# HannesStark/3DInfomax

Measured on AMD Instinct MI355X. Metric: molecules/sec pretraining step (PNA+Net3D, QM9-50k); PNA-agg HBM GB/s vs peak, higher is better.
Workload: dtype f32

## Files before the change

### 3dinfomax_amd/_lib.py

```python
import ctypes
import os
import re
from ctypes import POINTER, c_char_p, c_double, c_float, c_int, c_int64, c_long, c_uint64, c_void_p

HERE = os.path.dirname(os.path.abspath(__file__))
_TESTING = os.environ.get('I3D_TESTING') == '1'
TEST_HOOKS = dict(peer_selftest_fail=os.environ.get('I3D_TEST_PEER_SELFTEST_FAIL') if _TESTING else None,
                  peer_fail=os.environ.get('I3D_TEST_PEER_FAIL') if _TESTING else None,
                  force_early_allreduce=_TESTING and os.environ.get('I3D_TEST_FORCE_EARLY_ALLREDUCE') == '1',
                  verbose_selftest=_TESTING and bool(os.environ.get('I3D_DEBUG_SELFTEST')))
LIB_PATH = os.environ.get('I3D_LIB_PATH') or os.path.join(HERE, 'lib', 'lib3dinfomax_hip.so')
HEADER_PATH = os.path.join(os.path.dirname(HERE), 'include', 'infomax3d_hip.h')

ACT = {'none': 0, None: 0, 'relu': 1, 'silu': 2, 'sigmoid': 3, 'leakyrelu': 4, 'tanh': 5, 'elu': 6, 'selu': 7, 'softplus': 8}
AGG = {'mean': 0, 'sum': 1, 'max': 2, 'min': 3, 'std': 4, 'var': 5}
SCALER = {'identity': 0, 'amplification': 1, 'attenuation': 2}

_P = c_void_p


class BnTail(ctypes.Structure):
    _fields_ = [('act', c_int), ('post_act', c_int), ('eps', c_float), ('momentum', c_float), ('gamma', _P),
                ('beta', _P), ('running_mean', _P), ('running_var', _P), ('mean', _P), ('invstd', _P),
                ('workspace', _P), ('gemm_workspace', _P), ('gemm_workspace_bytes', c_long), ('num_batches_tracked', _P)]


class FcArgs(ctypes.Structure):
    _fields_ = [('tail', BnTail), ('rows', c_int), ('f_in', c_int), ('f_out', c_int), ('ldw', c_int), ('x', _P),
                ('W', _P), ('bias', _P), ('residual', _P), ('xact', _P), ('pre_keep', _P), ('y', _P), ('grad_y', _P),
                ('grad_pre', _P), ('grad_gamma', _P), ('grad_beta', _P), ('grad_W', _P), ('grad_bias', _P),
                ('grad_x', _P), ('W_dgrad_panel', _P), ('W_fwd_panel', _P)]


class EdgeFcArgs(ctypes.Structure):
    _fields_ = [('tail', BnTail), ('num_nodes', c_int), ('num_edges', c_int), ('f_h', c_int), ('f_q', c_int),
                ('f_out', c_int), ('ldw', c_int), ('q_rows', c_int), ('v_pad', c_int), ('q_code', _P), ('onehot', _P),
                ('grad_Q', _P), ('h', _P), ('q', _P), ('W', _P), ('bias', _P), ('src_s', _P),
                ('dst_s', _P), ('in_ptr', _P), ('out_ptr', _P), ('out_epos', _P), ('P', _P), ('Q', _P), ('xact', _P),
                ('pre_keep', _P), ('y', _P), ('grad_y', _P), ('grad_pre', _P), ('grad_P', _P), ('grad_gamma', _P),
                ('grad_beta', _P), ('grad_W', _P), ('grad_bias', _P), ('grad_h', _P), ('grad_q', _P),
                ('grad_q_accumulate', c_int)]


class GroupedFcArgs(ctypes.Structure):
    _fields_ = [('tail', BnTail), ('num_nodes', c_int), ('f_h', c_int), ('f_out', c_int), ('agg_width', c_int),
                ('ldw', c_int), ('n_groups', c_int), ('n_scalers', c_int), ('m_padded', c_int),
                ('group_start', c_int * 32), ('group_count', c_int * 32), ('coef', c_float * 128), ('h', _P),
                ('agg', _P), ('W', _P), ('bias', _P), ('residual', _P), ('deg_rows', _P), ('deg_tile_group', _P),
                ('WD', _P), ('xact', _P), ('pre_keep', _P), ('y', _P), ('grad_y', _P), ('grad_pre', _P),
                ('grad_WD', _P), ('grad_gamma', _P), ('grad_beta', _P), ('grad_W', _P), ('grad_bias', _P),
                ('grad_h', _P), ('grad_agg', _P)]


class PnaLayerArgs(ctypes.Structure):
    _fields_ = [('edge', EdgeFcArgs), ('n_pre_extra', c_int), ('pre', FcArgs * 3), ('n_aggregators', c_int),
                ('n_scalers', c_int), ('force_scalers', c_int), ('aggregators', c_int * 8), ('scalers', c_int * 4),
                ('avg_d_log', c_float), ('msg', _P), ('grad_msg', _P), ('post', GroupedFcArgs), ('n_post_extra', c_int),
                ('postx', FcArgs * 3), ('residual', c_int), ('grad_out', _P), ('agg_event_start', _P), ('agg_event_stop', _P),
                ('fused_bn', c_int), ('defer_join', c_int), ('stats_ws', _P), ('aff', _P * 4), ('weights_ready', c_int),
                ('merge_h', c_int), ('Wcat', _P), ('bcat', _P), ('PL', _P), ('DL', _P), ('wgrad_split', c_int), ('eval_mode', c_int), ('msg_bf16', c_int),
                ('edge_bias_partial', _P), ('Wcat_panel', _P), ('Wcat_dgrad_panel', _P)]


class Net3dEdgeArgs(ctypes.Structure):
    _fields_ = [('tail_in', BnTail), ('tail_msg', BnTail), ('num_nodes', c_int), ('num_edges', c_int), ('hidden', c_int),
                ('n_enc', c_int), ('reduce_mean', c_int), ('ld_w_in', c_int), ('ld_w_msg', c_int), ('d_raw', _P), ('perm', _P),
                ('dst_s', _P), ('in_ptr', _P), ('emb', _P), ('W_in', _P), ('b_in', _P), ('W_msg', _P), ('b_msg', _P),
                ('w_gate', _P), ('b_gate', _P), ('stats', _P), ('aff_in', _P), ('aff_msg', _P), ('x_msg', _P), ('d_out', _P),
                ('msg', _P), ('m_sum', _P), ('grad_m_sum', _P), ('grad_ya', _P), ('grad_lin', _P), ('partial', _P), ('grad_W_in', _P),
                ('grad_b_in', _P), ('grad_gamma_in', _P), ('grad_beta_in', _P), ('grad_W_msg', _P), ('grad_b_msg', _P),
                ('grad_gamma_msg', _P), ('grad_beta_msg', _P), ('grad_w_gate', _P), ('grad_b_gate', _P), ('grad_emb', _P), ('store_bf16', c_int), ('x_center', _P)]


class FcParams(ctypes.Structure):
    _fields_ = [('W', _P), ('bias', _P), ('gamma', _P), ('beta', _P), ('running_mean', _P), ('running_var', _P),
                ('num_batches_tracked', _P), ('grad_W', _P), ('grad_bias', _P), ('grad_gamma', _P), ('grad_beta', _P),
                ('f_in', c_int), ('f_out', c_int), ('act', c_int), ('eps', c_float), ('momentum', c_float)]


class PnaModel(ctypes.Structure):
    _fields_ = [('training', c_int), ('n_layers', c_int), ('hidden', c_int), ('n_pre', c_int), ('residual', c_int), ('n_aggregators', c_int),
                ('aggregators', c_int * 8), ('n_scalers', c_int), ('scalers', c_int * 4), ('avg_d_log', c_float),
                ('pre', (FcParams * 4) * 16), ('post', FcParams * 16), ('n_atom_tables', c_int), ('atom_dims', c_int * 16),
                ('atom_tables', _P * 16), ('grad_atom_tables', _P), ('n_bond_tables', c_int), ('bond_dims', c_int * 16),
                ('bond_tables', _P * 16), ('grad_bond_tables', _P), ('n_readout', c_int), ('readout_ops', c_int * 4),
                ('n_head', c_int), ('head', FcParams * 4)]


class PnaBatch(ctypes.Structure):
    _fields_ = [('num_nodes', c_int), ('num_edges', c_int), ('num_graphs', c_int), ('atom_feat', _P), ('bond_feat', _P),
                ('in_ptr', _P), ('perm', _P), ('src_s', _P), ('dst_s', _P), ('out_ptr', _P), ('out_epos', _P),
                ('graph_ptr', _P), ('deg_rows', _P), ('deg_tile_group', _P), ('m_padded', c_int), ('n_groups', c_int),
                ('group_degree', c_int * 32), ('group_start', c_int * 32), ('group_count', c_int * 32), ('comb', _P),
                ('n_comb', c_int), ('v_pad', c_int)]


class BnEvalAff(ctypes.Structure):
    _fields_ = [('running_mean', _P), ('running_var', _P), ('gamma', _P), ('beta', _P), ('aff', _P), ('feat', c_int),
                ('eps', c_float)]


class CopyBlock(ctypes.Structure):
    _fields_ = [('src', _P), ('dst', _P), ('rows', c_int), ('cols', c_int), ('ld_src', c_long), ('ld_dst', c_long)]


class TowerLayerArgs(ctypes.Structure):
    _fields_ = ([(n, c_int) for n in ('num_nodes', 'num_edges', 'f_in', 'f_edge', 'f_msg', 'f_out', 'f_mix', 'ldp', 'ldq', 'ldgp',
                                      'ldgq', 'n_aggregators', 'n_scalers', 'residual', 'training', 'grad_e_accumulate')]
                + [('aggregators', c_int * 8), ('scalers', c_int * 4), ('avg_d_log', c_float), ('eps', c_float), ('momentum', c_float)]
                + [(n, _P) for n in ('h', 'e', 'snorm', 'Wp', 'bp', 'Wq', 'bq', 'gamma', 'beta', 'running_mean', 'running_var', 'Wm',
                                     'bm', 'src_s', 'dst_s', 'in_ptr', 'out_ptr', 'out_epos', 'saved', 'scratch', 'workspace',
                                     'gemm_workspace')]
                + [('gemm_workspace_bytes', c_long)]
                + [(n, _P) for n in ('out', 'grad_out', 'grad_h', 'grad_e', 'grad_Wp', 'grad_bp', 'grad_Wq', 'grad_bq', 'grad_gamma',
                                     'grad_beta', 'grad_Wm', 'grad_bm')]
                + [('n_towers', c_int), ('n_deg_groups', c_int), ('m_padded', c_int), ('group_start', c_int * 32),
                   ('group_count', c_int * 32), ('coef', c_float * 128), ('deg_rows', _P), ('deg_tile_group', _P)])


class NodeDropView(ctypes.Structure):
    _fields_ = ([('keep', _P), ('graph_ptr', _P), ('edge_ptr', _P), ('deg_base', _P), ('pad_range', _P)]
                + [(n, c_int) for n in ('n_groups', 'num_nodes', 'num_edges', 'rows')]
                + [(n, _P) for n in ('src', 'dst', 'atom_feat', 'bond_feat', 'in_ptr', 'perm', 'src_s', 'dst_s', 'out_ptr', 'out_epos',
                                     'inv_perm', 'deg_rows')])


ALL_GATHER_F32 = ctypes.CFUNCTYPE(c_int, c_void_p, c_void_p, c_void_p, c_long, c_void_p)
ALL_REDUCE_F64 = ctypes.CFUNCTYPE(c_int, c_void_p, c_void_p, c_long, c_void_p)


class Collectives(ctypes.Structure):
    _fields_ = [('world', c_int), ('all_gather_f32', ALL_GATHER_F32), ('all_reduce_f64', ALL_REDUCE_F64), ('user', _P),
                ('scratch', _P), ('scratch_bytes', c_long)]


class WgradProblem(ctypes.Structure):
    _fields_ = [('A', _P), ('B', _P), ('rows', _P), ('rows_total', c_long), ('lda', c_int), ('ldb', c_int), ('M', c_int),
                ('N', c_int), ('k_begin', c_int), ('k_count', c_int)]


class WgradOutput(ctypes.Structure):
    _fields_ = [('kind', c_int), ('n_groups', c_int), ('first_problem', c_int), ('ldc', c_int), ('c_split', c_int),
                ('n_scalers', c_int), ('c_delta', c_long), ('scaler_stride', c_long), ('C', _P), ('aff', _P), ('row', _P),
                ('coef', POINTER(c_float))]


_SIGNATURES = {
    'i3d_bn_eval_aff_multi': (c_int, [POINTER(BnEvalAff), c_int, _P]),
    'i3d_set_collectives': (c_int, [POINTER(Collectives)]),
    'i3d_collectives_world': (c_int, []),
    'i3d_collectives_all_gather_f32': (c_int, [c_void_p, c_void_p, c_long, c_void_p]),
    'i3d_collectives_all_reduce_f64': (c_int, [c_void_p, c_long, c_void_p]),
    'i3d_rccl_available': (c_int, []),
    'i3d_rccl_unique_id': (c_int, [ctypes.c_char_p]),
    'i3d_rccl_init': (c_int, [ctypes.c_char_p, c_int, c_int, POINTER(c_void_p)]),
    'i3d_rccl_destroy': (c_int, [_P]),
    'i3d_set_collectives_rccl': (c_int, [_P, c_int, _P, c_long]),
    'i3d_block_copy': (c_int, [_P, c_int, c_int, _P]),
    'i3d_gru_gates_fwd': (c_int, [_P, _P, _P, c_int, c_int, _P, _P, _P]),
    'i3d_gru_gates_bwd': (c_int, [_P, _P, _P, _P, c_int, c_int, _P, _P, _P, _P]),
    'i3d_copy_cols': (c_int, [_P, c_int, c_int, _P, c_int, _P]),
    'i3d_edge_sqdist': (c_int, [_P, _P, _P, c_int, _P, c_int, c_int, c_int, _P]),
    'i3d_tower_layer_saved_floats': (c_long, [POINTER(TowerLayerArgs)]),
    'i3d_tower_layer_scratch_floats': (c_long, [POINTER(TowerLayerArgs)]),
    'i3d_tower_layer_fwd': (c_int, [POINTER(TowerLayerArgs), _P]),
    'i3d_tower_layer_bwd': (c_int, [POINTER(TowerLayerArgs), _P]),
    'i3d_peer_mailbox_bytes': (c_long, []),
    'i3d_peer_handle_bytes': (c_int, []),
    'i3d_peer_alloc': (c_int, [POINTER(c_void_p), ctypes.c_char_p]),
    'i3d_peer_free': (c_int, [_P]),
    'i3d_peer_open': (c_int, [_P, ctypes.c_char_p, c_int, c_int, c_double, POINTER(c_void_p)]),
    'i3d_set_collectives_peer': (c_int, [_P, _P, c_long]),
    'i3d_peer_bind_stream': (c_int, [_P, _P, _P, c_long]),
    'i3d_peer_status': (c_int, [_P]),
    'i3d_peer_sequence': (ctypes.c_longlong, [_P]),
    'i3d_peer_close': (c_int, [_P]),
    'i3d_gemm_f32_fused_src': (c_int, [c_int, c_int, c_int, _P, c_int, c_long, _P, c_int, _P, c_int, _P, c_int, _P, c_int, _P, c_int,
                                       _P, _P, _P, c_long, _P]),
    'i3d_pna_pack_h_weights': (c_int, [_P, c_int, c_int, _P, c_int, c_int, _P, c_int, _P, _P, _P]),
    'i3d_bn_bwd_strided': (c_int, [_P, _P, _P, c_int, c_int, c_int, c_int, _P, _P, _P, _P, _P, _P, _P, c_int, _P, _P, _P]),
    'i3d_wgrad_multi_supported': (c_int, [POINTER(WgradProblem), c_int, POINTER(WgradOutput), c_int]),
    'i3d_wgrad_multi_workspace_bytes': (c_long, [c_int]),
    'i3d_wgrad_multi_min_workspace_bytes': (c_long, [POINTER(WgradProblem), c_int]),
    'i3d_wgrad_multi': (c_int, [POINTER(WgradProblem), c_int, POINTER(WgradOutput), c_int, _P, c_long, _P]),
    'i3d_pna_model_saved_floats': (c_long, [POINTER(PnaModel), POINTER(PnaBatch)]),
    'i3d_pna_model_scratch_floats': (c_long, [POINTER(PnaModel), POINTER(PnaBatch)]),
    'i3d_pna_model_fwd': (c_int, [POINTER(PnaModel), POINTER(PnaBatch), _P, _P, _P, _P, _P, _P, _P, POINTER(c_void_p)]),
    'i3d_pna_model_bwd': (c_int, [_P, POINTER(PnaModel), _P, _P, _P, _P, c_long, _P]),
    'i3d_pna_model_bwd_part': (c_int, [_P, POINTER(PnaModel), _P, _P, _P, _P, c_long, c_int, c_int, _P]),
    'i3d_pna_model_ctx_free': (c_int, [_P]),
    'i3d_pna_messages_normalized': (c_int, [_P, _P, c_long, c_int, _P, _P]),
    'i3d_pna_messages_normalized_ex': (c_int, [_P, c_int, _P, c_long, c_int, _P, _P]),
    'i3d_pna_model_debug_messages': (c_int, [_P, c_int, _P, _P]),
    'i3d_event_create': (c_int, [POINTER(c_void_p)]),
    'i3d_event_destroy': (c_int, [_P]),
    'i3d_event_record': (c_int, [_P, _P]),
    'i3d_event_elapsed_ms': (c_int, [_P, _P, POINTER(c_float)]),
    'i3d_set_matmul_precision': (c_int, [c_int]),
    'i3d_get_matmul_precision': (c_int, []),
    'i3d_set_fp32_products': (c_int, [c_int]),
    'i3d_get_fp32_products': (c_int, []),
    'i3d_net3d_edge_supported': (c_int, [c_int, c_int]),
    'i3d_net3d_edge_stats_floats': (c_long, [c_int, c_int]),
    'i3d_net3d_edge_bwd_floats': (c_long, [c_int, c_int, c_int]),
    'i3d_net3d_edge_fwd': (c_int, [POINTER(Net3dEdgeArgs), _P]),
    'i3d_net3d_edge_bwd': (c_int, [POINTER(Net3dEdgeArgs), _P]),
    'i3d_wgrad_stream_fork': (c_int, [_P, POINTER(_P)]),
    'i3d_wgrad_stream_peek': (c_int, [_P, POINTER(_P)]),
    'i3d_pna_layer_weights_fwd': (c_int, [POINTER(PnaLayerArgs), _P]),
    'i3d_pna_layer_fwd': (c_int, [POINTER(PnaLayerArgs), _P]),
    'i3d_pna_layer_bwd': (c_int, [POINTER(PnaLayerArgs), _P]),
    'i3d_fc_bn_fwd': (c_int, [POINTER(FcArgs), _P]),
    'i3d_fc_bn_bwd': (c_int, [POINTER(FcArgs), _P]),
    'i3d_fc_bn_bwd_chain': (c_int, [POINTER(FcArgs), _P]),
    'i3d_fc_bn_bwd_wgrad': (c_int, [POINTER(FcArgs), _P]),
    'i3d_edge_fc_bn_fwd': (c_int, [POINTER(EdgeFcArgs), _P]),
    'i3d_edge_fc_bn_bwd': (c_int, [POINTER(EdgeFcArgs), _P]),
    'i3d_grouped_fc_bn_fwd': (c_int, [POINTER(GroupedFcArgs), _P]),
    'i3d_grouped_fc_bn_bwd': (c_int, [POINTER(GroupedFcArgs), _P]),
    'i3d_pna_layer_stats_floats': (c_long, [c_int, c_int, c_int, c_int]),
    'i3d_bn_finalize_partials': (c_int, [_P, c_int, c_int, c_float, c_float, _P, _P, _P, _P, _P, _P, _P, _P, _P]),
    'i3d_edge_stats_rows_per_tile': (c_int, [c_int]),
    'i3d_edge_combine_act_stats': (c_int, [_P, c_int, _P, _P, _P, _P, _P, c_int, c_int, c_int, _P, _P, _P]),
    'i3d_gemm_f32_fused': (c_int, [c_int, c_int, c_int, _P, c_int, c_long, _P, c_int, _P, c_int, _P, c_int, _P, c_int, _P, _P,
                                   _P, c_long, _P]),
    'i3d_gemm_f32_wgrad_bn': (c_int, [c_int, c_int, c_int, _P, c_int, _P, c_int, _P, c_int, _P, _P, _P, c_long, _P]),
    'i3d_pna_aggregate_fwd_aff': (c_int, [_P, _P, _P, c_int, c_int, POINTER(c_int), c_int, POINTER(c_int), c_int, c_int, c_float,
                                          _P, _P]),
    'i3d_pna_aggregate_fwd_ex': (c_int, [_P, c_int, _P, _P, c_int, c_int, POINTER(c_int), c_int, POINTER(c_int), c_int, c_int, c_float, _P, _P]),
    'i3d_pna_aggregate_bwd_ex': (c_int, [_P, _P, c_int, _P, _P, c_int, c_int, POINTER(c_int), c_int, POINTER(c_int), c_int, c_int, c_float, _P, _P]),
    'i3d_gemm_f32_fused_bf16out': (c_int, [c_int, c_int, c_int, _P, c_int, c_long, _P, c_int, _P, c_int, _P, _P, c_int, _P, _P]),
    'i3d_bn_bwd_x_bf16': (c_int, [_P, _P, c_int, c_int, c_int, c_int, _P, _P, _P, _P, _P, _P, _P, _P, _P, _P]),
    'i3d_pna_aggregate_bwd_aff': (c_int, [_P, _P, _P, _P, c_int, c_int, POINTER(c_int), c_int, POINTER(c_int), c_int, c_int,
                                          c_float, _P, _P]),
    'i3d_bn_bias_partial_floats': (c_long, [c_int]),
    'i3d_set_bn_bwd_one_launch': (c_int, [c_int]),
    'i3d_panel_packed_bytes': (c_long, [c_int, c_int]),
    'i3d_panel_pack': (c_int, [_P, c_int, c_int, c_int, c_int, _P, _P]),
    'i3d_panel_pack_multi': (c_int, [_P, c_int, _P]),
    'i3d_panel_gemm': (c_int, [c_int, c_int, c_int, _P, c_int, _P, _P, c_int, _P, c_int, _P]),
    'i3d_panel_stats_tiles': (c_int, [c_int]),
    'i3d_panel_gemm_fused': (c_int, [c_int, c_int, c_int, _P, c_int, _P, _P, c_int, _P, _P, c_int, _P, _P]),
    'i3d_bn_bwd_one_launch_supported': (c_int, [c_int, c_int]),
    'i3d_bn_bwd_edge_sums': (c_int, [_P, _P, c_int, c_int, c_int, _P, _P, _P, _P, _P, _P, _P, _P, _P, _P, c_int, _P, _P, c_int, _P, _P]),
    'i3d_colsum_strided': (c_int, [_P, c_int, c_int, c_int, _P, _P, _P]),
    'i3d_wgrad_stream_join': (c_int, [_P]),
    'i3d_adam_chunk_elems': (c_int, []),
    'i3d_adam_chunk_bytes': (c_int, []),
    'i3d_adam_step': (c_int, [_P, c_int, _P, c_int, c_double, c_double, c_double, c_double, c_double, c_double, c_double, _P]),
    'i3d_ema_chunk_elems': (c_int, []),
    'i3d_ema_chunk_bytes': (c_int, []),
    'i3d_ema_update': (c_int, [_P, c_int, c_float, c_float, _P]),
    'i3d_ntxent_loss_scratch_floats': (c_long, [c_int, c_int]),
    'i3d_ntxent_loss_fwd': (c_int, [_P, _P, c_int, c_int, c_int, c_int, c_int, c_float, c_float, c_float, _P, _P, _P]),
    'i3d_ntxent_loss_bwd': (c_int, [_P, _P, c_int, c_int, c_int, c_int, c_int, c_float, c_float, c_float, _P, _P, _P, _P, _P, _P]),
    'i3d_abi_version': (c_int, []),
    'i3d_last_error': (c_char_p, []),
    'i3d_embedding_sum_fwd': (c_int, [_P, _P, c_int, c_int, POINTER(c_void_p), c_int, _P, _P]),
    'i3d_embedding_sum_bwd': (c_int, [_P, _P, c_int, c_int, _P, c_int, POINTER(c_void_p), POINTER(c_int), _P]),
    'i3d_pna_aggregate_fwd_towers': (c_int, [_P, _P, c_int, c_int, c_int, POINTER(c_int), c_int, POINTER(c_int), c_int, c_int, c_float, _P, _P]),
    'i3d_pna_aggregate_bwd_towers': (c_int, [_P, _P, _P, c_int, c_int, c_int, POINTER(c_int), c_int, POINTER(c_int), c_int, c_int, c_float,
                                             _P, _P]),
    'i3d_pna_aggregate_fwd': (c_int, [_P, _P, c_int, c_int, POINTER(c_int), c_int, POINTER(c_int), c_int, c_int, c_float, _P,
                                      _P]),
    'i3d_pna_aggregate_bwd': (c_int, [_P, _P, _P, c_int, c_int, POINTER(c_int), c_int, POINTER(c_int), c_int, c_int, c_float,
                                      _P, _P]),
    'i3d_segment_readout_fwd': (c_int, [_P, _P, c_int, c_int, POINTER(c_int), c_int, _P, _P]),
    'i3d_segment_readout_bwd': (c_int, [_P, _P, _P, c_int, c_int, POINTER(c_int), c_int, _P, _P]),
    'i3d_gemm_f32': (c_int, [c_int, c_int, c_int, c_int, c_int, _P, c_int, _P, c_int, _P, c_int, _P, c_int, _P]),
    'i3d_gemm_f32_ex': (c_int, [c_int, c_int, c_int, c_int, c_int, _P, c_int, _P, c_int, _P, c_int, _P, c_int, c_int, c_int,
                                _P, c_long, _P]),
    'i3d_gemm_f32_blocks': (c_int, [c_int, c_int, c_int, c_int, c_int, _P, c_int, _P, c_int, c_int, c_long, c_long, _P, c_int,
                                    c_int, c_long, c_int, _P, c_long, _P]),
    'i3d_gemm_f32_ws': (c_int, [c_int, c_int, c_int, c_int, c_int, _P, c_int, _P, c_int, _P, c_int, _P, c_int, _P, c_long, _P]),
    'i3d_gemm_f32_grouped_batched': (c_int, [c_int, c_int, c_int, c_int, _P, c_int, c_long, c_long, _P, _P, _P, c_int, c_long, c_long, _P, c_int,
                                             c_long, c_int, c_int, _P]),
    'i3d_gemm_f32_batched': (c_int, [c_int, c_int, c_int, c_int, c_int, _P, c_int, c_long, _P, c_int, c_long, _P, c_int, c_long, c_int,
                                     c_int, _P, c_long, _P]),
    'i3d_pna_combine_weights_fwd': (c_int, [_P, c_int, c_int, c_int, c_int, c_int, c_int, POINTER(c_float), _P, _P]),
    'i3d_pna_combine_weights_bwd': (c_int, [_P, c_int, c_int, c_int, c_int, c_int, c_int, POINTER(c_float), _P, _P]),
    'i3d_gemm_f32_grouped': (c_int, [c_int, c_int, c_int, c_int, _P, c_int, c_long, _P, _P, _P, c_int, c_long, _P, c_int,
                                     c_int, _P]),
    'i3d_gemm_f32_rowsubset': (c_int, [c_int, c_int, c_int, _P, c_int, _P, c_int, _P, c_long, _P, c_int, c_int, _P]),
    'i3d_gemm_f32_rowsubset_multi': (c_int, [c_int, c_int, c_int, POINTER(c_int), POINTER(c_int), _P, c_int, _P, c_int, _P,
                                             c_long, _P, c_long, c_int, c_int, c_int, c_int, _P, c_long, _P]),
    'i3d_colreduce_workspace_bytes': (c_long, [c_int, c_int]),
    'i3d_act_stats_fwd': (c_int, [_P, c_int, c_int, c_int, _P, c_float, c_float, _P, _P, _P, _P, _P, _P, _P]),
    'i3d_act_stats_fwd_counted': (c_int, [_P, c_int, c_int, c_int, _P, c_float, c_float, _P, _P, _P, _P, _P, _P, _P, _P]),
    'i3d_bn_finalize_stats': (c_int, [_P, c_int, c_float, c_float, _P, _P, _P, _P, _P]),
    'i3d_bn_apply_fwd': (c_int, [_P, c_int, c_int, _P, _P, _P, _P, c_int, _P, _P, _P]),
    'i3d_bn_eval_fwd': (c_int, [_P, c_int, c_int, _P, _P, c_float, _P, _P, c_int, _P, _P, _P]),
    'i3d_bn_bwd': (c_int, [_P, _P, _P, c_int, c_int, c_int, c_int, _P, _P, _P, _P, _P, _P, _P, _P, _P, _P, c_long, _P, _P]),
    'i3d_bn_eval_bwd': (c_int, [_P, _P, _P, c_int, c_int, c_int, c_int, _P, _P, c_float, _P, _P, _P, _P, _P, _P, _P]),
    'i3d_colsum': (c_int, [_P, _P, c_int, c_int, _P, _P, _P]),
    'i3d_act_fwd': (c_int, [_P, c_long, c_int, _P, _P]),
    'i3d_act_bwd': (c_int, [_P, _P, c_long, c_int, _P, _P]),
    'i3d_add_inplace': (c_int, [_P, _P, c_long, _P]),
    'i3d_add': (c_int, [_P, _P, c_long, _P, _P]),
    'i3d_mul': (c_int, [_P, _P, c_long, _P, _P]),
    'i3d_broadcast_row': (c_int, [_P, c_long, c_int, _P, _P]),
    'i3d_edge_combine_fwd': (c_int, [_P, c_int, _P, _P, _P, _P, _P, c_int, c_int, _P, _P]),
    'i3d_multihot': (c_int, [_P, _P, c_int, c_int, POINTER(c_int), c_int, _P, _P]),
    'i3d_edge_codes': (c_int, [_P, _P, c_int, c_int, POINTER(c_int), c_int, _P, _P, _P]),
    'i3d_segment_sum_bf16': (c_int, [_P, c_int, _P, _P, c_int, c_int, c_int, _P, c_int, _P]),
    'i3d_segment_sum_pair': (c_int, [_P, c_int, _P, _P, _P, _P, _P, _P, c_int, c_int, c_int, _P]),
    'i3d_segment_sum': (c_int, [_P, c_int, _P, _P, c_int, c_int, c_int, _P, c_int, _P]),
    'i3d_segment_bcast': (c_int, [_P, _P, _P, c_int, c_int, c_int, _P, _P]),
    'i3d_gather_rows': (c_int, [_P, _P, c_int, c_int, _P, _P]),
    'i3d_fourier_encode': (c_int, [_P, c_int, c_int, _P, _P]),
    'i3d_soft_edge_fwd': (c_int, [_P, _P, _P, c_int, c_int, _P, _P, _P]),
    'i3d_soft_edge_bwd': (c_int, [_P, _P, _P, _P, c_int, c_int, _P, _P, _P]),
    'i3d_row_norms': (c_int, [_P, c_int, c_int, _P, _P]),
    'i3d_ntxent_fwd': (c_int, [_P, _P, _P, c_int, c_int, c_int, c_int, c_float, c_float, c_float, _P, _P, _P, _P]),
    'i3d_ntxent_bwd': (c_int, [_P, _P, _P, _P, _P, c_int, c_int, c_int, c_int, c_float, c_float, c_float, _P, _P, _P, _P, _P]),
    'i3d_row_axpy': (c_int, [_P, _P, c_int, c_int, _P, _P]),
    'i3d_row_scale': (c_int, [_P, _P, c_int, c_int, _P, _P]),
    'i3d_contrastive_metrics_out_doubles': (c_long, [c_int, c_int]),
    'i3d_contrastive_metrics_work_floats': (c_long, [c_int] * 5),
    'i3d_contrastive_metrics': (c_int, [_P, _P] + [c_int] * 5 + [c_float] * 3 + [_P, _P, _P]),
    'i3d_complete_graph_build': (c_int, [_P, _P, _P, c_int, c_int, c_int, _P, _P, _P, _P, _P, _P, _P, _P, _P, _P]),
    'i3d_mha_fwd': (c_int, [_P, _P, c_int, c_int, c_int, c_int, c_float, _P, _P, _P]),
    'i3d_mha_bwd': (c_int, [_P, _P, _P, _P, _P, c_int, c_int, c_int, c_int, c_float, _P, _P, _P]),
    'i3d_ln_res_fwd': (c_int, [_P, _P, _P, _P, c_int, c_int, c_float, _P, _P, _P, _P]),
    'i3d_ln_res_partial_floats': (c_long, [c_int, c_int]),
    'i3d_ln_res_bwd': (c_int, [_P, _P, _P, _P, _P, _P, c_int, c_int, _P, _P, _P, _P, _P]),
    'i3d_pair_sum_fwd': (c_int, [_P, _P, _P, _P, _P, c_int, c_int, _P, _P]),
    'i3d_pair_sum_bwd': (c_int, [_P, _P, _P, _P, _P, _P, c_int, c_int, _P, _P]),
    'i3d_pair_norm_fwd': (c_int, [_P, _P, _P, _P, c_int, c_int, _P, _P]),
    'i3d_pair_norm_bwd': (c_int, [_P, _P, _P, _P, _P, _P, c_int, c_int, _P, _P]),
    'i3d_pair_mlp_supported': (c_int, [c_int]),
    'i3d_pair_mlp_workspace_floats': (c_long, [c_int, c_int]),
    'i3d_pair_mlp_fwd': (c_int, [_P] * 9 + [c_int, c_int, c_int, c_float, c_float] + [_P] * 8),
    'i3d_pair_mlp_bwd': (c_int, [_P] * 13 + [c_int, c_int, c_int, c_int] + [_P] * 10),
    'i3d_mse_partial_floats': (c_long, [c_long]),
    'i3d_mse_fwd': (c_int, [_P, _P, c_long, c_double, _P, _P, _P]),
    'i3d_mse_bwd': (c_int, [_P, _P, c_long, c_double, _P, _P, _P, _P]),
    'i3d_node_drop_build': (c_int, [_P, _P, _P, _P, _P, _P, _P, _P, _P, _P, _P, c_int, c_int, c_int, c_int, c_int, c_int,
                                    POINTER(NodeDropView), c_int, _P]),
    'i3d_noised_graph_build': (c_int, [_P, _P, _P, c_int, c_int, c_int, c_int, c_int, c_float, c_uint64, c_uint64] + [_P] * 12),
    'i3d_row_normalize_fwd': (c_int, [_P, c_int, c_int, _P, _P, _P]),
    'i3d_row_normalize_bwd': (c_int, [_P, _P, _P, c_int, c_int, _P, _P]),
    'i3d_sep2d_max_conformers': (c_int, []),
    'i3d_sep2d_fwd': (c_int, [_P, _P, _P, c_int, c_int, c_float, _P, _P, _P, _P]),
    'i3d_sep2d_bwd': (c_int, [_P, _P, _P, _P, _P, c_int, c_int, c_float, _P, _P, _P, _P, _P]),
    'i3d_mmd_pair_fwd': (c_int, [_P, _P, c_int, c_int, c_int, c_int, c_double, _P, _P, _P, _P, _P]),
    'i3d_mmd_pair_bwd': (c_int, [_P] * 7 + [c_int, c_int, c_int, c_int, c_double] + [_P] * 5),
    'i3d_kl_mp_fwd': (c_int, [_P, _P, c_int, c_int, c_int, c_double, _P, _P, _P]),
    'i3d_kl_mp_bwd': (c_int, [_P, _P, c_int, c_int, c_int, c_double, _P, _P, _P, _P]),
    'i3d_gauss_lik_fwd': (c_int, [_P, _P, c_int, c_int, c_int, c_long, c_long, _P, _P]),
    'i3d_gauss_lik_loss': (c_int, [_P, c_int, c_double, _P, _P, _P]),
    'i3d_gauss_lik_probs': (c_int, [_P, c_int, _P, _P]),
    'i3d_gauss_lik_bwd': (c_int, [_P, _P, c_int, c_int, c_int, c_long, c_long, _P, _P, c_double, _P, _P, _P, _P, _P]),
    'i3d_gauss_jsd_fwd': (c_int, [_P, _P, c_int, c_int, c_int, _P, _P, _P, _P, _P]),
    'i3d_gauss_jsd_bwd': (c_int, [_P, _P, c_int, c_int, c_int, _P, _P, _P, _P, _P, _P]),
    'i3d_masked_loss_partial_floats': (c_long, [c_int, c_int]),
    'i3d_masked_loss_fwd': (c_int, [_P, _P, c_int, c_int, c_int, _P, _P, _P]),
    'i3d_masked_loss_bwd': (c_int, [_P, _P, c_int, c_int, c_int, _P, _P, _P, _P]),
    'i3d_task_moments_partial_floats': (c_long, [c_int, c_int]),
    'i3d_task_moments': (c_int, [_P, _P, c_int, c_int, _P, _P, _P]),
    'i3d_gin_chunk_edges': (c_int, []),
    'i3d_gin_conv_bwd_partial_floats': (c_long, [c_int, c_int, c_int, c_int]),
    'i3d_gin_conv_fwd': (c_int, [_P, _P, _P, c_int, _P, c_int, _P, _P, _P, _P, c_int, c_int, c_int, _P, _P, _P]),
    'i3d_gin_conv_bwd': (c_int, [_P] * 3 + [c_int] + [_P] * 8 + [c_int, c_int, c_int] + [_P] * 5),
    'i3d_gate_reduce_max_feat': (c_int, []),
    'i3d_gate_reduce_fwd': (c_int, [_P] * 5 + [c_int] * 4 + [_P] * 3),
    'i3d_gate_reduce_bwd': (c_int, [_P] * 5 + [c_int] * 4 + [_P] * 4),
    'i3d_geomol_edge_fwd': (c_int, [_P] * 4 + [c_int] * 3 + [_P] * 2),
    'i3d_geomol_edge_bwd': (c_int, [_P] * 5 + [c_int] * 3 + [_P] * 3),
    'i3d_geomol_residual_fwd': (c_int, [_P] * 3 + [c_long, c_int] + [_P] * 2),
    'i3d_geomol_residual_bwd': (c_int, [_P] * 3 + [c_long, c_int] + [_P] * 4),
    'i3d_lg_row_chunk': (c_int, []),
    'i3d_lg_ntxent_scratch_floats': (c_long, [c_int, c_int]),
    'i3d_lg_ntxent_work_floats': (c_long, [c_int, c_int, c_int]),
    'i3d_lg_ntxent_fwd': (c_int, [_P, _P, _P, c_int, c_int, c_int, c_float, c_float, c_int, _P, _P, _P]),
    'i3d_lg_ntxent_bwd': (c_int, [_P, _P, _P, c_int, c_int, c_int, c_float, c_float, c_int, _P, _P, _P, _P, _P, _P]),
    'i3d_conf_match_max_conformers': (c_int, []),
    'i3d_per_conf_max_conformers': (c_int, []),
    'i3d_conf_match_work_floats': (c_long, [c_int]),
    'i3d_conf_match_fwd': (c_int, [_P, _P, _P, c_int, c_int, c_int, c_float] + [_P] * 8),
    'i3d_conf_match_bwd': (c_int, [_P] * 9 + [c_int, c_int, c_int, c_int, c_int, c_float] + [_P] * 5),
    'i3d_per_conf_fwd': (c_int, [_P, _P, _P, c_int, c_int, c_int, c_float, _P, _P, _P, _P]),
    'i3d_per_conf_bwd': (c_int, [_P] * 5 + [c_int, c_int, c_int, c_float] + [_P] * 5),
    'i3d_hardneg_max_extra': (c_int, []),
    'i3d_hardneg_norms': (c_int, [_P] * 3 + [c_int] * 5 + [_P] * 5),
    'i3d_hardneg_fwd': (c_int, [c_int] + [_P] * 5 + [c_int] * 4 + [c_double] * 5 + [_P] * 4),
    'i3d_hardneg_bwd': (c_int, [c_int] + [_P] * 9 + [c_int] * 6 + [c_double] * 3 + [_P] * 8),
    'i3d_hardneg_loss_scratch_floats': (c_long, [c_int, c_int, c_int]),
    'i3d_hardneg_loss_fwd': (c_int, [c_int] + [_P] * 3 + [c_int] * 6 + [c_double] * 5 + [_P] * 3),
    'i3d_hardneg_loss_bwd': (c_int, [c_int] + [_P] * 3 + [c_int] * 6 + [c_double] * 3 + [_P] * 7),
    'i3d_bs_max_repeats': (c_int, []),
    'i3d_bs_pass_blocks': (c_int, [c_int]),
    'i3d_bs_moments': (c_int, [_P, _P, c_int, c_int] + [_P] * 6),
    'i3d_bs_matrix_pass': (c_int, [_P, c_int, c_int] + [c_double] * 4 + [_P, _P]),
    'i3d_bs_finish': (c_int, [_P, c_int, c_double, _P, c_int, c_int, c_double, _P, _P]),
    'i3d_bs_col_bwd': (c_int, [_P] * 8 + [c_int, c_int, _P] + [c_double] * 4 + [_P] * 4),
    'i3d_bs_rows_fwd': (c_int, [_P, _P, c_int, c_int, c_int, _P, _P, _P]),
    'i3d_bs_rows_bwd': (c_int, [_P, _P, c_int, c_int, c_int, _P, c_double] + [_P] * 4),
}

_lib = None


class HipLibraryError(RuntimeError):
    pass


def declared_symbols():
    with open(HEADER_PATH) as f:
        text = f.read()
    text = re.sub(r'/\*.*?\*/', '', text, flags=re.S)
    return sorted(set(re.findall(r'\b(i3d_[a-z0-9_]+)\s*\(', text)))


def load():
    global _lib
    if _lib is not None:
        return _lib
    if not os.path.exists(LIB_PATH):
        raise HipLibraryError(
            f'{LIB_PATH} not found: build it with `python -c "import __graft_entry__ as g; g.build()"` '
            '(hipcc --offload-arch=gfx950).  There is no CPU fallback for the product path.')
    lib = ctypes.CDLL(LIB_PATH)
    for name, (res, args) in _SIGNATURES.items():
        fn = getattr(lib, name)
        fn.restype = res
        fn.argtypes = args
    prec = os.environ.get('I3D_MATMUL_PRECISION', 'fp32').lower()
    if prec not in ('fp32', 'bf16'):
        raise HipLibraryError(f'I3D_MATMUL_PRECISION={prec!r}: fp32 or bf16')
    lib.i3d_set_matmul_precision(int(prec == 'bf16'))
    _lib = lib
    return lib


NOT_TAKEN = 1


def check(rc, name):
    if rc != 0:
        msg = load().i3d_last_error()
        raise HipLibraryError(f'{name} failed (rc={rc}): {msg.decode() if msg else ""}')


def int_array(values):
    return (c_int * len(values))(*values)


def ptr_array(ptrs):
    return (c_void_p * len(ptrs))(*ptrs)
```

### 3dinfomax_amd/csrc/composite.hip

```cpp
#include "common.h"

using namespace i3d;

#define TRY(call)                 \
    do {                          \
        int rc_ = (call);         \
        if (rc_ != I3D_OK) return rc_; \
    } while (0)

#include <algorithm>
#include <cstdlib>
#include <cstring>
#include <map>
#include <mutex>
#include <utility>

namespace {

struct Aux {
    hipStream_t s = nullptr;
    hipEvent_t fork = nullptr, join = nullptr;
};

Aux* aux_for(hipStream_t main) {
// ... 162 lines not shown
        const int V = a->q_rows;
        TRY(i3d_gemm_f32_ws(1, 0, a->v_pad, Fo, E, a->onehot, a->v_pad, a->grad_pre, Fo, a->grad_Q, Fo, nullptr, 0, ws, wsb, wst));
        TRY(i3d_gemm_f32_ws(1, 0, Fo, a->f_q, V, a->grad_Q, Fo, a->q, a->f_q, a->grad_W + 2 * Fh, a->ldw, nullptr, 0, ws, wsb, wst));
        if (a->grad_q != nullptr)
            TRY(i3d_gemm_f32(0, 0, V, a->f_q, Fo, a->grad_Q, Fo, a->W + 2 * Fh, a->ldw, a->grad_q, a->f_q, nullptr,
                             a->grad_q_accumulate, wst));
    } else if (a->q != nullptr) {
        TRY(i3d_gemm_f32_ws(1, 0, Fo, a->f_q, E, a->grad_pre, Fo, a->q, a->f_q, a->grad_W + 2 * Fh, a->ldw, nullptr, 0, ws, wsb, wst));
        if (a->grad_q != nullptr)
            TRY(i3d_gemm_f32(0, 0, E, a->f_q, Fo, a->grad_pre, Fo, a->W + 2 * Fh, a->ldw, a->grad_q, a->f_q, nullptr, 0, wst));
    }
    return I3D_OK;
}

static int edge_fc_bn_bwd_wgrad(const I3dEdgeFcArgs* a, void* wst) {
    TRY(edge_fc_bn_bwd_wgrad_p(a, wst));
    return edge_fc_bn_bwd_wgrad_q(a, wst);
}

extern "C" int i3d_edge_fc_bn_bwd(const I3dEdgeFcArgs* a, void* stream) {
    I3D_CHECK_ARG(a != nullptr && a->num_edges > 0 && a->num_nodes > 0, "bad arguments");
    TRY(edge_fc_bn_bwd_chain(a, stream));
    TRY(edge_fc_bn_bwd_wgrad(a, stream));
    return edge_fc_bn_bwd_dgrad(a, stream);
}

extern "C" int i3d_grouped_fc_bn_fwd(const I3dGroupedFcArgs* a, void* stream) {
    I3D_CHECK_ARG(a != nullptr && a->num_nodes > 0 && a->n_groups > 0, "bad arguments");
    const int Fh = a->f_h, Fo = a->f_out, A = a->agg_width, N = a->num_nodes;
    float* lin = a->pre_keep ? a->pre_keep : a->xact;
    TRY(i3d_gemm_f32(0, 1, N, Fo, Fh, a->h, Fh, a->W, a->ldw, lin, Fo, a->bias, 0, stream));
    TRY(i3d_pna_combine_weights_fwd(a->W, a->ldw, Fh, Fo, A, a->n_groups, a->n_scalers, a->coef, a->WD, stream));
    TRY(i3d_gemm_f32_grouped(1, a->m_padded, Fo, A, a->agg, A, N, a->deg_rows, a->deg_tile_group, a->WD, A, (long)Fo * A, lin,
                             Fo, 1, stream));
    return tail_fwd(&a->tail, N, Fo, lin, a->xact, a->residual, a->y, stream);
}

static int grouped_fc_bn_bwd_chain(const I3dGroupedFcArgs* a, void* stream, int grad_h_accumulate = 0) {
    const int Fh = a->f_h, Fo = a->f_out, A = a->agg_width, N = a->num_nodes;
    TRY(tail_bwd(&a->tail, N, Fo, a->grad_y, a->xact, a->pre_keep, a->grad_gamma, a->grad_beta, a->grad_pre, a->grad_bias,
                 stream));
    TRY(i3d_gemm_f32(0, 0, N, Fh, Fo, a->grad_pre, Fo, a->W, a->ldw, a->grad_h, Fh, nullptr, grad_h_accumulate, stream));
    return i3d_gemm_f32_grouped(0, a->m_padded, A, Fo, a->grad_pre, Fo, N, a->deg_rows, a->deg_tile_group, a->WD, A,
                                (long)Fo * A, a->grad_agg, A, 0, stream);
}

static int grouped_fc_bn_bwd_wgrad(const I3dGroupedFcArgs* a, void* wst) {
    const int Fh = a->f_h, Fo = a->f_out, A = a->agg_width, N = a->num_nodes;
    TRY(i3d_gemm_f32_ws(1, 0, Fo, Fh, N, a->grad_pre, Fo, a->h, Fh, a->grad_W, a->ldw, nullptr, 0, a->tail.gemm_workspace,
                        a->tail.gemm_workspace_bytes, wst));
    TRY(i3d_gemm_f32_rowsubset_multi(Fo, A, a->n_groups, a->group_start, a->group_count, a->grad_pre, Fo, a->agg, A,
                                     a->deg_rows, N, a->grad_WD, (long)Fo * A, A, 0, -1, 0, a->tail.gemm_workspace,
                                     a->tail.gemm_workspace_bytes, wst));
    return i3d_pna_combine_weights_bwd(a->grad_WD, a->ldw, Fh, Fo, A, a->n_groups, a->n_scalers, a->coef, a->grad_W, wst);
}

extern "C" int i3d_grouped_fc_bn_bwd(const I3dGroupedFcArgs* a, void* stream) {
    I3D_CHECK_ARG(a != nullptr && a->num_nodes > 0 && a->n_groups > 0, "bad arguments");
    TRY(grouped_fc_bn_bwd_chain(a, stream));
    return grouped_fc_bn_bwd_wgrad(a, stream);
}

static bool merge_h_ok(const I3dPnaLayerArgs* a) {
    return a->merge_h && a->fused_bn && a->n_post_extra == 0 && a->Wcat != nullptr && a->bcat != nullptr && a->PL != nullptr &&
           a->post.f_h == a->edge.f_h && a->post.pre_keep == nullptr;
}

static int pack_layer_weights(const I3dPnaLayerArgs* a, void* stream) {
    const I3dEdgeFcArgs* e = &a->edge;
    const I3dGroupedFcArgs* p = &a->post;
    TRY(i3d_pna_pack_h_weights(e->W, e->ldw, e->f_out, p->W, p->ldw, p->f_out, p->bias, e->f_h, a->Wcat, a->bcat, stream));
    I3dPanelPack w[8];
    int n = 0;
    const int WL = 2 * e->f_out + p->f_out;
    if (a->Wcat_panel != nullptr) w[n++] = I3dPanelPack{a->Wcat, e->f_h, WL, e->f_h, 1, a->Wcat_panel};
    if (a->Wcat_dgrad_panel != nullptr) w[n++] = I3dPanelPack{a->Wcat, e->f_h, e->f_h, WL, 0, a->Wcat_dgrad_panel};
    for (int i = 0; i < a->n_pre_extra && n + 2 <= 8; ++i) {
        const I3dFcArgs* c = &a->pre[i];
        if (c->W_dgrad_panel != nullptr) w[n++] = I3dPanelPack{c->W, c->ldw, c->f_in, c->f_out, 0, c->W_dgrad_panel};
        if (c->W_fwd_panel != nullptr) w[n++] = I3dPanelPack{c->W, c->ldw, c->f_out, c->f_in, 1, c->W_fwd_panel};
    }
    if (n > 0) TRY(i3d_panel_pack_multi(w, n, stream));
    return I3D_OK;
}

static bool edge_bias_on_chain(const I3dPnaLayerArgs* a) {
    return a->wgrad_split != 0;
}

static bool edge_bwd_fused_ok(const I3dPnaLayerArgs* a) {
    const I3dEdgeFcArgs* e = &a->edge;
    return merge_h_ok(a) && a->DL != nullptr && e->pre_keep == nullptr && relu_class(e->tail.act) && e->tail.post_act == I3D_ACT_NONE &&
           e->f_out % 4 == 0 && e->f_out <= 512 && a->post.f_out % 4 == 0 && e->out_ptr != nullptr && e->out_epos != nullptr &&
           a->edge_bias_partial != nullptr && e->grad_bias != nullptr;
}

static int pna_layer_wgrad_multi(const I3dPnaLayerArgs* a, void* wst, bool dry_run, int part = 0) {
    static const bool on = [] { const char* e = getenv("I3D_WGRAD_MULTI"); return e == nullptr || e[0] != '0'; }();
    const I3dEdgeFcArgs* e = &a->edge;
    const I3dGroupedFcArgs* g = &a->post;
    if (!on || a->n_post_extra != 0 || e->q == nullptr || e->q_rows <= 0) return 0;
    const int Fh = e->f_h, Fo = e->f_out, N = e->num_nodes, E = e->num_edges, A = g->agg_width;
    const bool merged = merge_h_ok(a) && a->DL != nullptr;
    const int WL = 2 * Fo + g->f_out;
    const float* dlin = merged ? a->DL + 2 * Fo : g->grad_pre;
    const int ld_dlin = merged ? WL : g->f_out;
    const float* dP = merged ? a->DL : e->grad_P;
    const int ld_dP = merged ? WL : 2 * Fo;
    constexpr int MAX_PROBLEMS = 40, MAX_OUTPUTS = 8, MAX_GROUPS = 32, MAX_SCALERS = 4;
    I3dWgradProblem pr[MAX_PROBLEMS];
    I3dWgradOutput out[MAX_OUTPUTS];
    float coef[MAX_GROUPS * MAX_SCALERS];
    const int fixed_problems = 3 + (a->n_pre_extra > 0 ? a->n_pre_extra : 0);
    if (g->n_scalers > MAX_SCALERS || g->n_scalers < 0 || fixed_problems >= MAX_PROBLEMS || 4 + a->n_pre_extra > MAX_OUTPUTS) return 0;
    const int max_group_problems = MAX_PROBLEMS - fixed_problems < MAX_GROUPS ? MAX_PROBLEMS - fixed_problems : MAX_GROUPS;
    std::memset(pr, 0, sizeof(pr));
    std::memset(out, 0, sizeof(out));
    int np = 0, no = 0;
    auto problem = [&](const float* Ap, int lda, int M, const float* Bp, int ldb, int Nn, long rows_total, const int* rows,
                       int k_begin, int k_count) {
        I3dWgradProblem& p = pr[np++];
        p.A = Ap; p.B = Bp; p.rows = rows; p.rows_total = rows_total; p.lda = lda; p.ldb = ldb; p.M = M; p.N = Nn;
        p.k_begin = k_begin; p.k_count = k_count;
    };
    const bool do_post = part != 2, do_pre = part != 1;
    if (do_post) {
        out[no].kind = I3D_WGRAD_PLAIN; out[no].n_groups = 1; out[no].first_problem = np; out[no].C = g->grad_W; out[no].ldc = g->ldw;
        ++no;
        problem(dlin, ld_dlin, g->f_out, g->h, Fh, Fh, N, nullptr, 0, N);
    }
    if (do_post) {
        I3dWgradOutput& o = out[no];
        o.kind = I3D_WGRAD_COMBINE; o.first_problem = np; o.C = g->grad_W + Fh; o.ldc = g->ldw;
        o.n_scalers = g->n_scalers; o.scaler_stride = A; o.coef = coef;
        int ng = 0;
        for (int k = 0; k < g->n_groups; ++k) {
            bool any = false;
            for (int s = 0; s < g->n_scalers; ++s) any = any || g->coef[k * g->n_scalers + s] != 0.f;
            if (!any || g->group_count[k] == 0) continue;
            if (ng >= max_group_problems) return 0;
            for (int s = 0; s < g->n_scalers; ++s) coef[ng * g->n_scalers + s] = g->coef[k * g->n_scalers + s];
            problem(dlin, ld_dlin, g->f_out, g->agg, A, A, N, g->deg_rows, g->group_start[k], g->group_count[k]);
            ++ng;
        }
        if (ng == 0) return 0;
        o.n_groups = ng;
        ++no;
    }
    for (int i = a->n_pre_extra - 1; i >= 0 && do_pre; --i) {
        const I3dFcArgs* c = &a->pre[i];
        I3dWgradOutput& o = out[no++];
        o.n_groups = 1; o.first_problem = np; o.C = c->grad_W; o.ldc = c->ldw;
        if (a->fused_bn) { o.kind = I3D_WGRAD_BN; o.aff = a->aff[i]; o.row = c->grad_bias; }
        else o.kind = I3D_WGRAD_PLAIN;
        problem(c->grad_pre, c->f_out, c->f_out, c->x, c->f_in, c->f_in, c->rows, nullptr, 0, c->rows);
    }
    if (do_pre) {
        I3dWgradOutput& o = out[no++];
        o.kind = I3D_WGRAD_PLAIN; o.n_groups = 1; o.first_problem = np; o.C = e->grad_W; o.ldc = e->ldw;
        o.c_split = Fo; o.c_delta = (long)Fh - (long)Fo * e->ldw;
        problem(dP, ld_dP, 2 * Fo, e->h, Fh, Fh, N, nullptr, 0, N);
    }
    if (do_pre) {
        I3dWgradOutput& o = out[no++];
        o.kind = I3D_WGRAD_PLAIN; o.n_groups = 1; o.first_problem = np; o.C = e->grad_Q; o.ldc = Fo;
        problem(e->onehot, e->v_pad, e->v_pad, e->grad_pre, Fo, Fo, E, nullptr, 0, E);
// ... 3 lines not shown
    if (ws == nullptr || !i3d_wgrad_multi_supported(pr, np, out, no) || i3d_wgrad_multi_min_workspace_bytes(pr, np) > wsb) return 0;
    if (dry_run) return 1;
    if (do_pre && edge_bwd_fused_ok(a) && !edge_bias_on_chain(a))
        TRY(i3d_colsum_strided(a->DL + Fo, 2 * Fo + a->post.f_out, N, Fo, e->grad_bias, a->edge_bias_partial, wst));
    TRY(i3d_wgrad_multi(pr, np, out, no, ws, wsb, wst));
    if (!do_pre) return 1;
    const int V = e->q_rows;
    TRY(i3d_gemm_f32_ws(1, 0, Fo, e->f_q, V, e->grad_Q, Fo, e->q, e->f_q, e->grad_W + 2 * Fh, e->ldw, nullptr, 0, ws, wsb, wst));
    if (e->grad_q != nullptr)
        TRY(i3d_gemm_f32(0, 0, V, e->f_q, Fo, e->grad_Q, Fo, e->W + 2 * Fh, e->ldw, e->grad_q, e->f_q, nullptr, e->grad_q_accumulate, wst));
    return 1;
}

static bool wgrad_multi_layer_ok(const I3dPnaLayerArgs* a);

static bool simple_act(int act) { return act == I3D_ACT_NONE || act == I3D_ACT_RELU || act == I3D_ACT_LEAKY_RELU; }

static int finalize_stats(const I3dBnTail* t, const float* partial, int tiles, int feat, float* aff, void* stream,
                          int eval_mode = 0) {
    if (eval_mode) return I3D_OK;
    return i3d_bn_finalize_partials(partial, tiles, feat, t->eps, t->momentum, t->gamma, t->beta, t->mean, t->invstd,
                                    t->running_mean, t->running_var, t->num_batches_tracked, aff, stream);
}

static int pna_layer_fwd_fused(const I3dPnaLayerArgs* a, void* stream) {
    const I3dEdgeFcArgs* e = &a->edge;
    const int Fh = e->f_h, Fo = e->f_out, N = e->num_nodes, E = e->num_edges;
    I3D_CHECK_ARG(a->stats_ws != nullptr && a->n_post_extra == 0 && e->pre_keep == nullptr && simple_act(e->tail.act) &&
                      e->tail.post_act == I3D_ACT_NONE && a->aff[0] != nullptr, "fused BatchNorm: unsupported block shape");
    const I3dGroupedFcArgs* pg = &a->post;
    const bool merged = merge_h_ok(a);
    const int WL = 2 * Fo + pg->f_out;
    const float* P = e->P;
    int ldp = 2 * Fo;
    if (merged) {
        if (!a->weights_ready) TRY(pack_layer_weights(a, stream));
        if (panel_ok(a->Wcat_panel, Fh, WL))
            TRY(i3d_panel_gemm(N, WL, Fh, e->h, Fh, a->Wcat_panel, a->PL, WL, a->bcat, 0, stream));
        else
            TRY(i3d_gemm_f32(0, 1, N, WL, Fh, e->h, Fh, a->Wcat, Fh, a->PL, WL, a->bcat, 0, stream));
        P = a->PL;
        ldp = WL;
    } else {
        const long wdelta = (long)Fh - (long)Fo * e->ldw, wview = (long)(Fo - 1) * e->ldw + 2 * Fh;
        TRY(i3d_gemm_f32_blocks(0, 1, N, 2 * Fo, Fh, e->h, Fh, e->W, e->ldw, Fo, wdelta, wview, e->P, 2 * Fo, 0, 0, 0, nullptr, 0,
                                stream));
    }
    if (e->q != nullptr && !a->weights_ready)
        TRY(i3d_gemm_f32(0, 1, e->q_rows > 0 ? e->q_rows : E, Fo, e->f_q, e->q, e->f_q, e->W + 2 * Fh, e->ldw, e->Q, Fo,
                         nullptr, 0, stream));
    TRY(i3d_edge_combine_act_stats(P, ldp, e->q ? e->Q : nullptr, e->q_rows > 0 ? e->q_code : nullptr, e->bias, e->src_s,
                                   e->dst_s, E, Fo, e->tail.act, e->xact, a->stats_ws, stream));
    TRY(finalize_stats(&e->tail, a->stats_ws, cdiv(E, i3d_edge_stats_rows_per_tile(Fo)), Fo, a->aff[0], stream, a->eval_mode));
    const float* x = e->xact;
    const float* aff = a->aff[0];
    int f_in = Fo;
    for (int i = 0; i < a->n_pre_extra; ++i) {
        const I3dFcArgs* c = &a->pre[i];
        I3D_CHECK_ARG(c->pre_keep == nullptr && simple_act(c->tail.act) && c->tail.post_act == I3D_ACT_NONE &&
                          a->aff[i + 1] != nullptr && c->rows == E && c->f_in == f_in, "fused BatchNorm: unsupported block shape");
        int stat_tiles = cdiv(E, 64);
        if (a->msg_bf16 && i == a->n_pre_extra - 1)
            TRY(i3d_gemm_f32_fused_bf16out(E, c->f_out, f_in, x, f_in, E, c->W, c->ldw, c->xact, c->f_out, c->bias, aff, c->tail.act,
                                           a->stats_ws, stream));
        else if (merged && panel_ok(c->W_fwd_panel, f_in, c->f_out) && (((uintptr_t)x | (uintptr_t)c->xact | (uintptr_t)aff) & 15) == 0) {
            TRY(i3d_panel_gemm_fused(E, c->f_out, f_in, x, f_in, c->W_fwd_panel, c->xact, c->f_out, c->bias, aff, c->tail.act, a->stats_ws,
                                     stream));
            stat_tiles = i3d_panel_stats_tiles(E);
        } else
            TRY(i3d_gemm_f32_fused(E, c->f_out, f_in, x, f_in, E, c->W, c->ldw, c->xact, c->f_out, c->bias, 0, aff, c->tail.act,
                                   a->stats_ws, nullptr, nullptr, 0, stream));
        TRY(finalize_stats(&c->tail, a->stats_ws, stat_tiles, c->f_out, a->aff[i + 1], stream, a->eval_mode));
        x = c->xact;
        aff = a->aff[i + 1];
        f_in = c->f_out;
    }
    if (a->agg_event_start != nullptr && a->agg_event_stop != nullptr) k4_time_next_launch(a->agg_event_start, a->agg_event_stop);
    TRY(i3d_pna_aggregate_fwd_ex(x, a->msg_bf16 && a->n_pre_extra > 0, aff, e->in_ptr, N, f_in, a->aggregators, a->n_aggregators, a->scalers,
                                 a->n_scalers, a->force_scalers, a->avg_d_log, const_cast<float*>(a->post.agg), stream));
    const I3dGroupedFcArgs* p = &a->post;
    I3D_CHECK_ARG(p->pre_keep == nullptr && simple_act(p->tail.act), "fused BatchNorm: unsupported block shape");
    const int A = p->agg_width, Fp = p->f_out;
    if (!merged) TRY(i3d_gemm_f32(0, 1, N, Fp, p->f_h, p->h, p->f_h, p->W, p->ldw, p->xact, Fp, p->bias, 0, stream));
    if (!a->weights_ready)
        TRY(i3d_pna_combine_weights_fwd(p->W, p->ldw, p->f_h, Fp, A, p->n_groups, p->n_scalers, p->coef, p->WD, stream));
    TRY(i3d_gemm_f32_fused_src(p->m_padded, Fp, A, p->agg, A, N, p->WD, A, p->xact, Fp, merged ? a->PL + 2 * Fo : nullptr, WL,
                               nullptr, 1, nullptr, p->tail.act, a->stats_ws, p->deg_rows, p->deg_tile_group, (long)Fp * A, stream));
    if (a->eval_mode)
        return i3d_bn_eval_fwd(p->xact, N, Fp, p->tail.running_mean, p->tail.running_var, p->tail.eps, p->tail.gamma, p->tail.beta,
                               p->tail.post_act, p->residual, p->y, stream);
    TRY(finalize_stats(&p->tail, a->stats_ws, p->m_padded / 64, Fp, nullptr, stream));
    return i3d_bn_apply_fwd(p->xact, N, Fp, p->tail.mean, p->tail.invstd, p->tail.gamma, p->tail.beta, p->tail.post_act,
                            p->residual, p->y, stream);
}

extern "C" int i3d_pna_layer_weights_fwd(const I3dPnaLayerArgs* a, void* stream) {
    I3D_CHECK_ARG(a != nullptr && a->fused_bn, "fused_bn layers only");
    const I3dEdgeFcArgs* e = &a->edge;
    const I3dGroupedFcArgs* p = &a->post;
    if (e->q != nullptr)
        TRY(i3d_gemm_f32(0, 1, e->q_rows > 0 ? e->q_rows : e->num_edges, e->f_out, e->f_q, e->q, e->f_q, e->W + 2 * e->f_h, e->ldw,
                         e->Q, e->f_out, nullptr, 0, stream));
    if (merge_h_ok(a)) TRY(pack_layer_weights(a, stream));
    return i3d_pna_combine_weights_fwd(p->W, p->ldw, p->f_h, p->f_out, p->agg_width, p->n_groups, p->n_scalers, p->coef, p->WD,
                                       stream);
}

extern "C" int i3d_wgrad_stream_fork(void* stream, void** side) {
    I3D_CHECK_ARG(side != nullptr, "null");
    *side = fork_wgrad(aux_for((hipStream_t)stream), stream);
    return I3D_OK;
}

extern "C" int i3d_wgrad_stream_peek(void* stream, void** side) {
    I3D_CHECK_ARG(side != nullptr, "null");
    Aux* x = aux_for((hipStream_t)stream);
    *side = x != nullptr ? (void*)x->s : stream;
    return I3D_OK;
}

extern "C" long i3d_pna_layer_stats_floats(int num_nodes, int num_edges, int m_padded, int f) {
    (void)num_nodes;
    const int rpt = i3d_edge_stats_rows_per_tile(f);
    long tiles = cdiv(num_edges, rpt > 0 ? rpt : 1);
    tiles = std::max<long>(tiles, 2L * cdiv(num_edges, 64));
    tiles = std::max<long>(tiles, m_padded / 64 + 1);
    return tiles * 3 * f;
}

extern "C" int i3d_pna_layer_fwd(const I3dPnaLayerArgs* a, void* stream) {
    I3D_CHECK_ARG(a != nullptr && a->n_pre_extra >= 0 && a->n_pre_extra <= I3D_MAX_EXTRA_FC && a->n_post_extra >= 0 &&
                      a->n_post_extra <= I3D_MAX_EXTRA_FC, "bad arguments");
    if (a->fused_bn) return pna_layer_fwd_fused(a, stream);
    TRY(i3d_edge_fc_bn_fwd(&a->edge, stream));
    for (int i = 0; i < a->n_pre_extra; ++i) TRY(i3d_fc_bn_fwd(&a->pre[i], stream));
    if (a->agg_event_start != nullptr && a->agg_event_stop != nullptr) k4_time_next_launch(a->agg_event_start, a->agg_event_stop);
    TRY(i3d_pna_aggregate_fwd(a->msg, a->edge.in_ptr, a->edge.num_nodes, a->edge.f_out, a->aggregators, a->n_aggregators,
                              a->scalers, a->n_scalers, a->force_scalers, a->avg_d_log, const_cast<float*>(a->post.agg), stream));
    TRY(i3d_grouped_fc_bn_fwd(&a->post, stream));
    for (int i = 0; i < a->n_post_extra; ++i) TRY(i3d_fc_bn_fwd(&a->postx[i], stream));
    return I3D_OK;
}

extern "C" int i3d_pna_layer_bwd(const I3dPnaLayerArgs* a, void* stream) {
    I3D_CHECK_ARG(a != nullptr && a->n_pre_extra >= 0 && a->n_pre_extra <= I3D_MAX_EXTRA_FC && a->n_post_extra >= 0 &&
                      a->n_post_extra <= I3D_MAX_EXTRA_FC, "bad arguments");
    Aux* x = aux_for((hipStream_t)stream);
    for (int i = a->n_post_extra - 1; i >= 0; --i) TRY(fc_bn_bwd_chain(&a->postx[i], stream));
    const bool inplace = a->residual && a->post.grad_h == a->grad_out && a->n_post_extra == 0;
    I3D_CHECK_ARG(a->post.grad_h != a->grad_out || inplace, "grad_h may alias grad_out only for a residual layer without extra blocks");
    const bool multi = wgrad_multi_layer_ok(a);
    const bool merged = multi && merge_h_ok(a) && a->DL != nullptr;
    const long n = (long)a->edge.num_nodes * a->edge.f_h;
    if (merged) {
        const I3dGroupedFcArgs* g = &a->post;
        const int WLb = 2 * a->edge.f_out + g->f_out;
        float* dlin = a->DL + 2 * a->edge.f_out;
        TRY(i3d_bn_bwd_strided(g->grad_y, g->xact, g->pre_keep, g->num_nodes, g->f_out, g->tail.act, g->tail.post_act, g->tail.mean,
                               g->tail.invstd, g->tail.gamma, g->tail.beta, g->grad_gamma, g->grad_beta, dlin, WLb, g->grad_bias,
                               g->tail.workspace, stream));
        TRY(i3d_gemm_f32_grouped(0, g->m_padded, g->agg_width, g->f_out, dlin, WLb, g->num_nodes, g->deg_rows, g->deg_tile_group, g->WD,
                                 g->agg_width, (long)g->f_out * g->agg_width, g->grad_agg, g->agg_width, 0, stream));
    } else {
        TRY(grouped_fc_bn_bwd_chain(&a->post, stream, inplace ? 1 : 0));
        if (a->residual && !inplace) TRY(i3d_add_inplace(a->post.grad_h, a->grad_out, n, stream));
    }
    void* wst = stream;
    if (multi && a->wgrad_split) {
        wst = fork_wgrad(x, stream);
        const int took = pna_layer_wgrad_multi(a, wst, false, 1);
        if (took < 0) return took;
        I3D_CHECK_ARG(took == 1, "weight-gradient launch refused a layer it had accepted");
    }
    if (!multi) {
        wst = fork_wgrad(x, stream);
        TRY(grouped_fc_bn_bwd_wgrad(&a->post, wst));
        for (int i = a->n_post_extra - 1; i >= 0; --i) TRY(fc_bn_bwd_wgrad(&a->postx[i], wst));
    }
    const float* msg_aff = a->fused_bn ? a->aff[a->n_pre_extra] : nullptr;
    const int f_msg = a->n_pre_extra > 0 ? a->pre[a->n_pre_extra - 1].f_out : a->edge.f_out;
    const int msg16 = a->fused_bn && a->msg_bf16 && a->n_pre_extra > 0;
    TRY(i3d_pna_aggregate_bwd_ex(a->post.grad_agg, a->msg, msg16, msg_aff, a->edge.in_ptr, a->edge.num_nodes, f_msg, a->aggregators,
                                 a->n_aggregators, a->scalers, a->n_scalers, a->force_scalers, a->avg_d_log, a->grad_msg, stream));
    for (int i = a->n_pre_extra - 1; i >= 0; --i) TRY(fc_bn_bwd_chain(&a->pre[i], stream, msg16 && i == a->n_pre_extra - 1));
    const bool edge_fused = multi && merged && edge_bwd_fused_ok(a);
    if (edge_fused) {
        const I3dEdgeFcArgs* e = &a->edge;
        const int WLb = 2 * e->f_out + a->post.f_out;
        if (i3d_bn_bwd_one_launch_supported(e->num_edges, e->f_out)) {
            TRY(i3d_bn_bwd_strided(e->grad_y, e->xact, nullptr, e->num_edges, e->f_out, e->tail.act, I3D_ACT_NONE, e->tail.mean, e->tail.invstd,
                                   e->tail.gamma, e->tail.beta, e->grad_gamma, e->grad_beta, e->grad_pre, e->f_out, nullptr,
                                   e->tail.workspace, stream));
            TRY(i3d_segment_sum_pair(e->grad_pre, e->f_out, e->out_ptr, e->out_epos, a->DL, e->in_ptr, nullptr, a->DL + e->f_out,
                                     e->num_nodes, e->f_out, WLb, stream));
        } else
        TRY(i3d_bn_bwd_edge_sums(e->grad_y, e->xact, e->num_edges, e->f_out, e->tail.act, e->tail.mean, e->tail.invstd, e->tail.gamma,
                                 e->tail.beta, e->grad_gamma, e->grad_beta, e->grad_pre, e->in_ptr, e->out_ptr, e->out_epos, e->num_nodes,
                                 a->DL, a->DL + e->f_out, WLb, e->tail.workspace, stream));
    } else {
        TRY(edge_fc_bn_bwd_tail(&a->edge, stream));
    }
    if (multi) {
        if (edge_fused) {
        } else if (merged) {
            const I3dEdgeFcArgs* e = &a->edge;
            const int WLb = 2 * e->f_out + a->post.f_out;
            TRY(i3d_segment_sum_pair(e->grad_pre, e->f_out, e->out_ptr, e->out_epos, a->DL, e->in_ptr, nullptr, a->DL + e->f_out,
                                     e->num_nodes, e->f_out, WLb, stream));
        } else {
            TRY(edge_fc_bn_bwd_sums(&a->edge, stream));
        }
        wst = fork_wgrad(x, stream);
        const int took = pna_layer_wgrad_multi(a, wst, false, a->wgrad_split ? 2 : 0);
        if (took < 0) return took;
        I3D_CHECK_ARG(took == 1, "weight-gradient launch refused a layer it had accepted");
    } else {
        TRY(edge_fc_bn_bwd_sums(&a->edge, stream));
        wst = fork_wgrad(x, stream);
        for (int i = a->n_pre_extra - 1; i >= 0; --i) TRY(fc_bn_bwd_wgrad(&a->pre[i], wst, a->fused_bn ? a->aff[i] : nullptr));
        TRY(edge_fc_bn_bwd_wgrad(&a->edge, wst));
    }
    if (merged) {
        const int WLb = 2 * a->edge.f_out + a->post.f_out;
        if (panel_ok(a->Wcat_dgrad_panel, WLb, a->edge.f_h, 1024) && (((uintptr_t)a->DL | (uintptr_t)a->post.grad_h) & 15) == 0)
            TRY(i3d_panel_gemm(a->edge.num_nodes, a->edge.f_h, WLb, a->DL, WLb, a->Wcat_dgrad_panel, a->post.grad_h, a->edge.f_h, nullptr,
                               inplace ? 1 : 0, stream));
        else
            TRY(i3d_gemm_f32(0, 0, a->edge.num_nodes, a->edge.f_h, WLb, a->DL, WLb, a->Wcat, a->edge.f_h, a->post.grad_h, a->edge.f_h,
                             nullptr, inplace ? 1 : 0, stream));
        if (a->residual && !inplace) TRY(i3d_add_inplace(a->post.grad_h, a->grad_out, n, stream));
    } else {
        TRY(edge_fc_bn_bwd_dgrad(&a->edge, stream, a->post.grad_h));
    }
    if (edge_fused && edge_bias_on_chain(a)) {
        const int Fo = a->edge.f_out;
        TRY(i3d_colsum_strided(a->DL + Fo, 2 * Fo + a->post.f_out, a->edge.num_nodes, Fo, a->edge.grad_bias, a->edge_bias_partial, stream));
    }
    if (a->defer_join) return I3D_OK;
    return join_wgrad(x, stream);
}

static bool wgrad_multi_layer_ok(const I3dPnaLayerArgs* a) { return pna_layer_wgrad_multi(a, nullptr, true) == 1; }

extern "C" int i3d_wgrad_stream_join(void* stream) { return join_wgrad(aux_for((hipStream_t)stream), stream); }

extern "C" int i3d_event_create(void** event) {
    I3D_CHECK_ARG(event != nullptr, "null");
    hipEvent_t e;
    if (hipEventCreateWithFlags(&e, hipEventDisableSystemFence) != hipSuccess &&
        hipEventCreateWithFlags(&e, hipEventReleaseToDevice) != hipSuccess && hipEventCreate(&e) != hipSuccess) {
        i3d::set_error("hipEventCreate failed");
        return I3D_ERR_LAUNCH;
    }
    *event = (void*)e;
    return I3D_OK;
}

extern "C" int i3d_event_destroy(void* event) {
    if (event != nullptr) (void)hipEventDestroy((hipEvent_t)event);
    return I3D_OK;
}

extern "C" int i3d_event_record(void* event, void* stream) {
    I3D_CHECK_ARG(event != nullptr, "null");
    if (hipEventRecord((hipEvent_t)event, (hipStream_t)stream) != hipSuccess) {
        i3d::set_error("hipEventRecord failed");
        return I3D_ERR_LAUNCH;
    }
    return I3D_OK;
}

extern "C" int i3d_event_elapsed_ms(void* start, void* stop, float* ms) {
    I3D_CHECK_ARG(start != nullptr && stop != nullptr && ms != nullptr, "null");
    if (hipEventElapsedTime(ms, (hipEvent_t)start, (hipEvent_t)stop) != hipSuccess) {
        i3d::set_error("hipEventElapsedTime failed (events not completed?)");
        return I3D_ERR_LAUNCH;
    }
    return I3D_OK;
}
```

### 3dinfomax_amd/csrc/gemm.hip

```cpp
#include "common.h"
#include <algorithm>

namespace i3d {

typedef float floatx4 __attribute__((ext_vector_type(4)));
typedef float floatx16 __attribute__((ext_vector_type(16)));

struct GemmArgs {
    const float* A;
    const float* B;
    float* C;
    const float* bias;
    int M, N, K;
    int lda, ldb, ldc;
    int accumulate;
    int k_per_split;
    int atomic_out;
    int c_vec;
    unsigned a_bytes, b_bytes;
    const int* m_rows;
    const int* k_rows;
    const int* tile_group;
    long b_group_stride;
    int b_split, c_split;
    long b_delta, c_delta;
    float* slab;
    const float* a_aff;
    float* stats;
    int epi_act;
    const float* Cin;
    int ldcin;
    int c_bf16;
    int n_batch, z_splits;
    long a_batch, b_batch, c_batch;
};

__device__ __forceinline__ int swz(int k, int idx) { return idx ^ ((((k) ^ (k >> 2)) & 1) << 4); }

typedef __bf16 bf16x4 __attribute__((ext_vector_type(4)));
typedef __bf16 bf16x2_t __attribute__((ext_vector_type(2)));
typedef float f32x2_t __attribute__((ext_vector_type(2)));
__device__ __forceinline__ void split_pair(float a, float b, unsigned& hi, unsigned& mid, unsigned& lo) {
    auto pack = [](f32x2_t v) { return __builtin_bit_cast(unsigned, __builtin_convertvector(v, bf16x2_t)); };
    auto widen = [](unsigned u) { f32x2_t r; r.x = __uint_as_float(u << 16); r.y = __uint_as_float(u & 0xffff0000u); return r; };
    f32x2_t v;
    v.x = a; v.y = b;
    hi = pack(v);
    const f32x2_t r1 = v - widen(hi);
    mid = pack(r1);
    const f32x2_t r2 = r1 - widen(mid);
    lo = pack(r2);
}
template <int R, int LD, int BK, bool KC, bool IM = false, int NT = 256, int IH = 0>
struct TileStage {
    static constexpr int LDK = BK + 2;
    static constexpr int LDKH = BK + 8;
    static constexpr int IMG_HALVES = R * LDKH;
    static constexpr int LDS_FLOATS = IH ? IH * R * LDKH / 2 : (IM ? R * LDK : BK * LD);
    static constexpr int SLOTS = R * BK / 4;
    static constexpr int KQ = BK / 4;
    static constexpr int PER_THREAD = (SLOTS + NT - 1) / NT;
    struct Regs { float4 v[PER_THREAD]; };
    unsigned base[PER_THREAD];
    int kloc[PER_THREAD];
    int iloc[PER_THREAD];
    int rowi[PER_THREAD];
    bool ok[PER_THREAD];

    __device__ __forceinline__ void prepare(int ld, int idx0, int idx_max, const int* __restrict__ rows, int split = 0x7fffffff,
                                            long delta = 0) {
#pragma unroll
        for (int it = 0; it < PER_THREAD; ++it) {
            const int s = threadIdx.x + it * NT;
            if (KC) {
                const int idx = idx0 + s / KQ;
                kloc[it] = (s % KQ) * 4;
                int row = -1;
                if (idx < idx_max && s < SLOTS) row = rows ? rows[idx] : idx;
                ok[it] = row >= 0;
                iloc[it] = idx;
                rowi[it] = max(row, 0);
                base[it] = (unsigned)((long)max(row, 0) * ld + kloc[it] + (idx >= split ? delta : 0)) * 4u;
            } else {
                kloc[it] = s / (R / 4);
                iloc[it] = idx0 + (s % (R / 4)) * 4;
                ok[it] = iloc[it] < idx_max && s < SLOTS;
                rowi[it] = 0;
                base[it] = (unsigned)iloc[it] * 4u;
            }
        }
    }

    template <bool VEC, bool ROWS>
    __device__ __forceinline__ void load(Regs& r, __amdgpu_buffer_rsrc_t rsrc, unsigned oob, int ld, int idx_max, int k0,
                                         int k_begin, int k_end, const int* kidx, int split = 0x7fffffff,
                                         long delta = 0) const {
#pragma unroll
        for (int it = 0; it < PER_THREAD; ++it) {
            const int k = k0 + kloc[it];
            unsigned off;
            const bool valid = ok[it] && k < k_end;
            if (KC) {
                off = base[it] + (unsigned)k0 * 4u;
            } else {
                int krow = k;
                if (ROWS) krow = kidx[max(min(k, k_end - 1) - k_begin, 0)];
                off = (unsigned)((long)krow * ld + (k >= split ? delta : 0)) * 4u + base[it];
            }
            if (VEC) {
                auto q = __builtin_amdgcn_raw_buffer_load_b128(rsrc, valid ? off : oob, 0, 0);
                static_assert(sizeof(q) == 16, "b128 load");
                r.v[it] = __builtin_bit_cast(float4, q);
            } else {
                float e[4];
#pragma unroll
                for (int u = 0; u < 4; ++u) {
                    const bool oku = valid && (KC ? (k + u < k_end) : (iloc[it] + u < idx_max));
                    e[u] = __builtin_bit_cast(float, __builtin_amdgcn_raw_buffer_load_b32(rsrc, oku ? off + 4u * u : oob, 0, 0));
// ... 362 lines not shown
                }
                if constexpr ((FUSE & 2) != 0) {
                    if (g.accumulate) {
                        const float* ci = g.Cin != nullptr ? g.Cin + (long)row * g.ldcin + n : c;
#pragma unroll
                        for (int q = 0; q < 4; ++q)
                            if (n + q < g.N) r[q] += ci[q];
                    }
#pragma unroll
                    for (int q = 0; q < 4; ++q) r[q] = apply_act_c<false>(r[q], g.epi_act);
                    if (g.c_bf16) {
                        auto rne = [](float x) { const unsigned u = __float_as_uint(x); return (u + 0x7fffu + ((u >> 16) & 1u)) >> 16; };
                        unsigned short* c16 = reinterpret_cast<unsigned short*>(Cout) + (long)row * g.ldc + n;
                        *reinterpret_cast<uint2*>(c16) = make_uint2(rne(r[0]) | (rne(r[1]) << 16), rne(r[2]) | (rne(r[3]) << 16));
                    } else if (full && g.c_vec) {
                        *reinterpret_cast<float4*>(c) = make_float4(r[0], r[1], r[2], r[3]);
                    } else {
#pragma unroll
                        for (int q = 0; q < 4; ++q)
                            if (n + q < g.N) c[q] = r[q];
                    }
#pragma unroll
                    for (int q = 0; q < 4; ++q) Ct[ml * CT_PITCH + nl + q] = r[q];
                    continue;
                }
                if (g.atomic_out) {
#pragma unroll
                    for (int q = 0; q < 4; ++q)
                        if (n + q < g.N) unsafeAtomicAdd(c + q, r[q]);
                } else if (full && g.c_vec) {
                    float4 o = make_float4(r[0], r[1], r[2], r[3]);
                    if (g.accumulate) {
                        float4 old = *reinterpret_cast<const float4*>(c);
                        o.x += old.x; o.y += old.y; o.z += old.z; o.w += old.w;
                    }
                    *reinterpret_cast<float4*>(c) = o;
                } else {
#pragma unroll
                    for (int q = 0; q < 4; ++q)
                        if (n + q < g.N) c[q] = g.accumulate ? c[q] + r[q] : r[q];
                }
            }
        }
    }
    if constexpr ((FUSE & 2) != 0) {
        static_assert(S::NT == 4 * BN, "statistics epilogue: four row quarters per column");
        __syncthreads();
        const int cl = threadIdx.x % BN, part = threadIdx.x / BN;
        constexpr int RQ = BM / 4;
        float x[RQ], v[RQ];
        float s1 = 0.f, cnt = 0.f;
#pragma unroll
        for (int k = 0; k < RQ; ++k) {
            const int ml = part * RQ + k;
            v[k] = rvalid[ml];
            x[k] = v[k] != 0.f ? Ct[ml * CT_PITCH + cl] : 0.f;
            s1 += x[k];
            cnt += v[k];
        }
        red[part * BN + cl] = s1;
        red[4 * BN + part * BN + cl] = cnt;
        __syncthreads();
        const float tot = ((red[cl] + red[BN + cl]) + red[2 * BN + cl]) + red[3 * BN + cl];
        const float n_rows = ((red[4 * BN + cl] + red[5 * BN + cl]) + red[6 * BN + cl]) + red[7 * BN + cl];
        const float mean_t = n_rows > 0.f ? tot / n_rows : 0.f;
        float m2 = 0.f;
#pragma unroll
        for (int k = 0; k < RQ; ++k) {
            const float d = x[k] - mean_t;
            if (v[k] != 0.f) m2 += d * d;
        }
        __syncthreads();
        red[part * BN + cl] = m2;
        __syncthreads();
        if (part == 0 && n0 + cl < g.N) {
            float* o = g.stats + (long)bx * 3 * g.N + n0 + cl;
            o[0] = tot;
            o[g.N] = ((red[cl] + red[BN + cl]) + red[2 * BN + cl]) + red[3 * BN + cl];
            o[2 * g.N] = n_rows;
        }
    }
}

template <class S, bool VEC, bool A_KC, bool B_KC, int BF16 = 0>
__global__ void __launch_bounds__(256)
gemm_f32_kernel(GemmArgs g) {
    I3D_CHAIN_PRIO();
    int bx, by, bz;
    xcd_tile(bx, by, bz);
    const int slice = bz;
    if (g.n_batch > 1) {
        const int bb = bz / g.z_splits;
        bz -= bb * g.z_splits;
        g.A += bb * g.a_batch; g.B += bb * g.b_batch; g.C += bb * g.c_batch;
    }
    const int k_begin = bz * g.k_per_split;
    const int k_end = min(g.K, k_begin + g.k_per_split);
    if (g.slab != nullptr) {
        GemmArgs gl = g;
        gl.ldc = g.N; gl.accumulate = 0; gl.atomic_out = 0; gl.c_vec = (g.N % 4 == 0); gl.bias = nullptr;
        gl.c_split = 0x7fffffff; gl.c_delta = 0;
        gemm_body<S, VEC, A_KC, B_KC, false, 0, BF16>(gl, bx, by, min(k_begin, g.K), k_end, g.slab + (long)slice * g.M * g.N, nullptr,
                                                      false);
        return;
    }
    if (k_begin >= k_end && !(bz == 0)) return;
    gemm_body<S, VEC, A_KC, B_KC, false, 0, BF16>(g, bx, by, k_begin, k_end, g.C, nullptr, bz == 0);
}

template <class S, bool VEC, int BF16 = 0>
__global__ void __launch_bounds__(256)
gemm_f32_rowseg_kernel(GemmArgs g, SegTable segs) {
    I3D_CHAIN_PRIO();
    __shared__ int kidx[SEG_MAX_K];
    int bx, by, bz;
    xcd_tile(bx, by, bz);
    const Seg sg = segs.s[bz];
    for (int i = threadIdx.x; i < sg.k_end - sg.k_begin; i += S::NT) kidx[i] = g.k_rows[sg.k_begin + i];
    __syncthreads();
    if (g.slab != nullptr) {
        GemmArgs gl = g;
        gl.ldc = g.N; gl.accumulate = 0; gl.atomic_out = 0; gl.c_vec = (g.N % 4 == 0);
        gl.c_split = 0x7fffffff; gl.c_delta = 0;
        gemm_body<S, VEC, false, false, true, 0, BF16>(gl, bx, by, sg.k_begin, sg.k_end, g.slab + (long)bz * g.M * g.N, kidx, false);
        return;
    }
    gemm_body<S, VEC, false, false, true, 0, BF16>(g, bx, by, sg.k_begin, sg.k_end, g.C + sg.c_off, kidx, false);
}

struct SlabReduce {
    const float* slab;
    float* C;
    const float* bias;
    int M, N, ldc, accumulate, n_groups;
    long c_group_stride;
    int c_split;
    long c_delta;
    int seg_ptr[34];
    const float* post_aff;
    const float* post_row;
};

template <int V>
__global__ void __launch_bounds__(256) slab_reduce_kernel(SlabReduce a) {
    I3D_CHAIN_PRIO();
    const int NV = a.N / V;
    const long per_group = (long)a.M * NV;
    long t = (long)blockIdx.x * blockDim.x + threadIdx.x;
    if (t >= per_group * a.n_groups) return;
    const int gi = (int)(t / per_group);
    const long r = t - gi * per_group;
    const int m = (int)(r / NV), n = (int)(r - (long)m * NV) * V;
    float* c = a.C + gi * a.c_group_stride + (long)m * a.ldc + n + (m >= a.c_split ? a.c_delta : 0);
    float acc[V];
#pragma unroll
    for (int i = 0; i < V; ++i) acc[i] = a.accumulate ? c[i] : 0.f;
    const long slice = (long)a.M * a.N;
    const float* p = a.slab + (long)m * a.N + n;
    const int z_end = a.seg_ptr[gi + 1];
    for (int z0 = a.seg_ptr[gi]; z0 < z_end; z0 += 4) {
        float x[4][V];
#pragma unroll
        for (int k = 0; k < 4; ++k) {
            const float* q = p + (long)min(z0 + k, z_end - 1) * slice;
            if (V == 4) {
                const float4 t4 = *reinterpret_cast<const float4*>(q);
                x[k][0] = t4.x; x[k][1 % V] = t4.y; x[k][2 % V] = t4.z; x[k][3 % V] = t4.w;
            } else {
                x[k][0] = q[0];
            }
        }
#pragma unroll
        for (int k = 0; k < 4; ++k) {
            if (z0 + k < z_end) {
#pragma unroll
                for (int i = 0; i < V; ++i) acc[i] += x[k][i];
            }
// ... 115 lines not shown
static void launch(const GemmArgs& g, int layout, int splits, bool vec, hipStream_t s) {
    dim3 grid(cdiv(g.M, S::BM), cdiv(g.N, S::BN), splits * (g.n_batch > 1 ? g.n_batch : 1)), block(S::NT);
    if constexpr (split_shape<S>()) {
        if (!g_matmul_bf16 && g_fp32_split && vec && layout <= 1) {
            if (layout == 0) hipLaunchKernelGGL((gemm_f32_kernel<S, true, true, true, 2>), grid, block, 0, s, g);
            else hipLaunchKernelGGL((gemm_f32_kernel<S, true, true, false, 2>), grid, block, 0, s, g);
            return;
        }
    }
    if constexpr (bf16_shape<S>()) {
        if (g_matmul_bf16 && vec) {
            switch (layout) {
                case 0: hipLaunchKernelGGL((gemm_f32_kernel<S, true, true, true, true>), grid, block, 0, s, g); break;
                case 1: hipLaunchKernelGGL((gemm_f32_kernel<S, true, true, false, true>), grid, block, 0, s, g); break;
                default: hipLaunchKernelGGL((gemm_f32_kernel<S, true, false, false, true>), grid, block, 0, s, g); break;
            }
            return;
        }
    }
#define I3D_GEMM_LAUNCH(V, AK, BKC) hipLaunchKernelGGL((gemm_f32_kernel<S, V, AK, BKC>), grid, block, 0, s, g)
    switch (layout * 2 + (vec ? 1 : 0)) {
        case 0: I3D_GEMM_LAUNCH(false, true, true); break;
        case 1: I3D_GEMM_LAUNCH(true, true, true); break;
        case 2: I3D_GEMM_LAUNCH(false, true, false); break;
        case 3: I3D_GEMM_LAUNCH(true, true, false); break;
        case 4: I3D_GEMM_LAUNCH(false, false, false); break;
        default: I3D_GEMM_LAUNCH(true, false, false); break;
    }
#undef I3D_GEMM_LAUNCH
}

template <class S>
static void launch_rowseg(const GemmArgs& g, const SegTable& t, int n_segs, bool vec, hipStream_t s) {
    dim3 grid(cdiv(g.M, S::BM), cdiv(g.N, S::BN), n_segs);
    if constexpr (bf16_shape<S>()) {
        if (g_matmul_bf16 && vec) {
            hipLaunchKernelGGL((gemm_f32_rowseg_kernel<S, true, true>), grid, dim3(S::NT), 0, s, g, t);
            return;
        }
    }
    if (vec) hipLaunchKernelGGL((gemm_f32_rowseg_kernel<S, true>), grid, dim3(S::NT), 0, s, g, t);
    else hipLaunchKernelGGL((gemm_f32_rowseg_kernel<S, false>), grid, dim3(S::NT), 0, s, g, t);
}

typedef Shape<32, 2, 2, 2, 2, 16, 2> Cfg0;
typedef Shape<16, 4, 1, 4, 2, 16, 2> Cfg1;
typedef Shape<32, 2, 2, 1, 1, 16, 4> Cfg2;
typedef Shape<16, 2, 2, 1, 2, 32, 2> Cfg3;
typedef Shape<32, 2, 2, 1, 1, 32, 2> Cfg4;
typedef Shape<32, 2, 2, 2, 1, 16, 4> Cfg5;
typedef Shape<32, 2, 2, 1, 1, 16, 1> Cfg6;
typedef Shape<32, 2, 2, 1, 1, 16, 2> Cfg7;
typedef Shape<16, 2, 2, 1, 1, 32, 2> Cfg8;
typedef Shape<32, 2, 2, 1, 1, 16, 4, true> Cfg9;
typedef Shape<32, 2, 2, 2, 2, 16, 2, true> Cfg10;
typedef Shape<32, 2, 1, 1, 1, 16, 4, true> Cfg11;
typedef Shape<32, 1, 1, 1, 1, 16, 4, true> Cfg12;
typedef Shape<32, 2, 2, 1, 1, 32, 2, true> Cfg13;
typedef Shape<32, 2, 1, 1, 1, 32, 2, true> Cfg14;
typedef Shape<32, 2, 2, 1, 1, 64, 2, true> Cfg15;
typedef Shape<32, 2, 1, 1, 1, 64, 2, true> Cfg16;
constexpr int N_CFG = 17;
static const int CFG_BM[N_CFG] = {Cfg0::BM, Cfg1::BM, Cfg2::BM, Cfg3::BM, Cfg4::BM, Cfg5::BM, Cfg6::BM, Cfg7::BM, Cfg8::BM, Cfg9::BM, Cfg10::BM, Cfg11::BM, Cfg12::BM, Cfg13::BM, Cfg14::BM, Cfg15::BM, Cfg16::BM};
static const int CFG_BN[N_CFG] = {Cfg0::BN, Cfg1::BN, Cfg2::BN, Cfg3::BN, Cfg4::BN, Cfg5::BN, Cfg6::BN, Cfg7::BN, Cfg8::BN, Cfg9::BN, Cfg10::BN, Cfg11::BN, Cfg12::BN, Cfg13::BN, Cfg14::BN, Cfg15::BN, Cfg16::BN};
static const int CFG_BK[N_CFG] = {Cfg0::BK, Cfg1::BK, Cfg2::BK, Cfg3::BK, Cfg4::BK, Cfg5::BK, Cfg6::BK, Cfg7::BK, Cfg8::BK, Cfg9::BK, Cfg10::BK, Cfg11::BK, Cfg12::BK, Cfg13::BK, Cfg14::BK, Cfg15::BK, Cfg16::BK};

static int bf16_bk() {
    return 32;
}

template <bool VEC>
__global__ void __launch_bounds__(256)
gemm_f32_tt_kernel(GemmArgs g) {
    I3D_CHAIN_PRIO();
    gemm_body<Cfg6, VEC, false, true, false>(g, blockIdx.x, blockIdx.y, 0, g.K, g.C, nullptr, true);
}

template <class S, int FUSE, int BF16 = 0>
__global__ void __launch_bounds__(256)
gemm_f32_fused_kernel(GemmArgs g) {
    I3D_CHAIN_PRIO();
    int bx, by, bz;
    xcd_tile(bx, by, bz);
    gemm_body<S, true, true, true, false, FUSE, BF16>(g, bx, by, 0, g.K, g.C, nullptr, true);
}

template <class S, int FUSE>
__global__ void __launch_bounds__(256) __attribute__((amdgpu_waves_per_eu(5)))
gemm_f32_fused_o5_kernel(GemmArgs g) {
    I3D_CHAIN_PRIO();
    int bx, by, bz;
    xcd_tile(bx, by, bz);
    gemm_body<S, true, true, true, false, FUSE, false>(g, bx, by, 0, g.K, g.C, nullptr, true);
}

template <class S>
static void launch_fused(const GemmArgs& g, int fuse, hipStream_t s) {
    dim3 grid(cdiv(g.M, S::BM), cdiv(g.N, S::BN), 1), block(S::NT);
    if (g_matmul_bf16) {
        switch (fuse) {
            case 1: hipLaunchKernelGGL((gemm_f32_fused_kernel<S, 1, true>), grid, block, 0, s, g); break;
            case 2: hipLaunchKernelGGL((gemm_f32_fused_kernel<S, 2, true>), grid, block, 0, s, g); break;
            default: hipLaunchKernelGGL((gemm_f32_fused_kernel<S, 3, true>), grid, block, 0, s, g); break;
        }
        return;
    }
    if constexpr (split_shape<S>()) {
        if (g_fp32_split) {
            switch (fuse) {
                case 1: hipLaunchKernelGGL((gemm_f32_fused_kernel<S, 1, 2>), grid, block, 0, s, g); break;
                case 2: hipLaunchKernelGGL((gemm_f32_fused_kernel<S, 2, 2>), grid, block, 0, s, g); break;
                default: hipLaunchKernelGGL((gemm_f32_fused_kernel<S, 3, 2>), grid, block, 0, s, g); break;
            }
            return;
        }
    }
    constexpr bool occ5 = true;
    if constexpr (S::WAVES_N == 2 && S::BK == 16) {
        if (occ5) {
            switch (fuse) {
                case 1: hipLaunchKernelGGL((gemm_f32_fused_o5_kernel<S, 1>), grid, block, 0, s, g); break;
                case 2: hipLaunchKernelGGL((gemm_f32_fused_o5_kernel<S, 2>), grid, block, 0, s, g); break;
                default: hipLaunchKernelGGL((gemm_f32_fused_o5_kernel<S, 3>), grid, block, 0, s, g); break;
            }
            return;
        }
    }
    switch (fuse) {
        case 1: hipLaunchKernelGGL((gemm_f32_fused_kernel<S, 1>), grid, block, 0, s, g); break;
        case 2: hipLaunchKernelGGL((gemm_f32_fused_kernel<S, 2>), grid, block, 0, s, g); break;
        default: hipLaunchKernelGGL((gemm_f32_fused_kernel<S, 3>), grid, block, 0, s, g); break;
    }
}

struct Extra {
    const int* m_rows = nullptr;
    const int* k_rows = nullptr;
    const int* tile_group = nullptr;
    long b_group_stride = 0;
    long a_rows_total = -1;
    long k_rows_total = -1;
    int n_groups = 0;
    const int* group_start = nullptr;
    const int* group_count = nullptr;
    long c_group_stride = 0;
    void* workspace = nullptr;
    long workspace_bytes = 0;
    int b_split = 0x7fffffff, c_split = 0x7fffffff;
    long b_delta = 0, c_delta = 0, b_view_floats = 0;
    const float* post_aff = nullptr;
    const float* post_row = nullptr;
    int n_batch = 1;
    long a_batch = 0, b_batch = 0, c_batch = 0;
};

static int fill_views(GemmArgs& g, int trans_a, int trans_b, int M, int N, int K, int lda, int ldb, const Extra& ex) {
    long a_rows = trans_a ? K : M, a_cols = trans_a ? M : K, b_rows = trans_b ? N : K, b_cols = trans_b ? K : N;
    if (!trans_a && ex.m_rows) a_rows = ex.a_rows_total;
    if (trans_a && ex.k_rows) a_rows = ex.k_rows_total;
    if (!trans_b && ex.k_rows) b_rows = ex.k_rows_total;
    const long ab = a_rows > 0 ? ((a_rows - 1) * lda + a_cols) * 4 : 0, bb = b_rows > 0 ? ((b_rows - 1) * ldb + b_cols) * 4 : 0;
    I3D_CHECK_ARG(ab < (1L << 32) - 16 && bb < (1L << 32) - 16, "operand view larger than 4 GiB (32-bit buffer offsets)");
    g.a_bytes = (unsigned)ab;
    g.b_bytes = (unsigned)bb;
    return I3D_OK;
}

static int gemm_impl(int trans_a, int trans_b, int M, int N, int K, const float* A, int lda, const float* B, int ldb,
                     float* C, int ldc, const float* bias, int accumulate, int force_cfg, int force_splits,
                     const Extra& ex, void* stream) {
    I3D_CHECK_ARG(M >= 0 && N >= 0 && K >= 0, "negative dimension");
    I3D_CHECK_ARG(lda >= (trans_a ? M : K) && ldb >= (trans_b ? K : N) && ldc >= N, "leading dimension too small");
    if (M == 0 || N == 0) return I3D_OK;
    hipStream_t s = (hipStream_t)stream;
    GemmArgs g = {};
    g.A = A; g.B = B; g.C = C; g.bias = bias;
    g.M = M; g.N = N; g.K = K;
    g.lda = lda; g.ldb = ldb; g.ldc = ldc;
    g.accumulate = accumulate ? 1 : 0;
    g.m_rows = ex.m_rows; g.k_rows = nullptr; g.tile_group = ex.tile_group; g.b_group_stride = ex.b_group_stride;
    g.slab = nullptr;
    g.a_aff = nullptr; g.stats = nullptr; g.epi_act = I3D_ACT_NONE; g.Cin = nullptr; g.ldcin = 0; g.c_bf16 = 0;
    g.b_split = ex.b_split; g.b_delta = ex.b_delta; g.c_split = ex.c_split; g.c_delta = ex.c_delta;
    int rc = fill_views(g, trans_a, trans_b, M, N, K, lda, ldb, ex);
    if (rc != I3D_OK) return rc;
    if (ex.b_view_floats > 0) {
        I3D_CHECK_ARG(ex.b_view_floats * 4 < (1L << 32) - 16, "operand view larger than 4 GiB (32-bit buffer offsets)");
        g.b_bytes = (unsigned)(ex.b_view_floats * 4);
    }
    const bool a_al = (((uintptr_t)A & 15) == 0) && (lda % 4 == 0), b_al = (((uintptr_t)B & 15) == 0) && (ldb % 4 == 0);
    g.c_vec = (((uintptr_t)C & 15) == 0) && (ldc % 4 == 0);
    const int nb = ex.n_batch > 1 ? ex.n_batch : 1;
    const bool vec = a_al && b_al && ((trans_a ? M : K) % 4 == 0) && ((trans_b ? K : N) % 4 == 0) &&
                     (ex.b_group_stride % 4 == 0) && (ex.b_delta % 4 == 0) && (nb == 1 || (ex.a_batch % 4 == 0 && ex.b_batch % 4 == 0));
    if (ex.c_delta % 4 != 0 || (nb > 1 && ex.c_batch % 4 != 0)) g.c_vec = 0;
    const int layout = trans_a ? (trans_b ? 3 : 2) : (trans_b ? 0 : 1);
    if (nb > 1) {
        I3D_CHECK_ARG(nb <= 32 && layout != 3 && (trans_a == 0 || (ex.m_rows == nullptr && ex.tile_group == nullptr)) &&
                          ex.b_split == 0x7fffffff && ex.c_split == 0x7fffffff && bias == nullptr && ex.post_aff == nullptr,
                      "batched product: plain (or row-grouped forward / data-gradient) operands, at most 32 batches");
        g.n_batch = nb; g.a_batch = ex.a_batch; g.b_batch = ex.b_batch; g.c_batch = ex.c_batch;
    }

    if (layout == 3) {
        I3D_CHECK_ARG(ex.m_rows == nullptr && ex.tile_group == nullptr, "row indirection needs a k-contiguous A");
        g.k_per_split = K; g.atomic_out = 0;
        dim3 grid(cdiv(M, Cfg6::BM), cdiv(N, Cfg6::BN), 1);
        if (vec) hipLaunchKernelGGL((gemm_f32_tt_kernel<true>), grid, dim3(256), 0, s, g);
        else hipLaunchKernelGGL((gemm_f32_tt_kernel<false>), grid, dim3(256), 0, s, g);
        I3D_CHECK_LAUNCH();
        return I3D_OK;
    }

    int cfg;
    const long tiles64 = (long)cdiv(M, 64) * cdiv(N, 64) * nb;
    const bool have_ws = ex.workspace != nullptr && (((uintptr_t)ex.workspace & 15) == 0) && ex.m_rows == nullptr;
    if (trans_a && M <= 32 && N <= 32) cfg = 8;
    else if (trans_a && have_ws && tiles64 <= 16) cfg = 8;
    else if (N <= 32) cfg = (nb > 1 && !trans_a && trans_b) ? 11 : 1;
    else if (trans_a && tiles64 < 512) cfg = 3;
    else cfg = 2;
    if (ex.tile_group != nullptr) cfg = 2;
    if (cfg == 2 && (!trans_a || trans_b)) cfg = 9;
    if (cfg == 9 && !trans_a && narrow_pays(N, tiles64)) cfg = 11;
    const long tiles32 = (long)cdiv(M, 32) * cdiv(N, 32) * nb;
    constexpr bool small_tiles = true;
    if (small_tiles && ex.tile_group == nullptr && N > 32 && tiles32 <= 1024 && (!trans_a || K < 2048)) cfg = 8;
    if (g_matmul_bf16 && vec && (cfg == 9 || cfg == 11) && bf16_bk() != 16)
        cfg = (cfg == 9 ? 13 : 14) + (bf16_bk() == 64 ? 2 : 0);
    if (force_cfg >= 0) {
        I3D_CHECK_ARG(force_cfg < N_CFG, "tile_cfg out of range");
        I3D_CHECK_ARG(ex.tile_group == nullptr || CFG_BM[force_cfg] == 64, "grouped GEMM needs 64-row tiles");
        cfg = force_cfg;
    }
    const int bm = CFG_BM[cfg], bn = CFG_BN[cfg], BK = CFG_BK[cfg];
    int tiles = cdiv(M, bm) * cdiv(N, bn) * nb;
    int splits = 1;
    if (trans_a && have_ws && tiles < 800 && K >= 2048) {
        const int target = K >= 65536 ? 3072 : (K >= 32768 ? 1600 : 800);
        splits = (target + tiles / 2) / tiles;
        int max_splits = K / 1024;
        if (splits > max_splits) splits = max_splits;
        if (splits < 1) splits = 1;
    } else if (trans_a && tiles < 512 && K >= 1024) {
        splits = (512 + tiles - 1) / tiles;
        int max_splits = K / 512;
        if (splits > max_splits) splits = max_splits;
        if (splits < 1) splits = 1;
    }
    if (force_splits > 0) splits = force_splits;
    int kps = cdiv(cdiv(K, splits), BK) * BK;
    if (kps < BK) kps = BK;
    splits = K > 0 ? cdiv(K, kps) : 1;
    g.k_per_split = kps;
    g.atomic_out = splits > 1;
    const bool use_slab = splits > 1 && ex.workspace != nullptr && (long)splits * nb * M * N * 4 <= ex.workspace_bytes &&
                          (((uintptr_t)ex.workspace & 15) == 0) && ex.m_rows == nullptr;
    g.z_splits = splits;
    I3D_CHECK_ARG(nb == 1 || splits == 1 || use_slab, "batched product with K-slices needs the scratch");
    if (use_slab) {
        g.slab = (float*)ex.workspace;
        g.atomic_out = 0;
    }
    if (splits > 1 && !accumulate && !use_slab) {
        const int m1 = std::min(M, ex.c_split);
        hipError_t e = hipMemset2DAsync(C, (size_t)ldc * sizeof(float), 0, (size_t)N * sizeof(float), m1, s);
        if (e == hipSuccess && M > m1)
            e = hipMemset2DAsync(C + (long)m1 * ldc + ex.c_delta, (size_t)ldc * sizeof(float), 0, (size_t)N * sizeof(float), M - m1, s);
        if (e != hipSuccess) {
            set_error("i3d_gemm_f32: memset failed");
            return I3D_ERR_LAUNCH;
        }
    }
    switch (cfg) {
        case 0: launch<Cfg0>(g, layout, splits, vec, s); break;
        case 1: launch<Cfg1>(g, layout, splits, vec, s); break;
        case 2: launch<Cfg2>(g, layout, splits, vec, s); break;
        case 3: launch<Cfg3>(g, layout, splits, vec, s); break;
        case 4: launch<Cfg4>(g, layout, splits, vec, s); break;
        case 5: launch<Cfg5>(g, layout, splits, vec, s); break;
        case 6: launch<Cfg6>(g, layout, splits, vec, s); break;
        case 7: launch<Cfg7>(g, layout, splits, vec, s); break;
        case 8: launch<Cfg8>(g, layout, splits, vec, s); break;
        case 9: launch<Cfg9>(g, layout, splits, vec, s); break;
        case 10: launch<Cfg10>(g, layout, splits, vec, s); break;
// ... 133 lines not shown

}

using namespace i3d;

extern "C" int i3d_set_matmul_precision(int bf16) {
    I3D_CHECK_ARG(bf16 == 0 || bf16 == 1, "0: fp32 MFMA, 1: bf16 MFMA on bf16-rounded operands");
    g_matmul_bf16 = bf16;
    return I3D_OK;
}

extern "C" int i3d_get_matmul_precision(void) { return g_matmul_bf16; }

extern "C" int i3d_set_fp32_products(int split) {
    I3D_CHECK_ARG(split == 0 || split == 1, "0: fp32 MFMA, 1: three-part bf16 split of both operands, six part products");
    g_fp32_split = split;
    return I3D_OK;
}

extern "C" int i3d_get_fp32_products(void) { return g_fp32_split; }

extern "C" int i3d_gemm_f32(int trans_a, int trans_b, int M, int N, int K, const float* A, int lda, const float* B,
                            int ldb, float* C, int ldc, const float* bias, int accumulate, void* stream) {
    return gemm_impl(trans_a, trans_b, M, N, K, A, lda, B, ldb, C, ldc, bias, accumulate, -1, 0, Extra(), stream);
}

extern "C" int i3d_gemm_f32_ex(int trans_a, int trans_b, int M, int N, int K, const float* A, int lda, const float* B,
                               int ldb, float* C, int ldc, const float* bias, int accumulate, int tile_cfg,
                               int splits, void* workspace, long workspace_bytes, void* stream) {
    Extra ex;
    ex.workspace = workspace; ex.workspace_bytes = workspace_bytes;
    return gemm_impl(trans_a, trans_b, M, N, K, A, lda, B, ldb, C, ldc, bias, accumulate, tile_cfg, splits, ex, stream);
}

extern "C" int i3d_gemm_f32_ws(int trans_a, int trans_b, int M, int N, int K, const float* A, int lda, const float* B,
                               int ldb, float* C, int ldc, const float* bias, int accumulate, void* workspace,
                               long workspace_bytes, void* stream) {
    Extra ex;
    ex.workspace = workspace; ex.workspace_bytes = workspace_bytes;
    return gemm_impl(trans_a, trans_b, M, N, K, A, lda, B, ldb, C, ldc, bias, accumulate, -1, 0, ex, stream);
}

extern "C" int i3d_gemm_f32_blocks(int trans_a, int trans_b, int M, int N, int K, const float* A, int lda, const float* B,
                                   int ldb, int b_split, long b_delta, long b_view_floats, float* C, int ldc, int c_split,
                                   long c_delta, int accumulate, void* workspace, long workspace_bytes, void* stream) {
    Extra ex;
    ex.workspace = workspace; ex.workspace_bytes = workspace_bytes;
    if (b_split > 0) { ex.b_split = b_split; ex.b_delta = b_delta; ex.b_view_floats = b_view_floats; }
    if (c_split > 0) { ex.c_split = c_split; ex.c_delta = c_delta; }
    I3D_CHECK_ARG(!(trans_a && trans_b), "layout not supported");
    return gemm_impl(trans_a, trans_b, M, N, K, A, lda, B, ldb, C, ldc, nullptr, accumulate, -1, 0, ex, stream);
}

extern "C" int i3d_gemm_f32_batched(int trans_a, int trans_b, int M, int N, int K, const float* A, int lda, long a_batch,
                                    const float* B, int ldb, long b_batch, float* C, int ldc, long c_batch, int n_batch,
                                    int accumulate, void* workspace, long workspace_bytes, void* stream) {
    I3D_CHECK_ARG(n_batch >= 1 && !(trans_a && trans_b), "n_batch >= 1, layout not supported");
    Extra ex;
    ex.workspace = workspace; ex.workspace_bytes = workspace_bytes;
    ex.n_batch = n_batch; ex.a_batch = a_batch; ex.b_batch = b_batch; ex.c_batch = c_batch;
    return gemm_impl(trans_a, trans_b, M, N, K, A, lda, B, ldb, C, ldc, nullptr, accumulate, -1, 0, ex, stream);
}

extern "C" int i3d_gemm_f32_grouped_batched(int trans_b, int m_padded, int N, int K, const float* A, int lda, long a_batch,
                                            long a_rows_total, const int* m_rows, const int* tile_group, const float* B, int ldb,
                                            long b_group_stride, long b_batch, float* C, int ldc, long c_batch, int n_batch,
                                            int accumulate, void* stream) {
    I3D_CHECK_ARG(m_rows != nullptr && tile_group != nullptr && m_padded % 64 == 0 && n_batch >= 1, "grouped GEMM needs 64-padded m_rows");
    Extra ex;
    ex.m_rows = m_rows; ex.tile_group = tile_group; ex.b_group_stride = b_group_stride; ex.a_rows_total = a_rows_total;
    ex.n_batch = n_batch; ex.a_batch = a_batch; ex.b_batch = b_batch; ex.c_batch = c_batch;
    return gemm_impl(0, trans_b, m_padded, N, K, A, lda, B, ldb, C, ldc, nullptr, accumulate, -1, 0, ex, stream);
}

extern "C" int i3d_gemm_f32_grouped(int trans_b, int m_padded, int N, int K, const float* A, int lda, long a_rows_total,
                                    const int* m_rows, const int* tile_group, const float* B, int ldb,
                                    long b_group_stride, float* C, int ldc, int accumulate, void* stream) {
    I3D_CHECK_ARG(m_rows != nullptr && tile_group != nullptr && m_padded % 64 == 0, "grouped GEMM needs 64-padded m_rows");
    Extra ex;
    ex.m_rows = m_rows; ex.tile_group = tile_group; ex.b_group_stride = b_group_stride; ex.a_rows_total = a_rows_total;
    return gemm_impl(0, trans_b, m_padded, N, K, A, lda, B, ldb, C, ldc, nullptr, accumulate, -1, 0, ex, stream);
}

extern "C" int i3d_gemm_f32_rowsubset(int M, int N, int n_rows, const float* A, int lda, const float* B, int ldb,
                                      const int* k_rows, long rows_total, float* C, int ldc, int accumulate,
                                      void* stream) {
    I3D_CHECK_ARG(k_rows != nullptr && n_rows >= 0, "k_rows required");
    const int start = 0;
    Extra ex;
    ex.k_rows = k_rows; ex.k_rows_total = rows_total;
    ex.n_groups = 1; ex.group_start = &start; ex.group_count = &n_rows; ex.c_group_stride = 0;
    return rowseg_impl(M, N, A, lda, B, ldb, C, ldc, accumulate, -1, 0, ex, stream);
}

extern "C" int i3d_gemm_f32_rowsubset_multi(int M, int N, int n_groups, const int* group_start, const int* group_count,
                                            const float* A, int lda, const float* B, int ldb, const int* k_rows,
                                            long rows_total, float* C, long c_group_stride, int ldc, int accumulate,
                                            int tile_cfg, int seg_rows, void* workspace, long workspace_bytes,
                                            void* stream) {
    I3D_CHECK_ARG(k_rows != nullptr && group_start != nullptr && group_count != nullptr && n_groups > 0, "bad arguments");
    Extra ex;
    ex.workspace = workspace; ex.workspace_bytes = workspace_bytes;
    ex.k_rows = k_rows; ex.k_rows_total = rows_total;
    ex.n_groups = n_groups; ex.group_start = group_start; ex.group_count = group_count; ex.c_group_stride = c_group_stride;
    return rowseg_impl(M, N, A, lda, B, ldb, C, ldc, accumulate, tile_cfg, seg_rows, ex, stream);
}

extern "C" int i3d_gemm_f32_fused(int M, int N, int K, const float* A, int lda, long a_rows_total, const float* W, int ldb,
                                  float* C, int ldc, const float* bias, int accumulate, const float* a_aff, int epi_act,
                                  float* stats, const int* m_rows, const int* tile_group, long b_group_stride,
                                  void* stream) {
    return i3d_gemm_f32_fused_src(M, N, K, A, lda, a_rows_total, W, ldb, C, ldc, nullptr, 0, bias, accumulate, a_aff, epi_act, stats,
                                  m_rows, tile_group, b_group_stride, stream);
}

static thread_local int g_fused_c_bf16 = 0;
extern "C" int i3d_gemm_f32_fused_bf16out(int M, int N, int K, const float* A, int lda, long a_rows_total, const float* W, int ldb,
                                          void* C, int ldc, const float* bias, const float* a_aff, int epi_act, float* stats,
                                          void* stream) {
    I3D_CHECK_ARG(stats != nullptr && N % 4 == 0 && ldc % 4 == 0 && (((uintptr_t)C) & 15) == 0, "bf16 output: statistics variant, N and ldc multiples of 4");
    g_fused_c_bf16 = 1;
    const int rc = i3d_gemm_f32_fused_src(M, N, K, A, lda, a_rows_total, W, ldb, (float*)C, ldc, nullptr, 0, bias, 0, a_aff, epi_act, stats,
                                          nullptr, nullptr, 0, stream);
    g_fused_c_bf16 = 0;
    return rc;
}

extern "C" int i3d_gemm_f32_fused_src(int M, int N, int K, const float* A, int lda, long a_rows_total, const float* W, int ldb,
                                      float* C, int ldc, const float* c_in, int ldcin, const float* bias, int accumulate,
                                      const float* a_aff, int epi_act, float* stats, const int* m_rows, const int* tile_group,
                                      long b_group_stride, void* stream) {
    I3D_CHECK_ARG(c_in == nullptr || (stats != nullptr && accumulate && ldcin >= N && ldcin % 4 == 0 && (((uintptr_t)c_in) & 15) == 0),
                  "c_in needs the statistics variant with accumulate, a pitch >= N that is a multiple of 4, 16-byte alignment");
    I3D_CHECK_ARG(M > 0 && N > 0 && K > 0, "empty GEMM");
    I3D_CHECK_ARG(a_aff != nullptr || stats != nullptr, "nothing to fuse: use i3d_gemm_f32");
    I3D_CHECK_ARG(lda >= K && ldb >= K && ldc >= N, "leading dimension too small");
    I3D_CHECK_ARG(a_aff == nullptr || K <= FUSE_MAX_K, "BatchNorm prologue: K <= 1024");
    I3D_CHECK_ARG((m_rows == nullptr) == (tile_group == nullptr), "grouped GEMM needs m_rows and tile_group");
    I3D_CHECK_ARG(m_rows == nullptr || M % 64 == 0, "grouped GEMM needs 64-padded m_rows");
    I3D_CHECK_ARG(relu_class(epi_act), "epilogue activation: none, ReLU or LeakyReLU (the others: a pass of their own)");
    const bool al = ((((uintptr_t)A | (uintptr_t)W | (uintptr_t)C) & 15) == 0) && lda % 4 == 0 && ldb % 4 == 0 && ldc % 4 == 0 &&
                    K % 4 == 0 && b_group_stride % 4 == 0;
    I3D_CHECK_ARG(al, "fused GEMM needs 16-byte aligned operands and K, leading dimensions multiples of 4");
    GemmArgs g = {};
    g.A = A; g.B = W; g.C = C; g.bias = bias;
    g.M = M; g.N = N; g.K = K;
    g.lda = lda; g.ldb = ldb; g.ldc = ldc;
    g.accumulate = accumulate ? 1 : 0;
    g.k_per_split = K; g.atomic_out = 0; g.c_vec = 1;
    g.m_rows = m_rows; g.k_rows = nullptr; g.tile_group = tile_group; g.b_group_stride = b_group_stride;
    g.b_split = g.c_split = 0x7fffffff; g.b_delta = g.c_delta = 0;
    g.slab = nullptr;
    g.a_aff = a_aff; g.stats = stats; g.epi_act = epi_act; g.Cin = c_in; g.ldcin = ldcin; g.c_bf16 = g_fused_c_bf16;
    Extra ex;
    ex.m_rows = m_rows; ex.a_rows_total = a_rows_total;
    int rc = fill_views(g, 0, 1, M, N, K, lda, ldb, ex);
    if (rc != I3D_OK) return rc;
    const int fuse = (a_aff != nullptr ? 1 : 0) | (stats != nullptr ? 2 : 0);
    hipStream_t s = (hipStream_t)stream;
    const bool narrow = narrow_pays(N, (long)cdiv(M, 64) * cdiv(N, 64)) && K >= 400;
    if (g_matmul_bf16 && bf16_bk() == 32) {
        if (narrow) launch_fused<Cfg14>(g, fuse, s);
        else launch_fused<Cfg13>(g, fuse, s);
    } else if (g_matmul_bf16 && bf16_bk() == 64) {
        if (narrow) launch_fused<Cfg16>(g, fuse, s);
        else launch_fused<Cfg15>(g, fuse, s);
    } else if (narrow) launch_fused<Cfg11>(g, fuse, s);
    else launch_fused<Cfg9>(g, fuse, s);
    I3D_CHECK_LAUNCH();
    return I3D_OK;
}

extern "C" int i3d_gemm_f32_wgrad_bn(int f_out, int f_in, int rows, const float* dY, int ldy, const float* x, int ldx,
                                     float* dW, int ldw, const float* grad_bias, const float* aff, void* workspace,
                                     long workspace_bytes, void* stream) {
    I3D_CHECK_ARG(grad_bias != nullptr && aff != nullptr, "grad_bias and aff required");
    Extra ex;
    ex.workspace = workspace; ex.workspace_bytes = workspace_bytes;
    ex.post_aff = aff; ex.post_row = grad_bias;
    return gemm_impl(1, 0, f_out, f_in, rows, dY, ldy, x, ldx, dW, ldw, nullptr, 0, -1, 0, ex, stream);
}
```

### 3dinfomax_amd/csrc/grouped.hip

```cpp
#include "common.h"

namespace i3d {

constexpr int MAX_GROUPS = 32, MAX_SCALERS = 4;
struct Coef {
    float c[MAX_GROUPS][MAX_SCALERS];
};

template <int S>
__global__ void __launch_bounds__(256)
combine_weights_fwd_kernel(const float4* __restrict__ W, int ldw4, int f_in4, int f_out, int A4, int n_groups, Coef coef,
                           float4* __restrict__ WD) {
    I3D_CHAIN_PRIO();
    long t = (long)blockIdx.x * blockDim.x + threadIdx.x;
    long per = (long)f_out * A4;
    if (t >= per) return;
    int n = (int)(t / A4), k = (int)(t - (long)n * A4);
    float4 w[S];
#pragma unroll
    for (int s = 0; s < S; ++s) w[s] = W[(long)n * ldw4 + f_in4 + (long)s * A4 + k];
    for (int g = 0; g < n_groups; ++g) {
        float4 o = make_float4(0.f, 0.f, 0.f, 0.f);
#pragma unroll
        for (int s = 0; s < S; ++s) {
            const float c = coef.c[g][s];
            o.x += c * w[s].x; o.y += c * w[s].y; o.z += c * w[s].z; o.w += c * w[s].w;
        }
        WD[(long)g * per + t] = o;
    }
}

template <int S>
__global__ void __launch_bounds__(256)
combine_weights_bwd_kernel(const float4* __restrict__ dWD, int ldw4, int f_in4, int f_out, int A4, int n_groups, Coef coef,
                           float4* __restrict__ dW) {
    I3D_CHAIN_PRIO();
    long t = (long)blockIdx.x * blockDim.x + threadIdx.x;
    long per = (long)f_out * A4;
    if (t >= per) return;
    int n = (int)(t / A4), k = (int)(t - (long)n * A4);
    float4 acc[S];
#pragma unroll
    for (int s = 0; s < S; ++s) acc[s] = make_float4(0.f, 0.f, 0.f, 0.f);
    for (int g = 0; g < n_groups; ++g) {
        const float4 d = dWD[(long)g * per + t];
#pragma unroll
        for (int s = 0; s < S; ++s) {
            const float c = coef.c[g][s];
            acc[s].x += c * d.x; acc[s].y += c * d.y; acc[s].z += c * d.z; acc[s].w += c * d.w;
        }
    }
#pragma unroll
    for (int s = 0; s < S; ++s) dW[(long)n * ldw4 + f_in4 + (long)s * A4 + k] = acc[s];
}

__global__ void __launch_bounds__(256)
pack_h_weights_kernel(const float4* __restrict__ We, int ldwe4, int Fo, const float4* __restrict__ Wp, int ldwp4, int Fp,
                      const float* __restrict__ bias_p, int Fh4, float4* __restrict__ Wcat, float* __restrict__ bcat) {
    I3D_CHAIN_PRIO();
    const long t = (long)blockIdx.x * blockDim.x + threadIdx.x;
    const int rows = 2 * Fo + Fp;
    if (t < rows) bcat[t] = t < 2 * Fo ? 0.f : (bias_p != nullptr ? bias_p[t - 2 * Fo] : 0.f);
    if (t >= (long)rows * Fh4) return;
    const int r = (int)(t / Fh4), k = (int)(t - (long)r * Fh4);
    float4 v;
    if (r < Fo) v = We[(long)r * ldwe4 + k];
    else if (r < 2 * Fo) v = We[(long)(r - Fo) * ldwe4 + Fh4 + k];
    else v = Wp[(long)(r - 2 * Fo) * ldwp4 + k];
    Wcat[t] = v;
}

#define I3D_COMBINE_LAUNCH(KERNEL, ...)                                                                         \
    switch (n_scalers) {                                                                                        \
        case 1: hipLaunchKernelGGL(KERNEL<1>, dim3(cdiv(items, 256)), dim3(256), 0, (hipStream_t)stream, __VA_ARGS__); break; \
        case 2: hipLaunchKernelGGL(KERNEL<2>, dim3(cdiv(items, 256)), dim3(256), 0, (hipStream_t)stream, __VA_ARGS__); break; \
        case 3: hipLaunchKernelGGL(KERNEL<3>, dim3(cdiv(items, 256)), dim3(256), 0, (hipStream_t)stream, __VA_ARGS__); break; \
        default: hipLaunchKernelGGL(KERNEL<4>, dim3(cdiv(items, 256)), dim3(256), 0, (hipStream_t)stream, __VA_ARGS__); break; \
    }

static int fill_coef(const float* coef_host, int n_groups, int n_scalers, Coef& c) {
    if (n_groups < 1 || n_groups > MAX_GROUPS || n_scalers < 1 || n_scalers > MAX_SCALERS) return -1;
    for (int g = 0; g < n_groups; ++g)
        for (int s = 0; s < n_scalers; ++s) c.c[g][s] = coef_host[g * n_scalers + s];
    return 0;
}

}

using namespace i3d;

extern "C" int i3d_pna_combine_weights_fwd(const float* W, int ldw, int f_in, int f_out, int agg_width, int n_groups,
                                           int n_scalers, const float* coef, float* WD, void* stream) {
    I3D_CHECK_ARG(f_in % 4 == 0 && agg_width % 4 == 0 && ldw % 4 == 0, "dimensions must be multiples of 4");
    I3D_CHECK_ARG((((uintptr_t)W | (uintptr_t)WD) & 15) == 0, "16-byte aligned pointers required");
    Coef c;
    I3D_CHECK_ARG(fill_coef(coef, n_groups, n_scalers, c) == 0, "1..32 groups and 1..4 scalers supported");
    long items = (long)f_out * (agg_width / 4);
    I3D_COMBINE_LAUNCH(combine_weights_fwd_kernel, (const float4*)W, ldw / 4, f_in / 4, f_out, agg_width / 4, n_groups, c,
                       (float4*)WD);
    I3D_CHECK_LAUNCH();
    return I3D_OK;
}

extern "C" int i3d_pna_combine_weights_bwd(const float* dWD, int ldw, int f_in, int f_out, int agg_width, int n_groups,
                                           int n_scalers, const float* coef, float* dW, void* stream) {
    I3D_CHECK_ARG(f_in % 4 == 0 && agg_width % 4 == 0 && ldw % 4 == 0, "dimensions must be multiples of 4");
    I3D_CHECK_ARG((((uintptr_t)dW | (uintptr_t)dWD) & 15) == 0, "16-byte aligned pointers required");
    Coef c;
    I3D_CHECK_ARG(fill_coef(coef, n_groups, n_scalers, c) == 0, "1..32 groups and 1..4 scalers supported");
    long items = (long)f_out * (agg_width / 4);
    I3D_COMBINE_LAUNCH(combine_weights_bwd_kernel, (const float4*)dWD, ldw / 4, f_in / 4, f_out, agg_width / 4, n_groups, c,
                       (float4*)dW);
    I3D_CHECK_LAUNCH();
    return I3D_OK;
}

extern "C" int i3d_pna_pack_h_weights(const float* W_edge, int ldw_edge, int f_out_edge, const float* W_post, int ldw_post,
                                      int f_out_post, const float* bias_post, int f_h, float* Wcat, float* bcat, void* stream) {
    I3D_CHECK_ARG(W_edge != nullptr && W_post != nullptr && Wcat != nullptr && bcat != nullptr, "null");
    I3D_CHECK_ARG(f_h % 4 == 0 && ldw_edge % 4 == 0 && ldw_post % 4 == 0 && ldw_edge >= 2 * f_h && ldw_post >= f_h,
                  "dimensions must be multiples of 4");
    I3D_CHECK_ARG((((uintptr_t)W_edge | (uintptr_t)W_post | (uintptr_t)Wcat) & 15) == 0, "16-byte aligned pointers required");
    const long items = (long)(2 * f_out_edge + f_out_post) * (f_h / 4);
    hipLaunchKernelGGL(pack_h_weights_kernel, dim3(cdiv(items, 256)), dim3(256), 0, (hipStream_t)stream, (const float4*)W_edge,
                       ldw_edge / 4, f_out_edge, (const float4*)W_post, ldw_post / 4, f_out_post, bias_post, f_h / 4, (float4*)Wcat,
                       bcat);
    I3D_CHECK_LAUNCH();
    return I3D_OK;
}
```

### 3dinfomax_amd/csrc/model.hip

```cpp
#include "common.h"


#include <algorithm>
#include <cmath>
#include <cstdlib>
#include <cstring>
#include <new>
#include <vector>

using namespace i3d;

#define TRY(call)                 \
    do {                          \
        int rc_ = (call);         \
        if (rc_ != I3D_OK) return rc_; \
    } while (0)

namespace {

inline long al4(long n) { return (n + 3) & ~3L; }

struct Bump {
    float* base;
    long used = 0;
// ... 123 lines not shown
    I3D_CHECK_ARG(b->n_groups >= 1 && b->n_groups <= 32 && b->n_groups * m->n_scalers <= 128 && b->m_padded % 64 == 0,
                  "bad degree groups");
    I3D_CHECK_ARG(b->n_comb >= 1 && b->v_pad >= b->n_comb && b->v_pad % 4 == 0, "bad bond table");
    for (int l = 0; l < m->n_layers; ++l) {
        for (int i = 0; i < m->n_pre; ++i) {
            const I3dFcParams& p = m->pre[l][i];
            I3D_CHECK_ARG(p.gamma != nullptr && simple_act(p.act) && p.f_out % 4 == 0 && p.f_in % 4 == 0 && p.f_in <= 3 * 1024,
                          "pretrans block: BatchNorm, activation none / ReLU / LeakyReLU, widths multiples of 4");
        }
        const I3dFcParams& p = m->post[l];
        I3D_CHECK_ARG(p.gamma != nullptr && simple_act(p.act) && p.f_out == m->hidden, "posttrans block");
    }
    return I3D_OK;
}

long plan_forward(PnaCtx& c, float* saved, float* node_emb, float* out) {
    const I3dPnaModel& m = c.m;
    const I3dPnaBatch& b = c.b;
    const int N = b.num_nodes, E = b.num_edges, B = b.num_graphs, F = m.hidden, L = m.n_layers;
    Bump ar(saved);
    c.h.assign(L + 1, nullptr);
    c.h[0] = ar.take((long)N * F);
    c.bond_table = ar.take((long)b.n_comb * F);
    c.codes = reinterpret_cast<int*>(ar.take(E));
    c.onehot = ar.take((long)E * b.v_pad);
    c.n_scalers_cfg = m.n_scalers;
    for (int g = 0; g < b.n_groups; ++g)
        for (int s = 0; s < m.n_scalers; ++s) c.coef[g * m.n_scalers + s] = scaler_coef(m.scalers[s], b.group_degree[g], m.avg_d_log);
    int f_max = F;
    for (int l = 0; l < L; ++l)
        for (int i = 0; i < m.n_pre; ++i) f_max = std::max(f_max, m.pre[l][i].f_out);
    float* stats_ws = ar.take(i3d_pna_layer_stats_floats(N, E, b.m_padded, f_max));
    c.layers.assign(L, I3dPnaLayerArgs());
    for (int l = 0; l < L; ++l) {
        I3dPnaLayerArgs& a = c.layers[l];
        std::memset(&a, 0, sizeof(a));
        a.fused_bn = 1;
        a.merge_h = 1;
        a.stats_ws = stats_ws;
        c.h[l + 1] = (l == L - 1) ? node_emb : ar.take((long)N * F);
        I3dEdgeFcArgs& e = a.edge;
        const I3dFcParams& p0 = m.pre[l][0];
        const int Fo0 = p0.f_out;
        fill_tail(e.tail, p0, ar.take(Fo0), ar.take(Fo0));
        e.num_nodes = N; e.num_edges = E; e.f_h = F; e.f_q = F; e.f_out = Fo0; e.ldw = p0.f_in;
        e.q_rows = b.n_comb; e.v_pad = b.v_pad; e.q_code = c.codes; e.onehot = c.onehot;
        e.h = c.h[l]; e.q = c.bond_table; e.W = p0.W; e.bias = p0.bias;
        e.src_s = b.src_s; e.dst_s = b.dst_s; e.in_ptr = b.in_ptr; e.out_ptr = b.out_ptr; e.out_epos = b.out_epos;
        e.Q = ar.take((long)b.n_comb * Fo0);
        e.P = ar.take((long)N * 2 * Fo0);
        a.Wcat = ar.take((long)(2 * Fo0 + F) * F);
        a.bcat = ar.take(2 * Fo0 + F);
        a.PL = ar.take((long)N * (2 * Fo0 + F));
        a.Wcat_panel = ar.take(i3d_panel_packed_bytes(2 * Fo0 + F, F) / 4);
        a.Wcat_dgrad_panel = ar.take(i3d_panel_packed_bytes(F, 2 * Fo0 + F) / 4);
        e.xact = ar.take((long)E * Fo0);
        a.aff[0] = ar.take(3L * Fo0);
        const float* x = e.xact;
        int f_in = Fo0;
        a.n_pre_extra = m.n_pre - 1;
        for (int i = 1; i < m.n_pre; ++i) {
            const I3dFcParams& p = m.pre[l][i];
            I3dFcArgs& fc = a.pre[i - 1];
            fill_tail(fc.tail, p, ar.take(p.f_out), ar.take(p.f_out));
            fc.rows = E; fc.f_in = f_in; fc.f_out = p.f_out; fc.ldw = p.f_in;
            fc.x = x; fc.W = p.W; fc.bias = p.bias;
            fc.xact = ar.take((long)E * p.f_out);
            fc.W_dgrad_panel = ar.take(i3d_panel_packed_bytes(f_in, p.f_out) / 4);
            fc.W_fwd_panel = ar.take(i3d_panel_packed_bytes(p.f_out, f_in) / 4);
            a.aff[i] = ar.take(3L * p.f_out);
            x = fc.xact;
            f_in = p.f_out;
        }
        a.n_aggregators = m.n_aggregators;
        for (int i = 0; i < m.n_aggregators; ++i) a.aggregators[i] = m.aggregators[i];
        a.n_scalers = 1; a.scalers[0] = I3D_SCALE_IDENTITY; a.force_scalers = 0; a.avg_d_log = m.avg_d_log;
        a.msg = x;
        const int A = m.n_aggregators * f_in;
        I3dGroupedFcArgs& g = a.post;
        const I3dFcParams& pp = m.post[l];
        fill_tail(g.tail, pp, ar.take(F), ar.take(F));
        g.num_nodes = N; g.f_h = F; g.f_out = F; g.agg_width = A; g.ldw = pp.f_in;
        g.n_groups = b.n_groups; g.n_scalers = m.n_scalers; g.m_padded = b.m_padded;
        for (int k = 0; k < b.n_groups; ++k) { g.group_start[k] = b.group_start[k]; g.group_count[k] = b.group_count[k]; }
        for (int k = 0; k < b.n_groups * m.n_scalers; ++k) g.coef[k] = c.coef[k];
        g.h = c.h[l]; g.W = pp.W; g.bias = pp.bias;
        g.agg = ar.take((long)N * A);
        g.deg_rows = b.deg_rows; g.deg_tile_group = b.deg_tile_group;
        g.WD = ar.take((long)b.n_groups * F * A);
        g.xact = ar.take((long)N * F);
        g.y = c.h[l + 1];
        a.n_post_extra = 0;
        a.residual = m.residual ? 1 : 0;
        g.residual = m.residual ? c.h[l] : nullptr;
    }
    c.readout = ar.take((long)B * m.n_readout * F);
    c.head.assign(m.n_head, HeadSaved());
    c.head_args.assign(m.n_head, I3dFcArgs());
    const float* x = c.readout;
    for (int i = 0; i < m.n_head; ++i) {
        const I3dFcParams& p = m.head[i];
        I3dFcArgs& fc = c.head_args[i];
        std::memset(&fc, 0, sizeof(fc));
        const bool last = i == m.n_head - 1;
        float* y = last ? out : ar.take((long)B * p.f_out);
        fc.rows = B; fc.f_in = p.f_in; fc.f_out = p.f_out; fc.ldw = p.f_in;
        fc.x = x; fc.W = p.W; fc.bias = p.bias; fc.y = y;
        if (p.gamma != nullptr) {
            c.head[i].mean = ar.take(p.f_out);
            c.head[i].invstd = ar.take(p.f_out);
            fill_tail(fc.tail, p, c.head[i].mean, c.head[i].invstd);
            fc.xact = ar.take((long)B * p.f_out);
            if (!simple_act(p.act)) fc.pre_keep = ar.take((long)B * p.f_out);
        } else if (p.act != I3D_ACT_NONE) {
            fc.xact = ar.take((long)B * p.f_out);
        }
        c.head[i].xact = fc.xact;
        c.head[i].y = y;
        x = y;
    }
    c.out = out;
    {
        long oa = 0, ob = 0;
        for (int k = 0; k < m.n_atom_tables; ++k) oa += m.atom_dims[k];
        for (int k = 0; k < m.n_bond_tables; ++k) ob += m.bond_dims[k];
        c.hot_atoms = ar.take((long)N * ((oa + 31) / 32 * 32));
        c.hot_bonds = ar.take((long)b.n_comb * ((ob + 31) / 32 * 32));
    }
    c.saved_floats = ar.used;
    return ar.used;
}

}

extern "C" long i3d_pna_model_saved_floats(const I3dPnaModel* m, const I3dPnaBatch* b) {
    if (check_model(m, b) != I3D_OK) return -1;
    PnaCtx c;
    c.m = *m;
    c.b = *b;
    return plan_forward(c, nullptr, nullptr, nullptr);
}

extern "C" long i3d_pna_model_scratch_floats(const I3dPnaModel* m, const I3dPnaBatch* b) {
    if (check_model(m, b) != I3D_OK) return -1;
    const long N = b->num_nodes, E = b->num_edges, B = b->num_graphs, F = m->hidden;
    const long top = 2 * al4(N * F) + al4((long)b->n_comb * F);
    const long head = head_floats(*m, B) + head_colsum_floats(*m, B);
    long layer = 0;
    for (int l = 0; l < m->n_layers; ++l) {
        const long f_msg = m->pre[l][m->n_pre - 1].f_out, A = m->n_aggregators * f_msg, Fo0 = m->pre[l][0].f_out;
        long t = al4(N * F) + al4((long)b->n_groups * F * A) + al4(N * A) + al4(E * f_msg);
        for (int i = 1; i < m->n_pre; ++i)
            t += al4(E * (long)m->pre[l][i].f_out) + al4(E * (long)m->pre[l][i].f_in);
        t += al4(E * Fo0) + al4(N * 2 * Fo0) + al4(N * F) + al4((long)b->v_pad * Fo0) + al4(i3d_bn_bias_partial_floats(Fo0));
        t += al4(N * (2 * Fo0 + F));
        layer = std::max(layer, t);
    }
    long oa = 0, ob = 0;
    for (int k = 0; k < m->n_atom_tables; ++k) oa += m->atom_dims[k];
    for (int k = 0; k < m->n_bond_tables; ++k) ob += m->bond_dims[k];
    const long emb = al4(N * ((oa + 31) / 32 * 32)) + al4((long)b->n_comb * ((ob + 31) / 32 * 32)) + al4(((oa + 3) / 4 * 4) * F);
    long side = 0;
    for (int l = 0; l < m->n_layers; ++l) side += side_floats(*m, *b, l);
    return top + side + head + std::max(layer, emb);
}

extern "C" int i3d_pna_model_fwd(const I3dPnaModel* m, const I3dPnaBatch* b, float* saved, float* node_emb, float* edge_emb,
// ... 277 lines not shown
```

### 3dinfomax_amd/layer_native.py

```python
import ctypes

import torch

from . import _lib, ops, tape
from . import layers as _layers
from .layers import _keeps_pre, _set_workspaces

_SIMPLE_ACTS = (None, 'relu', 'leakyrelu')
KEEP_LAST_ARGS = None


def fused_bn_ok(plan, params, n_pre, n_post):
    if n_post != 1:
        return False
    for spec in plan.pre_specs + plan.post_specs[:1]:
        if spec.act not in _SIMPLE_ACTS:
            return False
    for spec in plan.pre_specs:
        if spec.post_act is not None:
            return False
    for i in range(1, n_pre):
        if params[4 * i].shape[1] > 1024:
            return False
    return True
# ... 82 lines not shown
    total += _al(N * A) + _al(nG * Fp0 * A)
    merged = fused and n_post == 1 and Fp0 % 4 == 0
    WL = 2 * Fo0 + Fp0
    if merged:
        total += _al(WL * Fh) + _al(WL) + _al(N * WL)
        total += _al(L.i3d_panel_packed_bytes(WL, Fh) // 4) + _al(L.i3d_panel_packed_bytes(Fh, WL) // 4)
        f_prev = Fo0
        for i in range(1, n_pre):
            total += _al(L.i3d_panel_packed_bytes(f_prev, pre_p[i][0].shape[0]) // 4)
            total += _al(L.i3d_panel_packed_bytes(pre_p[i][0].shape[0], f_prev) // 4)
            f_prev = pre_p[i][0].shape[0]
    for i, spec in enumerate(plan.post_specs):
        Fo = post_p[i][0].shape[0]
        total += _al(N * Fo) * (2 + (1 if _keeps_pre(spec) else 0)) + 2 * _al(Fo)
    ar = _Arena(total, dev)
    Fout = post_p[-1][0].shape[0]
    y_out = torch.empty(N, Fout, dtype=torch.float32, device=dev)

    a = _lib.PnaLayerArgs()
    if fused:
        a.fused_bn = 1
        a.stats_ws = ar.take(n_stats)
    e = a.edge
    W, b, ga, be = pre_p[0]
    spec = plan.pre_specs[0]
    _tail(e.tail, spec, ga, be, ar.take(Fo0), ar.take(Fo0), Fo0, dev)
    e.num_nodes, e.num_edges, e.f_h, e.f_q, e.f_out, e.ldw = N, E, Fh, Fq, Fo0, W.stride(0)
    e.h, e.W, e.bias = h.data_ptr(), W.data_ptr(), b.data_ptr()
    if q is not None:
        e.q = q.data_ptr()
        if q_rows:
            e.q_rows, e.v_pad, e.q_code, e.onehot = q_rows, qmap.v_pad, qmap.codes.data_ptr(), qmap.onehot.data_ptr()
        e.Q = ar.take((q_rows or E) * Fo0)
    e.src_s, e.dst_s, e.in_ptr = index.src_s.data_ptr(), index.dst_s.data_ptr(), index.in_ptr.data_ptr()
    e.out_ptr, e.out_epos = index.out_ptr.data_ptr(), index.out_epos.data_ptr()
    e.P = ar.take(N * 2 * Fo0)
    if merged:
        a.merge_h = 1
        a.Wcat, a.bcat, a.PL = ar.take(WL * Fh), ar.take(WL), ar.take(N * WL)
        a.Wcat_panel = ar.take(L.i3d_panel_packed_bytes(WL, Fh) // 4)
        a.Wcat_dgrad_panel = ar.take(L.i3d_panel_packed_bytes(Fh, WL) // 4)
    e.xact = ar.take(E * Fo0)
    if _keeps_pre(spec):
        e.pre_keep = ar.take(E * Fo0)
    if fused:
        a.aff[0] = ar.take(3 * Fo0)
        x_ptr, f_in = e.xact, Fo0
    else:
        e.y = ar.take(E * Fo0)
        x_ptr, f_in = e.y, Fo0
    a.n_pre_extra = n_pre - 1
    for i in range(1, n_pre):
        W, b, ga, be = pre_p[i]
        spec = plan.pre_specs[i]
        Fo = W.shape[0]
        c = a.pre[i - 1]
        _tail(c.tail, spec, ga, be, ar.take(Fo), ar.take(Fo), Fo, dev)
        c.rows, c.f_in, c.f_out, c.ldw = E, f_in, Fo, W.stride(0)
        c.x, c.W, c.bias = x_ptr, W.data_ptr(), b.data_ptr()
        c.xact = ar.take(E * Fo)
        if merged:
            c.W_dgrad_panel = ar.take(L.i3d_panel_packed_bytes(f_in, Fo) // 4)
            c.W_fwd_panel = ar.take(L.i3d_panel_packed_bytes(Fo, f_in) // 4)
        if _keeps_pre(spec):
            c.pre_keep = ar.take(E * Fo)
        if fused:
            a.aff[i] = ar.take(3 * Fo)
            x_ptr, f_in = c.xact, Fo
        else:
            c.y = ar.take(E * Fo)
            x_ptr, f_in = c.y, Fo
    a.n_aggregators, a.n_scalers, a.force_scalers, a.avg_d_log = len(plan.aggregators), len(plan.agg_scalers), 0, plan.avg
    for i, v in enumerate(plan.aggregators):
        a.aggregators[i] = v
    for i, v in enumerate(plan.agg_scalers):
        a.scalers[i] = v
    a.msg = x_ptr
    p = a.post
    W, b, ga, be = post_p[0]
    spec = plan.post_specs[0]
    _tail(p.tail, spec, ga, be, ar.take(Fp0), ar.take(Fp0), Fp0, dev)
    p.num_nodes, p.f_h, p.f_out, p.agg_width, p.ldw = N, Fh, Fp0, A, W.stride(0)
    p.n_groups, p.n_scalers, p.m_padded = nG, nS, rows_d.shape[0]
    for gi, (_, start, count) in enumerate(groups):
        p.group_start[gi], p.group_count[gi] = start, count
    k = 0
    for g_ in plan.coef:
        for v in g_:
            p.coef[k] = v
            k += 1
    p.h, p.W, p.bias = h.data_ptr(), W.data_ptr(), b.data_ptr()
    p.agg = ar.take(N * A)
    p.deg_rows, p.deg_tile_group = rows_d.data_ptr(), tiles_d.data_ptr()
    p.WD = ar.take(nG * Fp0 * A)
    p.xact = ar.take(N * Fp0)
    if _keeps_pre(spec):
        p.pre_keep = ar.take(N * Fp0)
    a.n_post_extra = n_post - 1
    a.residual = 1 if plan.residual else 0
    if n_post == 1:
        p.y = y_out.data_ptr()
        if plan.residual:
            p.residual = h.data_ptr()
    else:
        p.y = ar.take(N * Fp0)
    x_ptr, f_in = p.y, Fp0
    for i in range(1, n_post):
        W, b, ga, be = post_p[i]
        spec = plan.post_specs[i]
        Fo = W.shape[0]
        c = a.postx[i - 1]
        _tail(c.tail, spec, ga, be, ar.take(Fo), ar.take(Fo), Fo, dev)
        c.rows, c.f_in, c.f_out, c.ldw = N, f_in, Fo, W.stride(0)
        c.x, c.W, c.bias = x_ptr, W.data_ptr(), b.data_ptr()
        c.xact = ar.take(N * Fo)
        if _keeps_pre(spec):
            c.pre_keep = ar.take(N * Fo)
        last = i == n_post - 1
        c.y = y_out.data_ptr() if last else ar.take(N * Fo)
        if last and plan.residual:
            c.residual = h.data_ptr()
        x_ptr, f_in = c.y, Fo
    if ops.KERNEL_TIMERS is not None:
        t0, t1 = ops.RawEvent(), ops.RawEvent()
        a.agg_event_start, a.agg_event_stop = t0.handle, t1.handle
        ops.KERNEL_TIMERS.setdefault('pna_aggregate_fwd', []).append(
            (t0, t1, N, E, Fmsg, len(plan.aggregators) * len(plan.agg_scalers) * Fmsg))
    _lib.check(L.i3d_pna_layer_fwd(ctypes.byref(a), ops._stream()), 'i3d_pna_layer_fwd')
    a.agg_event_start = a.agg_event_stop = None
    ctx.native = (a, ar, h, q, qmap, index, plan, params, (N, E, Fh, Fq, A, nG))
    if KEEP_LAST_ARGS is not None:
        KEEP_LAST_ARGS.append((a, ctx.native))
    return y_out


def backward(ctx, grad):
    a, ar_fwd, h, q, qmap, index, plan, params, (N, E, Fh, Fq, A, nG) = ctx.native
    dev = h.device
    grad = grad.contiguous()
    n_pre, n_post = len(plan.pre_specs), len(plan.post_specs)
    dims_pre = [params[4 * i].shape for i in range(n_pre)]
    dims_post = [params[4 * (n_pre + i)].shape for i in range(n_post)]
    Fo0, Fmsg, Fp0 = dims_pre[0][0], dims_pre[-1][0], dims_post[0][0]
    need_q = q is not None and ctx.needs_input_grad[1]
    total = 0
    for (Fo, Fi) in dims_post[1:]:
        total += _al(N * Fo) + _al(N * Fi)
    total += _al(N * Fp0) + _al(nG * Fp0 * A) + _al(N * A) + _al(E * Fmsg)
    for (Fo, Fi) in dims_pre[1:]:
        total += _al(E * Fo) + _al(E * Fi)
    total += _al(E * Fo0) + _al(N * 2 * Fo0) + _al(N * Fh) + (_al(qmap.v_pad * Fo0) if (qmap is not None and q is not None) else 0)
    if a.merge_h:
        total += _al(N * (2 * Fo0 + Fp0)) + _al(_lib.load().i3d_bn_bias_partial_floats(Fo0))
    ar = _Arena(total, dev)
    grads = []

    def param_grads(k):
        return tuple(tape.grad_like(params[4 * k + j]) for j in range(4))

    def set_param_grads(c, g4):
        c.grad_W, c.grad_bias, c.grad_gamma, c.grad_beta = (t.data_ptr() for t in g4)

    a.grad_out = grad.data_ptr()
    gy = grad.data_ptr()
    post_g = [None] * n_post
    for i in range(n_post - 1, 0, -1):
        c = a.postx[i - 1]
        Fo, Fi = dims_post[i]
# ... 44 lines not shown
```

### include/infomax3d_hip.h

```cpp
#ifndef INFOMAX3D_HIP_H
#define INFOMAX3D_HIP_H

#include <stdint.h>

#ifdef __cplusplus
extern "C" {
#endif

#define I3D_OK 0
#define I3D_ERR_INVALID (-1)
#define I3D_ERR_LAUNCH (-2)
#define I3D_NOT_TAKEN 1

#define I3D_ACT_NONE 0
#define I3D_ACT_RELU 1
#define I3D_ACT_SILU 2
#define I3D_ACT_SIGMOID 3
#define I3D_ACT_LEAKY_RELU 4
#define I3D_ACT_TANH 5
#define I3D_ACT_ELU 6
#define I3D_ACT_SELU 7
#define I3D_ACT_SOFTPLUS 8

#define I3D_AGG_MEAN 0
#define I3D_AGG_SUM 1
#define I3D_AGG_MAX 2
#define I3D_AGG_MIN 3
#define I3D_AGG_STD 4
#define I3D_AGG_VAR 5

#define I3D_SCALE_IDENTITY 0
#define I3D_SCALE_AMPLIFICATION 1
#define I3D_SCALE_ATTENUATION 2

int i3d_abi_version(void);
const char* i3d_last_error(void);

int i3d_embedding_sum_fwd(const int64_t* idx, const int* row_perm, int rows, int n_cols, const float* const* tables,
                          int feat, float* out, void* stream);
int i3d_embedding_sum_bwd(const int64_t* idx, const int* row_perm, int rows, int n_cols, const float* grad_out,
                          int feat, float* const* grad_tables, const int* dims, void* stream);

int i3d_pna_aggregate_fwd(const float* e, const int* in_ptr, int num_nodes, int feat, const int* aggregators,
                          int n_aggregators, const int* scalers, int n_scalers, int force_scalers, float avg_d_log,
                          float* out, void* stream);
int i3d_pna_aggregate_bwd(const float* grad_out, const float* e, const int* in_ptr, int num_nodes, int feat,
                          const int* aggregators, int n_aggregators, const int* scalers, int n_scalers,
                          int force_scalers, float avg_d_log, float* grad_e, void* stream);

int i3d_segment_readout_fwd(const float* x, const int* graph_ptr, int num_graphs, int feat, const int* ops,
                            int n_ops, float* out, void* stream);
int i3d_segment_readout_bwd(const float* grad_out, const float* x, const int* graph_ptr, int num_graphs, int feat,
                            const int* ops, int n_ops, float* grad_x, void* stream);

int i3d_gemm_f32(int trans_a, int trans_b, int M, int N, int K, const float* A, int lda, const float* B, int ldb,
                 float* C, int ldc, const float* bias, int accumulate, void* stream);
int i3d_gemm_f32_ex(int trans_a, int trans_b, int M, int N, int K, const float* A, int lda, const float* B, int ldb,
                    float* C, int ldc, const float* bias, int accumulate, int tile_cfg, int splits, void* workspace,
                    long workspace_bytes, void* stream);
int i3d_set_matmul_precision(int bf16);
int i3d_get_matmul_precision(void);
int i3d_set_fp32_products(int split);
int i3d_get_fp32_products(void);

long i3d_panel_packed_bytes(int N, int K);
int i3d_panel_pack(const float* W, int ldw, int N, int K, int trans, void* packed, void* stream);
typedef struct {
    const float* W;
    int ldw, N, K, trans;
    void* packed;
} I3dPanelPack;
int i3d_panel_pack_multi(const I3dPanelPack* weights, int n, void* stream);
int i3d_panel_gemm(int M, int N, int K, const float* A, int lda, const void* packed, float* C, int ldc, const float* bias,
                   int accumulate, void* stream);
int i3d_panel_stats_tiles(int M);
int i3d_panel_gemm_fused(int M, int N, int K, const float* A, int lda, const void* packed, float* C, int ldc, const float* bias,
                         const float* a_aff, int epi_act, float* stats, void* stream);

int i3d_gemm_f32_ws(int trans_a, int trans_b, int M, int N, int K, const float* A, int lda, const float* B, int ldb,
                    float* C, int ldc, const float* bias, int accumulate, void* workspace, long workspace_bytes,
                    void* stream);

int i3d_gemm_f32_blocks(int trans_a, int trans_b, int M, int N, int K, const float* A, int lda, const float* B, int ldb,
                        int b_split, long b_delta, long b_view_floats, float* C, int ldc, int c_split, long c_delta,
                        int accumulate, void* workspace, long workspace_bytes, void* stream);

int i3d_pna_aggregate_fwd_towers(const float* e, const int* in_ptr, int num_nodes, int feat, int tower_feat,
                                 const int* aggregators, int n_aggregators, const int* scalers, int n_scalers,
                                 int force_scalers, float avg_d_log, float* out, void* stream);
int i3d_pna_aggregate_bwd_towers(const float* grad_out, const float* e, const int* in_ptr, int num_nodes, int feat,
                                 int tower_feat, const int* aggregators, int n_aggregators, const int* scalers,
                                 int n_scalers, int force_scalers, float avg_d_log, float* grad_e, void* stream);
int i3d_gemm_f32_batched(int trans_a, int trans_b, int M, int N, int K, const float* A, int lda, long a_batch, const float* B,
                         int ldb, long b_batch, float* C, int ldc, long c_batch, int n_batch, int accumulate, void* workspace,
                         long workspace_bytes, void* stream);

int i3d_gemm_f32_grouped_batched(int trans_b, int m_padded, int N, int K, const float* A, int lda, long a_batch, long a_rows_total,
                                 const int* m_rows, const int* tile_group, const float* B, int ldb, long b_group_stride, long b_batch,
                                 float* C, int ldc, long c_batch, int n_batch, int accumulate, void* stream);

int i3d_pna_combine_weights_fwd(const float* W, int ldw, int f_in, int f_out, int agg_width, int n_groups,
                                int n_scalers, const float* coef, float* WD, void* stream);
int i3d_pna_combine_weights_bwd(const float* dWD, int ldw, int f_in, int f_out, int agg_width, int n_groups,
                                int n_scalers, const float* coef, float* dW, void* stream);
int i3d_gemm_f32_grouped(int trans_b, int m_padded, int N, int K, const float* A, int lda, long a_rows_total,
                         const int* m_rows, const int* tile_group, const float* B, int ldb, long b_group_stride,
                         float* C, int ldc, int accumulate, void* stream);
int i3d_gemm_f32_rowsubset(int M, int N, int n_rows, const float* A, int lda, const float* B, int ldb,
                           const int* k_rows, long rows_total, float* C, int ldc, int accumulate, void* stream);
int i3d_gemm_f32_rowsubset_multi(int M, int N, int n_groups, const int* group_start, const int* group_count,
                                 const float* A, int lda, const float* B, int ldb, const int* k_rows, long rows_total,
                                 float* C, long c_group_stride, int ldc, int accumulate, int tile_cfg, int seg_rows,
                                 void* workspace, long workspace_bytes, void* stream);

long i3d_colreduce_workspace_bytes(int rows, int feat);
int i3d_act_stats_fwd(const float* pre, int rows, int feat, int act, float* x, float eps, float momentum,
                      float* mean, float* invstd, float* running_mean, float* running_var, double* sums_out,
                      void* workspace, void* stream);
int i3d_act_stats_fwd_counted(const float* pre, int rows, int feat, int act, float* x, float eps, float momentum,
                      float* mean, float* invstd, float* running_mean, float* running_var, double* sums_out, long long* num_batches_tracked,
                      void* workspace, void* stream);
int i3d_bn_finalize_stats(const double* sums, int feat, float eps, float momentum, float* mean, float* invstd,
                          float* running_mean, float* running_var, void* stream);
int i3d_bn_apply_fwd(const float* x, int rows, int feat, const float* mean, const float* invstd,
                     const float* gamma, const float* beta, int post_act, const float* residual, float* y,
                     void* stream);
int i3d_bn_eval_fwd(const float* x, int rows, int feat, const float* running_mean, const float* running_var,
                    float eps, const float* gamma, const float* beta, int post_act, const float* residual, float* y,
                    void* stream);
int i3d_bn_bwd(const float* grad_y, const float* x, const float* pre, int rows, int feat, int act, int post_act,
               const float* mean, const float* invstd, const float* gamma, const float* beta, float* grad_gamma,
               float* grad_beta, float* grad_pre, float* grad_bias, double* sums_out, const double* sums_in,
               long total_rows, void* workspace, void* stream);
int i3d_bn_eval_bwd(const float* grad_y, const float* x, const float* pre, int rows, int feat, int act,
                    int post_act, const float* running_mean, const float* running_var, float eps,
                    const float* gamma, const float* beta, float* grad_gamma, float* grad_beta, float* grad_pre,
                    void* workspace, void* stream);
int i3d_colsum(const float* x, const float* w, int rows, int feat, float* out, void* workspace, void* stream);
int i3d_act_fwd(const float* x, long n, int act, float* y, void* stream);
int i3d_act_bwd(const float* grad_y, const float* x, long n, int act, float* grad_x, void* stream);
int i3d_gru_gates_fwd(const float* GI, const float* GH, const float* h0, int rows, int hidden, float* out, float* saved, void* stream);
int i3d_gru_gates_bwd(const float* grad_out, const float* saved, const float* GH, const float* h0, int rows, int hidden, float* grad_GI,
                      float* grad_GH, float* grad_h0, void* stream);
int i3d_add_inplace(float* dst, const float* src, long n, void* stream);
int i3d_add(const float* a, const float* b, long n, float* out, void* stream);
int i3d_mul(const float* a, const float* b, long n, float* out, void* stream);
int i3d_broadcast_row(const float* row, long rows, int feat, float* out, void* stream);

int i3d_edge_combine_fwd(const float* P, int ldp, const float* Q, const int* q_code, const float* bias,
                         const int* src_s, const int* dst_s, int num_edges, int feat, float* pre, void* stream);
int i3d_multihot(const int64_t* idx, const int* row_perm, int rows, int n_cols, const int* offsets, int v_pad, float* out,
                 void* stream);
int i3d_edge_codes(const int64_t* idx, const int* row_perm, int rows, int n_cols, const int* strides, int v_pad,
                   int* codes, float* onehot, void* stream);
int i3d_segment_sum(const float* x, int ldx, const int* ptr, const int* idx, int num_segments, int feat,
                    int scale_mode, float* out, int ldo, void* stream);
int i3d_segment_sum_bf16(const void* x, int ldx, const int* ptr, const int* idx, int num_segments, int feat, int scale_mode,
                         float* out, int ldo, void* stream);
int i3d_segment_sum_pair(const float* x, int ldx, const int* ptr0, const int* idx0, float* out0, const int* ptr1,
                         const int* idx1, float* out1, int num_segments, int feat, int ldo, void* stream);
int i3d_segment_bcast(const float* g, const int* ptr, const int* seg_of_row, int rows, int feat, int scale_mode,
                      float* out, void* stream);
int i3d_gather_rows(const float* x, const int* idx, int rows, int feat, float* out, void* stream);

int i3d_fourier_encode(const float* d, int num_edges, int n_enc, float* out, void* stream);
int i3d_soft_edge_fwd(const float* m, const float* ws, const float* bs, int num_edges, int feat, float* msg,
                      float* w, void* stream);
int i3d_soft_edge_bwd(const float* grad_msg, const float* m, const float* w, const float* ws, int num_edges,
                      int feat, float* grad_m, float* g_gate, void* stream);

int i3d_row_norms(const float* z, int rows, int dim, float* norms, void* stream);
int i3d_ntxent_fwd(const float* sim, const float* n1, const float* n2, int b1, int b2, int conf, int pos_offset,
                   float tau, float eps, float loss_scale, float* row_sum, float* row_pos, float* loss_sum, void* stream);
int i3d_ntxent_bwd(const float* sim, const float* n1, const float* n2, const float* row_sum, const float* row_pos,
                   int b1, int b2, int conf, int pos_offset, float tau, float eps, float grad_scale,
                   const float* grad_scale_dev, float* dsim, float* ca, float* cb, void* stream);
long i3d_ntxent_loss_scratch_floats(int b1, int b2c);
int i3d_ntxent_loss_fwd(const float* z1, const float* z2, int b1, int b2, int conf, int dim, int pos_offset, float tau,
                        float eps, float loss_scale, float* scratch, float* loss, void* stream);
int i3d_ntxent_loss_bwd(const float* z1, const float* z2, int b1, int b2, int conf, int dim, int pos_offset, float tau,
                        float eps, float loss_scale, const float* scratch, const float* grad_scale_dev, float* work, float* dz1,
                        float* dz2, void* stream);
int i3d_row_axpy(const float* z, const float* coef, int rows, int dim, float* out, void* stream);
int i3d_row_scale(const float* z, const float* coef, int rows, int dim, float* out, void* stream);
typedef struct {
    const float* src;
    float* dst;
    int rows, cols;
    long ld_src, ld_dst;
} I3dCopyBlock;
int i3d_block_copy(const I3dCopyBlock* table , int n_blocks, int reverse, void* stream);
int i3d_copy_cols(const float* src, int rows, int cols_src, float* dst, int cols_dst, void* stream);
int i3d_edge_sqdist(const float* x, const int* src, const int* dst, int num_edges, float* out, int ld, int col, int take_sqrt,
                    void* stream);

typedef struct {
    int num_nodes, num_edges, f_in, f_edge, f_msg, f_out, f_mix, ldp, ldq, ldgp, ldgq;
    int n_aggregators, n_scalers, residual, training, grad_e_accumulate;
    int aggregators[8], scalers[4];
    float avg_d_log, eps, momentum;
    const float* h;
    const float* e;
    const float* snorm;
    const float* Wp;
    const float* bp;
    const float* Wq;
    const float* bq;
    const float* gamma;
    const float* beta;
    float* running_mean;
    float* running_var;
    const float* Wm;
    const float* bm;
    const int* src_s;
    const int* dst_s;
    const int* in_ptr;
    const int* out_ptr;
    const int* out_epos;
    float* saved;
    float* scratch;
    void* workspace;
    void* gemm_workspace;
    long gemm_workspace_bytes;
    float* out;
    const float* grad_out;
    float* grad_h;
    float* grad_e;
    float* grad_Wp;
    float* grad_bp;
    float* grad_Wq;
    float* grad_bq;
    float* grad_gamma;
    float* grad_beta;
    float* grad_Wm;
    float* grad_bm;
    int n_towers;
    int n_deg_groups, m_padded;
    int group_start[32];
    int group_count[32];
    float coef[128];
    const int* deg_rows;
    const int* deg_tile_group;
} I3dTowerLayerArgs;
long i3d_tower_layer_saved_floats(const I3dTowerLayerArgs* a);
long i3d_tower_layer_scratch_floats(const I3dTowerLayerArgs* a);
int i3d_tower_layer_fwd(const I3dTowerLayerArgs* a, void* stream);
int i3d_tower_layer_bwd(const I3dTowerLayerArgs* a, void* stream);

int i3d_bn_finalize_partials(const float* partial, int n_tiles, int feat, float eps, float momentum, const float* gamma,
                             const float* beta, float* mean, float* invstd, float* running_mean, float* running_var,
                             long long* num_batches_tracked, float* aff, void* stream);
int i3d_edge_stats_rows_per_tile(int feat);
int i3d_edge_combine_act_stats(const float* P, int ldp, const float* Q, const int* q_code, const float* bias,
                               const int* src_s, const int* dst_s, int num_edges, int feat, int act, float* x,
                               float* partial, void* stream);
int i3d_gemm_f32_fused(int M, int N, int K, const float* A, int lda, long a_rows_total, const float* W, int ldb, float* C,
                       int ldc, const float* bias, int accumulate, const float* a_aff, int epi_act, float* stats,
                       const int* m_rows, const int* tile_group, long b_group_stride, void* stream);
int i3d_gemm_f32_fused_src(int M, int N, int K, const float* A, int lda, long a_rows_total, const float* W, int ldb, float* C,
                           int ldc, const float* c_in, int ldcin, const float* bias, int accumulate, const float* a_aff,
                           int epi_act, float* stats, const int* m_rows, const int* tile_group, long b_group_stride,
                           void* stream);
int i3d_gemm_f32_fused_bf16out(int M, int N, int K, const float* A, int lda, long a_rows_total, const float* W, int ldb, void* C, int ldc,
                               const float* bias, const float* a_aff, int epi_act, float* stats, void* stream);
int i3d_pna_pack_h_weights(const float* W_edge, int ldw_edge, int f_out_edge, const float* W_post, int ldw_post, int f_out_post,
                           const float* bias_post, int f_h, float* Wcat, float* bcat, void* stream);
int i3d_bn_bwd_strided(const float* grad_y, const float* x, const float* pre, int rows, int feat, int act, int post_act,
                       const float* mean, const float* invstd, const float* gamma, const float* beta, float* grad_gamma,
                       float* grad_beta, float* grad_pre, int ld_out, float* grad_bias, void* workspace, void* stream);
int i3d_bn_bwd_x_bf16(const float* grad_y, const void* x, int rows, int feat, int act, int post_act, const float* mean,
                      const float* invstd, const float* gamma, const float* beta, float* grad_gamma, float* grad_beta, float* grad_pre,
                      float* grad_bias, void* workspace, void* stream);
int i3d_gemm_f32_wgrad_bn(int f_out, int f_in, int rows, const float* dY, int ldy, const float* x, int ldx, float* dW,
                          int ldw, const float* grad_bias, const float* aff, void* workspace, long workspace_bytes,
                          void* stream);
typedef struct {
    int world;
    int (*all_gather_f32)(void* user, const float* send, float* recv, long count, void* stream);
    int (*all_reduce_f64)(void* user, double* buf, long count, void* stream);
    void* user;
    void* scratch;
    long scratch_bytes;
} I3dCollectives;
int i3d_set_collectives(const I3dCollectives* c );
int i3d_collectives_world(void);
int i3d_collectives_all_gather_f32(const float* send, float* recv, long count, void* stream);
int i3d_collectives_all_reduce_f64(double* buf, long count, void* stream);
int i3d_rccl_available(void);
int i3d_rccl_unique_id(char* out128 );
int i3d_rccl_init(const char* id128 , int rank, int world, void** comm);
int i3d_rccl_destroy(void* comm);
int i3d_set_collectives_rccl(void* comm, int world, void* scratch, long scratch_bytes);
long i3d_peer_mailbox_bytes(void);
int i3d_peer_handle_bytes(void);
int i3d_peer_alloc(void** mailbox , char* handle_out );
int i3d_peer_free(void* mailbox);
int i3d_peer_open(void* mailbox, const char* handles , int rank, int world,
                  double timeout_s , void** ctx );
int i3d_set_collectives_peer(void* ctx, void* scratch, long scratch_bytes);
int i3d_peer_bind_stream(void* ctx, void* stream, void* scratch, long scratch_bytes);
int i3d_peer_status(void* ctx);
long long i3d_peer_sequence(void* ctx);
int i3d_peer_close(void* ctx);

#define I3D_WGRAD_PLAIN 0
#define I3D_WGRAD_BN 1
#define I3D_WGRAD_COMBINE 2
typedef struct {
    const float* A;
    const float* B;
    const int* rows;
    long rows_total;
    int lda, ldb, M, N;
    int k_begin, k_count;
} I3dWgradProblem;
typedef struct {
    int kind, n_groups, first_problem;
    int ldc, c_split, n_scalers;
    long c_delta, scaler_stride;
    float* C;
    const float* aff;
    const float* row;
    const float* coef;
} I3dWgradOutput;
int i3d_wgrad_multi_supported(const I3dWgradProblem* problems, int n_problems, const I3dWgradOutput* outputs, int n_outputs);
long i3d_wgrad_multi_workspace_bytes(int max_units);
long i3d_wgrad_multi_min_workspace_bytes(const I3dWgradProblem* problems, int n_problems);
int i3d_wgrad_multi(const I3dWgradProblem* problems, int n_problems, const I3dWgradOutput* outputs, int n_outputs,
                    void* workspace, long workspace_bytes, void* stream);

int i3d_pna_aggregate_fwd_aff(const float* e, const float* aff, const int* in_ptr, int num_nodes, int feat,
                              const int* aggregators, int n_aggregators, const int* scalers, int n_scalers,
                              int force_scalers, float avg_d_log, float* out, void* stream);
int i3d_pna_aggregate_bwd_aff(const float* grad_out, const float* e, const float* aff, const int* in_ptr, int num_nodes,
                              int feat, const int* aggregators, int n_aggregators, const int* scalers, int n_scalers,
                              int force_scalers, float avg_d_log, float* grad_e, void* stream);
int i3d_pna_aggregate_fwd_ex(const void* e, int e_bf16, const float* aff, const int* in_ptr, int num_nodes, int feat,
                             const int* aggregators, int n_aggregators, const int* scalers, int n_scalers, int force_scalers,
                             float avg_d_log, float* out, void* stream);
int i3d_pna_aggregate_bwd_ex(const float* grad_out, const void* e, int e_bf16, const float* aff, const int* in_ptr, int num_nodes,
                             int feat, const int* aggregators, int n_aggregators, const int* scalers, int n_scalers,
                             int force_scalers, float avg_d_log, float* grad_e, void* stream);

int i3d_set_bn_bwd_one_launch(int on);
int i3d_bn_bwd_one_launch_supported(int rows, int feat);
// ... 20 lines not shown
} I3dBnTail;

typedef struct {
    I3dBnTail tail;
    int rows, f_in, f_out, ldw;
    const float* x;
    const float* W;
    const float* bias;
    const float* residual;
    float* xact;
    float* pre_keep;
    float* y;
    const float* grad_y;
    float* grad_pre;
    float* grad_gamma;
    float* grad_beta;
    float* grad_W;
    float* grad_bias;
    float* grad_x;
    void* W_dgrad_panel;
    void* W_fwd_panel;
} I3dFcArgs;

typedef struct {
    I3dBnTail tail;
    int num_nodes, num_edges, f_h, f_q, f_out, ldw;
    int q_rows;
    int v_pad;
    const int* q_code;
    const float* onehot;
    float* grad_Q;
    const float* h;
    const float* q;
    const float* W;
    const float* bias;
    const int* src_s;
    const int* dst_s;
    const int* in_ptr;
    const int* out_ptr;
    const int* out_epos;
    float* P;
    float* Q;
    float* xact;
    float* pre_keep;
    float* y;
    const float* grad_y;
    float* grad_pre;
    float* grad_P;
    float* grad_gamma;
    float* grad_beta;
    float* grad_W;
    float* grad_bias;
    float* grad_h;
    float* grad_q;
    int grad_q_accumulate;
} I3dEdgeFcArgs;

typedef struct {
    I3dBnTail tail;
    int num_nodes, f_h, f_out, agg_width, ldw, n_groups, n_scalers, m_padded;
    int group_start[32];
    int group_count[32];
    float coef[128];
    const float* h;
    const float* agg;
    const float* W;
    const float* bias;
    const float* residual;
    const int* deg_rows;
    const int* deg_tile_group;
    float* WD;
    float* xact;
    float* pre_keep;
    float* y;
    const float* grad_y;
    float* grad_pre;
    float* grad_WD;
    float* grad_gamma;
    float* grad_beta;
    float* grad_W;
    float* grad_bias;
    float* grad_h;
    float* grad_agg;
} I3dGroupedFcArgs;

#define I3D_MAX_EXTRA_FC 3
typedef struct {
    I3dEdgeFcArgs edge;
    int n_pre_extra;
    I3dFcArgs pre[I3D_MAX_EXTRA_FC];
    int n_aggregators, n_scalers, force_scalers;
    int aggregators[8];
    int scalers[4];
    float avg_d_log;
    const float* msg;
    float* grad_msg;
    I3dGroupedFcArgs post;
    int n_post_extra;
    I3dFcArgs postx[I3D_MAX_EXTRA_FC];
    int residual;
    const float* grad_out;
    void* agg_event_start;
    void* agg_event_stop;
    int fused_bn;
    int defer_join;
    float* stats_ws;
    float* aff[I3D_MAX_EXTRA_FC + 1];
    int weights_ready;
    int merge_h;
    float* Wcat;
    float* bcat;
    float* PL;
    float* DL;
    int wgrad_split;
    int eval_mode;
    int msg_bf16;
    float* edge_bias_partial;
    void* Wcat_panel;
    void* Wcat_dgrad_panel;
} I3dPnaLayerArgs;

typedef struct {
    const float* running_mean;
    const float* running_var;
    const float* gamma;
    const float* beta;
    float* aff;
    int feat;
    float eps;
} I3dBnEvalAff;
int i3d_bn_eval_aff_multi(const I3dBnEvalAff* entries , int n, void* stream);

long i3d_pna_layer_stats_floats(int num_nodes, int num_edges, int m_padded, int f);

typedef struct {
    I3dBnTail tail_in;
    I3dBnTail tail_msg;
    int num_nodes, num_edges, hidden, n_enc, reduce_mean;
    int ld_w_in, ld_w_msg;
    const float* d_raw;
    const int* perm;
    const int* dst_s;
    const int* in_ptr;
    const float* emb;
    const float* W_in;
    const float* b_in;
    const float* W_msg;
    const float* b_msg;
    const float* w_gate;
    const float* b_gate;
    float* stats;
    float* aff_in;
    float* aff_msg;
    float* x_msg;
    float* d_out;
    float* msg;
    float* m_sum;
    const float* grad_m_sum;
    float* grad_ya;
    float* grad_lin;
    float* partial;
    float* grad_W_in;
    float* grad_b_in;
    float* grad_gamma_in;
    float* grad_beta_in;
    float* grad_W_msg;
    float* grad_b_msg;
// ... 307 lines not shown
```

Baseline: 281,100.

## Collapse PNA aggregator K-range for degree-1 node groups in post GEMMs

```diff
diff --git a/3dinfomax_amd/_lib.py b/3dinfomax_amd/_lib.py
--- a/3dinfomax_amd/_lib.py
+++ b/3dinfomax_amd/_lib.py
@@ -1,7 +1,7 @@
 import ctypes
 import os
 import re
-from ctypes import POINTER, c_char_p, c_double, c_float, c_int, c_int64, c_long, c_uint64, c_void_p
+from ctypes import POINTER, c_char_p, c_double, c_float, c_int, c_int64, c_long, c_uint, c_uint64, c_void_p
 
 HERE = os.path.dirname(os.path.abspath(__file__))
 _TESTING = os.environ.get('I3D_TESTING') == '1'
@@ -49,7 +49,7 @@
                 ('agg', _P), ('W', _P), ('bias', _P), ('residual', _P), ('deg_rows', _P), ('deg_tile_group', _P),
                 ('WD', _P), ('xact', _P), ('pre_keep', _P), ('y', _P), ('grad_y', _P), ('grad_pre', _P),
                 ('grad_WD', _P), ('grad_gamma', _P), ('grad_beta', _P), ('grad_W', _P), ('grad_bias', _P),
-                ('grad_h', _P), ('grad_agg', _P)]
+                ('grad_h', _P), ('grad_agg', _P), ('group_degree', c_int * 32)]
 
 
 class PnaLayerArgs(ctypes.Structure):
@@ -177,6 +177,8 @@
     'i3d_peer_close': (c_int, [_P]),
     'i3d_gemm_f32_fused_src': (c_int, [c_int, c_int, c_int, _P, c_int, c_long, _P, c_int, _P, c_int, _P, c_int, _P, c_int, _P, c_int,
                                        _P, _P, _P, c_long, _P]),
+    'i3d_gemm_f32_fused_src_kskip': (c_int, [c_int, c_int, c_int, _P, c_int, c_long, _P, c_int, _P, c_int, _P, c_int, _P, c_int, _P,
+                                             c_int, _P, _P, _P, c_long, c_uint, c_int, _P]),
     'i3d_pna_pack_h_weights': (c_int, [_P, c_int, c_int, _P, c_int, c_int, _P, c_int, _P, _P, _P]),
     'i3d_bn_bwd_strided': (c_int, [_P, _P, _P, c_int, c_int, c_int, c_int, _P, _P, _P, _P, _P, _P, _P, c_int, _P, _P, _P]),
     'i3d_wgrad_multi_supported': (c_int, [POINTER(WgradProblem), c_int, POINTER(WgradOutput), c_int]),
@@ -278,6 +280,12 @@
     'i3d_gemm_f32_batched': (c_int, [c_int, c_int, c_int, c_int, c_int, _P, c_int, c_long, _P, c_int, c_long, _P, c_int, c_long, c_int,
                                      c_int, _P, c_long, _P]),
     'i3d_pna_combine_weights_fwd': (c_int, [_P, c_int, c_int, c_int, c_int, c_int, c_int, POINTER(c_float), _P, _P]),
+    'i3d_pna_combine_weights_fwd_deg1': (c_int, [_P, c_int, c_int, c_int, c_int, c_int, c_int, POINTER(c_float), c_uint, _P, _P]),
+    'i3d_gemm_f32_grouped_live': (c_int, [c_int, c_int, c_int, _P, c_int, c_long, _P, _P, _P, c_int, c_long, _P, c_int, c_uint,
+                                          c_int, c_int, _P]),
+    'i3d_pna_layer_args_bytes': (c_long, []),
+    'i3d_set_deg1_collapse': (c_int, [c_int]),
+    'i3d_get_deg1_collapse': (c_int, []),
     'i3d_pna_combine_weights_bwd': (c_int, [_P, c_int, c_int, c_int, c_int, c_int, c_int, POINTER(c_float), _P, _P]),
     'i3d_gemm_f32_grouped': (c_int, [c_int, c_int, c_int, c_int, _P, c_int, c_long, _P, _P, _P, c_int, c_long, _P, c_int,
                                      c_int, _P]),
@@ -425,6 +433,9 @@
         fn = getattr(lib, name)
         fn.restype = res
         fn.argtypes = args
+    if lib.i3d_pna_layer_args_bytes() != ctypes.sizeof(PnaLayerArgs):
+        raise HipLibraryError(f'{LIB_PATH} is stale: I3dPnaLayerArgs is {lib.i3d_pna_layer_args_bytes()} bytes there, '
+                              f'{ctypes.sizeof(PnaLayerArgs)} here - rebuild it')
     prec = os.environ.get('I3D_MATMUL_PRECISION', 'fp32').lower()
     if prec not in ('fp32', 'bf16'):
         raise HipLibraryError(f'I3D_MATMUL_PRECISION={prec!r}: fp32 or bf16')
diff --git a/3dinfomax_amd/csrc/composite.hip b/3dinfomax_amd/csrc/composite.hip
--- a/3dinfomax_amd/csrc/composite.hip
+++ b/3dinfomax_amd/csrc/composite.hip
@@ -268,6 +268,34 @@
     }
     if (n > 0) TRY(i3d_panel_pack_multi(w, n, stream));
     return I3D_OK;
+}
+
+constexpr long DEG1_MIN_WORKGROUPS = 1024;
+static int g_deg1_collapse = [] {
+    const char* e = getenv("I3D_DEG1_COLLAPSE");
+    return e == nullptr ? 1 : (e[0] == '0' ? 0 : (e[0] == '2' ? 2 : 1));
+}();
+extern "C" int i3d_set_deg1_collapse(int mode) {
+    g_deg1_collapse = mode <= 0 ? 0 : (mode >= 2 ? 2 : 1);
+    return I3D_OK;
+}
+extern "C" int i3d_get_deg1_collapse(void) { return g_deg1_collapse; }
+
+static unsigned deg1_mask(const I3dPnaLayerArgs* a) {
+    const I3dGroupedFcArgs* p = &a->post;
+    if (!g_deg1_collapse || !a->fused_bn || a->n_post_extra != 0) return 0;
+    if (a->n_aggregators != 4 || a->aggregators[0] != I3D_AGG_MEAN || a->aggregators[1] != I3D_AGG_MAX ||
+        a->aggregators[2] != I3D_AGG_MIN || a->aggregators[3] != I3D_AGG_STD)
+        return 0;
+    if (a->n_scalers != 1 || (a->force_scalers && a->scalers[0] != I3D_SCALE_IDENTITY)) return 0;
+    const int f_msg = a->n_pre_extra > 0 ? a->pre[a->n_pre_extra - 1].f_out : a->edge.f_out;
+    if (f_msg <= 0 || f_msg % 4 != 0 || p->agg_width != 4 * f_msg || p->n_groups > 32) return 0;
+    if ((((uintptr_t)p->WD | (uintptr_t)p->agg | (uintptr_t)p->W) & 15) != 0 || p->ldw % 4 != 0 || p->f_h % 4 != 0) return 0;
+    if (g_deg1_collapse < 2 && (long)(p->m_padded / 64) * cdiv(p->agg_width, 64) < DEG1_MIN_WORKGROUPS) return 0;
+    unsigned mask = 0;
+    for (int g = 0; g < p->n_groups; ++g)
+        if (p->group_degree[g] == 1) mask |= 1u << g;
+    return mask;
 }
 
 static bool edge_bias_on_chain(const I3dPnaLayerArgs* a) {
@@ -437,10 +465,12 @@
     I3D_CHECK_ARG(p->pre_keep == nullptr && simple_act(p->tail.act), "fused BatchNorm: unsupported block shape");
     const int A = p->agg_width, Fp = p->f_out;
     if (!merged) TRY(i3d_gemm_f32(0, 1, N, Fp, p->f_h, p->h, p->f_h, p->W, p->ldw, p->xact, Fp, p->bias, 0, stream));
+    const unsigned deg1 = deg1_mask(a);
     if (!a->weights_ready)
-        TRY(i3d_pna_combine_weights_fwd(p->W, p->ldw, p->f_h, Fp, A, p->n_groups, p->n_scalers, p->coef, p->WD, stream));
-    TRY(i3d_gemm_f32_fused_src(p->m_padded, Fp, A, p->agg, A, N, p->WD, A, p->xact, Fp, merged ? a->PL + 2 * Fo : nullptr, WL,
-                               nullptr, 1, nullptr, p->tail.act, a->stats_ws, p->deg_rows, p->deg_tile_group, (long)Fp * A, stream));
+        TRY(i3d_pna_combine_weights_fwd_deg1(p->W, p->ldw, p->f_h, Fp, A, p->n_groups, p->n_scalers, p->coef, deg1, p->WD, stream));
+    TRY(i3d_gemm_f32_fused_src_kskip(p->m_padded, Fp, A, p->agg, A, N, p->WD, A, p->xact, Fp, merged ? a->PL + 2 * Fo : nullptr, WL,
+                                     nullptr, 1, nullptr, p->tail.act, a->stats_ws, p->deg_rows, p->deg_tile_group, (long)Fp * A,
+                                     deg1, A / 2, stream));
     if (a->eval_mode)
         return i3d_bn_eval_fwd(p->xact, N, Fp, p->tail.running_mean, p->tail.running_var, p->tail.eps, p->tail.gamma, p->tail.beta,
                                p->tail.post_act, p->residual, p->y, stream);
@@ -457,8 +487,8 @@
         TRY(i3d_gemm_f32(0, 1, e->q_rows > 0 ? e->q_rows : e->num_edges, e->f_out, e->f_q, e->q, e->f_q, e->W + 2 * e->f_h, e->ldw,
                          e->Q, e->f_out, nullptr, 0, stream));
     if (merge_h_ok(a)) TRY(pack_layer_weights(a, stream));
-    return i3d_pna_combine_weights_fwd(p->W, p->ldw, p->f_h, p->f_out, p->agg_width, p->n_groups, p->n_scalers, p->coef, p->WD,
-                                       stream);
+    return i3d_pna_combine_weights_fwd_deg1(p->W, p->ldw, p->f_h, p->f_out, p->agg_width, p->n_groups, p->n_scalers, p->coef,
+                                            deg1_mask(a), p->WD, stream);
 }
 
 extern "C" int i3d_wgrad_stream_fork(void* stream, void** side) {
@@ -514,8 +544,10 @@
         TRY(i3d_bn_bwd_strided(g->grad_y, g->xact, g->pre_keep, g->num_nodes, g->f_out, g->tail.act, g->tail.post_act, g->tail.mean,
                                g->tail.invstd, g->tail.gamma, g->tail.beta, g->grad_gamma, g->grad_beta, dlin, WLb, g->grad_bias,
                                g->tail.workspace, stream));
-        TRY(i3d_gemm_f32_grouped(0, g->m_padded, g->agg_width, g->f_out, dlin, WLb, g->num_nodes, g->deg_rows, g->deg_tile_group, g->WD,
-                                 g->agg_width, (long)g->f_out * g->agg_width, g->grad_agg, g->agg_width, 0, stream));
+        const int A = g->agg_width;
+        const bool al16 = ((((uintptr_t)dlin | (uintptr_t)g->grad_agg) & 15) == 0) && WLb % 4 == 0 && g->f_out % 4 == 0;
+        TRY(i3d_gemm_f32_grouped_live(g->m_padded, A, g->f_out, dlin, WLb, g->num_nodes, g->deg_rows, g->deg_tile_group, g->WD, A,
+                                      (long)g->f_out * A, g->grad_agg, A, al16 ? deg1_mask(a) : 0u, A / 2, A / 4 * 3, stream));
     } else {
         TRY(grouped_fc_bn_bwd_chain(&a->post, stream, inplace ? 1 : 0));
         if (a->residual && !inplace) TRY(i3d_add_inplace(a->post.grad_h, a->grad_out, n, stream));
@@ -597,6 +629,8 @@
 
 static bool wgrad_multi_layer_ok(const I3dPnaLayerArgs* a) { return pna_layer_wgrad_multi(a, nullptr, true) == 1; }
 
+extern "C" long i3d_pna_layer_args_bytes(void) { return (long)sizeof(I3dPnaLayerArgs); }
+
 extern "C" int i3d_wgrad_stream_join(void* stream) { return join_wgrad(aux_for((hipStream_t)stream), stream); }
 
 extern "C" int i3d_event_create(void** event) {
diff --git a/3dinfomax_amd/csrc/gemm.hip b/3dinfomax_amd/csrc/gemm.hip
--- a/3dinfomax_amd/csrc/gemm.hip
+++ b/3dinfomax_amd/csrc/gemm.hip
@@ -33,7 +33,17 @@
     int c_bf16;
     int n_batch, z_splits;
     long a_batch, b_batch, c_batch;
+    unsigned grp_mask;
+    int grp_k_begin, grp_n_begin, grp_n_end;
+    int grp_m_stride;
 };
+
+__device__ __forceinline__ bool grp_marked(const GemmArgs& g, int bx) {
+    return g.grp_mask != 0 && ((g.grp_mask >> g.tile_group[bx]) & 1u) != 0;
+}
+__device__ __forceinline__ int grp_m_tile(const GemmArgs& g, int bx) {
+    return g.grp_mask != 0 ? (int)(((long)bx * g.grp_m_stride) % gridDim.x) : bx;
+}
 
 __device__ __forceinline__ int swz(int k, int idx) { return idx ^ ((((k) ^ (k >> 2)) & 1) << 4); }
 
@@ -562,17 +572,39 @@
     }
 }
 
+template <class S>
+__device__ __forceinline__ void zero_tile_cols(const GemmArgs& g, int bx, int c0, int c1) {
+    const int w4 = (c1 - c0) / 4;
+    for (int i = threadIdx.x; i < S::BM * w4; i += S::NT) {
+        const int ml = i / w4, m = bx * S::BM + ml;
+        const int row = m < g.M ? g.m_rows[m] : -1;
+        if (row >= 0) *reinterpret_cast<float4*>(g.C + (long)row * g.ldc + c0 + 4 * (i - ml * w4)) = make_float4(0.f, 0.f, 0.f, 0.f);
+    }
+}
+
 template <class S, bool VEC, bool A_KC, bool B_KC, int BF16 = 0>
 __global__ void __launch_bounds__(256)
 gemm_f32_kernel(GemmArgs g) {
     I3D_CHAIN_PRIO();
     int bx, by, bz;
     xcd_tile(bx, by, bz);
+    bx = grp_m_tile(g, bx);
     const int slice = bz;
     if (g.n_batch > 1) {
         const int bb = bz / g.z_splits;
         bz -= bb * g.z_splits;
         g.A += bb * g.a_batch; g.B += bb * g.b_batch; g.C += bb * g.c_batch;
+    }
+    if (grp_marked(g, bx)) {
+        const int n0 = by * S::BN, n1 = min(n0 + S::BN, g.N);
+        if (n0 >= g.grp_n_end || n1 <= g.grp_n_begin) {
+            zero_tile_cols<S>(g, bx, n0, n1);
+            return;
+        }
+        if (n1 > g.grp_n_end) {
+            zero_tile_cols<S>(g, bx, g.grp_n_end, n1);
+            g.N = g.grp_n_end;
+        }
     }
     const int k_begin = bz * g.k_per_split;
     const int k_end = min(g.K, k_begin + g.k_per_split);
@@ -854,7 +886,8 @@
     I3D_CHAIN_PRIO();
     int bx, by, bz;
     xcd_tile(bx, by, bz);
-    gemm_body<S, true, true, true, false, FUSE, BF16>(g, bx, by, 0, g.K, g.C, nullptr, true);
+    bx = grp_m_tile(g, bx);
+    gemm_body<S, true, true, true, false, FUSE, BF16>(g, bx, by, grp_marked(g, bx) ? g.grp_k_begin : 0, g.K, g.C, nullptr, true);
 }
 
 template <class S, int FUSE>
@@ -863,7 +896,8 @@
     I3D_CHAIN_PRIO();
     int bx, by, bz;
     xcd_tile(bx, by, bz);
-    gemm_body<S, true, true, true, false, FUSE, false>(g, bx, by, 0, g.K, g.C, nullptr, true);
+    bx = grp_m_tile(g, bx);
+    gemm_body<S, true, true, true, false, FUSE, false>(g, bx, by, grp_marked(g, bx) ? g.grp_k_begin : 0, g.K, g.C, nullptr, true);
 }
 
 template <class S>
@@ -902,6 +936,15 @@
         case 1: hipLaunchKernelGGL((gemm_f32_fused_kernel<S, 1>), grid, block, 0, s, g); break;
         case 2: hipLaunchKernelGGL((gemm_f32_fused_kernel<S, 2>), grid, block, 0, s, g); break;
         default: hipLaunchKernelGGL((gemm_f32_fused_kernel<S, 3>), grid, block, 0, s, g); break;
+    }
+}
+
+static int grp_stride_for(int m_tiles) {
+    if (m_tiles <= 8) return 1;
+    for (int s = 7;; ++s) {
+        int a = s, b = m_tiles;
+        while (b != 0) { const int t = a % b; a = b; b = t; }
+        if (a == 1) return s;
     }
 }
 
@@ -924,6 +967,8 @@
     const float* post_row = nullptr;
     int n_batch = 1;
     long a_batch = 0, b_batch = 0, c_batch = 0;
+    unsigned grp_mask = 0;
+    int grp_n_begin = 0, grp_n_end = 0;
 };
 
 static int fill_views(GemmArgs& g, int trans_a, int trans_b, int M, int N, int K, int lda, int ldb, const Extra& ex) {
@@ -973,6 +1018,14 @@
                       "batched product: plain (or row-grouped forward / data-gradient) operands, at most 32 batches");
         g.n_batch = nb; g.a_batch = ex.a_batch; g.b_batch = ex.b_batch; g.c_batch = ex.c_batch;
     }
+    if (ex.grp_mask != 0) {
+        I3D_CHECK_ARG(layout == 1 && nb == 1 && ex.m_rows != nullptr && ex.tile_group != nullptr && !accumulate && bias == nullptr &&
+                          vec && g.c_vec && N % 4 == 0 && ex.grp_n_begin % 4 == 0 && ex.grp_n_end % 4 == 0 &&
+                          0 <= ex.grp_n_begin && ex.grp_n_begin < ex.grp_n_end && ex.grp_n_end <= N,
+                      "live columns: grouped data gradient without accumulate, 16-byte aligned operands, bounds multiples of 4");
+        g.grp_mask = ex.grp_mask; g.grp_n_begin = ex.grp_n_begin; g.grp_n_end = ex.grp_n_end;
+        g.grp_m_stride = grp_stride_for(cdiv(M, 64));
+    }
 
     if (layout == 3) {
         I3D_CHECK_ARG(ex.m_rows == nullptr && ex.tile_group == nullptr, "row indirection needs a k-contiguous A");
@@ -1272,6 +1325,16 @@
     return gemm_impl(0, trans_b, m_padded, N, K, A, lda, B, ldb, C, ldc, nullptr, accumulate, -1, 0, ex, stream);
 }
 
+extern "C" int i3d_gemm_f32_grouped_live(int m_padded, int N, int K, const float* A, int lda, long a_rows_total, const int* m_rows,
+                                         const int* tile_group, const float* B, int ldb, long b_group_stride, float* C, int ldc,
+                                         unsigned group_mask, int n_begin, int n_end, void* stream) {
+    I3D_CHECK_ARG(m_rows != nullptr && tile_group != nullptr && m_padded % 64 == 0, "grouped GEMM needs 64-padded m_rows");
+    Extra ex;
+    ex.m_rows = m_rows; ex.tile_group = tile_group; ex.b_group_stride = b_group_stride; ex.a_rows_total = a_rows_total;
+    ex.grp_mask = group_mask; ex.grp_n_begin = n_begin; ex.grp_n_end = n_end;
+    return gemm_impl(0, 0, m_padded, N, K, A, lda, B, ldb, C, ldc, nullptr, 0, -1, 0, ex, stream);
+}
+
 extern "C" int i3d_gemm_f32_rowsubset(int M, int N, int n_rows, const float* A, int lda, const float* B, int ldb,
                                       const int* k_rows, long rows_total, float* C, int ldc, int accumulate,
                                       void* stream) {
@@ -1320,6 +1383,16 @@
                                       float* C, int ldc, const float* c_in, int ldcin, const float* bias, int accumulate,
                                       const float* a_aff, int epi_act, float* stats, const int* m_rows, const int* tile_group,
                                       long b_group_stride, void* stream) {
+    return i3d_gemm_f32_fused_src_kskip(M, N, K, A, lda, a_rows_total, W, ldb, C, ldc, c_in, ldcin, bias, accumulate, a_aff, epi_act,
+                                        stats, m_rows, tile_group, b_group_stride, 0, 0, stream);
+}
+
+extern "C" int i3d_gemm_f32_fused_src_kskip(int M, int N, int K, const float* A, int lda, long a_rows_total, const float* W, int ldb,
+                                            float* C, int ldc, const float* c_in, int ldcin, const float* bias, int accumulate,
+                                            const float* a_aff, int epi_act, float* stats, const int* m_rows, const int* tile_group,
+                                            long b_group_stride, unsigned group_mask, int k_begin, void* stream) {
+    I3D_CHECK_ARG(group_mask == 0 || (tile_group != nullptr && k_begin >= 0 && k_begin < K && k_begin % 4 == 0),
+                  "per-group K start: grouped form, a multiple of 4 inside [0, K)");
     I3D_CHECK_ARG(c_in == nullptr || (stats != nullptr && accumulate && ldcin >= N && ldcin % 4 == 0 && (((uintptr_t)c_in) & 15) == 0),
                   "c_in needs the statistics variant with accumulate, a pitch >= N that is a multiple of 4, 16-byte alignment");
     I3D_CHECK_ARG(M > 0 && N > 0 && K > 0, "empty GEMM");
@@ -1342,6 +1415,8 @@
     g.b_split = g.c_split = 0x7fffffff; g.b_delta = g.c_delta = 0;
     g.slab = nullptr;
     g.a_aff = a_aff; g.stats = stats; g.epi_act = epi_act; g.Cin = c_in; g.ldcin = ldcin; g.c_bf16 = g_fused_c_bf16;
+    g.grp_mask = group_mask; g.grp_k_begin = group_mask != 0 ? k_begin : 0;
+    g.grp_m_stride = grp_stride_for(cdiv(M, 64));
     Extra ex;
     ex.m_rows = m_rows; ex.a_rows_total = a_rows_total;
     int rc = fill_views(g, 0, 1, M, N, K, lda, ldb, ex);
diff --git a/3dinfomax_amd/csrc/grouped.hip b/3dinfomax_amd/csrc/grouped.hip
--- a/3dinfomax_amd/csrc/grouped.hip
+++ b/3dinfomax_amd/csrc/grouped.hip
@@ -25,6 +25,47 @@
         for (int s = 0; s < S; ++s) {
             const float c = coef.c[g][s];
             o.x += c * w[s].x; o.y += c * w[s].y; o.z += c * w[s].z; o.w += c * w[s].w;
+        }
+        WD[(long)g * per + t] = o;
+    }
+}
+
+template <int S>
+__global__ void __launch_bounds__(256)
+combine_weights_fwd_deg1_kernel(const float4* __restrict__ W, int ldw4, int f_in4, int f_out, int A4, int n_groups, Coef coef,
+                                unsigned collapse, float4* __restrict__ WD) {
+    I3D_CHAIN_PRIO();
+    long t = (long)blockIdx.x * blockDim.x + threadIdx.x;
+    long per = (long)f_out * A4;
+    if (t >= per) return;
+    int n = (int)(t / A4), k = (int)(t - (long)n * A4);
+    const int FV = A4 / 4, blk = k / FV;
+    float4 w[S], w0[S], w1[S];
+#pragma unroll
+    for (int s = 0; s < S; ++s) {
+        const float4* row = W + (long)n * ldw4 + f_in4 + (long)s * A4;
+        w[s] = row[k];
+        w0[s] = blk == 2 ? row[k - 2 * FV] : make_float4(0.f, 0.f, 0.f, 0.f);
+        w1[s] = blk == 2 ? row[k - FV] : make_float4(0.f, 0.f, 0.f, 0.f);
+    }
+    auto combine = [&](const float4* v, int g) {
+        float4 o = make_float4(0.f, 0.f, 0.f, 0.f);
+#pragma unroll
+        for (int s = 0; s < S; ++s) {
+            const float c = coef.c[g][s];
+            o.x += c * v[s].x; o.y += c * v[s].y; o.z += c * v[s].z; o.w += c * v[s].w;
+        }
+        return o;
+    };
+    for (int g = 0; g < n_groups; ++g) {
+        float4 o = combine(w, g);
+        if ((collapse >> g) & 1u) {
+            if (blk < 2) {
+                o = make_float4(0.f, 0.f, 0.f, 0.f);
+            } else if (blk == 2) {
+                const float4 a = combine(w0, g), b = combine(w1, g);
+                o = make_float4((a.x + b.x) + o.x, (a.y + b.y) + o.y, (a.z + b.z) + o.z, (a.w + b.w) + o.w);
+            }
         }
         WD[(long)g * per + t] = o;
     }
@@ -102,6 +143,20 @@
     return I3D_OK;
 }
 
+extern "C" int i3d_pna_combine_weights_fwd_deg1(const float* W, int ldw, int f_in, int f_out, int agg_width, int n_groups,
+                                                int n_scalers, const float* coef, unsigned collapse_mask, float* WD, void* stream) {
+    if (collapse_mask == 0) return i3d_pna_combine_weights_fwd(W, ldw, f_in, f_out, agg_width, n_groups, n_scalers, coef, WD, stream);
+    I3D_CHECK_ARG(f_in % 4 == 0 && agg_width % 16 == 0 && ldw % 4 == 0, "four aggregator blocks whose width is a multiple of 4");
+    I3D_CHECK_ARG((((uintptr_t)W | (uintptr_t)WD) & 15) == 0, "16-byte aligned pointers required");
+    Coef c;
+    I3D_CHECK_ARG(fill_coef(coef, n_groups, n_scalers, c) == 0, "1..32 groups and 1..4 scalers supported");
+    long items = (long)f_out * (agg_width / 4);
+    I3D_COMBINE_LAUNCH(combine_weights_fwd_deg1_kernel, (const float4*)W, ldw / 4, f_in / 4, f_out, agg_width / 4, n_groups, c,
+                       collapse_mask, (float4*)WD);
+    I3D_CHECK_LAUNCH();
+    return I3D_OK;
+}
+
 extern "C" int i3d_pna_combine_weights_bwd(const float* dWD, int ldw, int f_in, int f_out, int agg_width, int n_groups,
                                            int n_scalers, const float* coef, float* dW, void* stream) {
     I3D_CHECK_ARG(f_in % 4 == 0 && agg_width % 4 == 0 && ldw % 4 == 0, "dimensions must be multiples of 4");
diff --git a/3dinfomax_amd/csrc/model.hip b/3dinfomax_amd/csrc/model.hip
--- a/3dinfomax_amd/csrc/model.hip
+++ b/3dinfomax_amd/csrc/model.hip
@@ -229,7 +229,9 @@
         fill_tail(g.tail, pp, ar.take(F), ar.take(F));
         g.num_nodes = N; g.f_h = F; g.f_out = F; g.agg_width = A; g.ldw = pp.f_in;
         g.n_groups = b.n_groups; g.n_scalers = m.n_scalers; g.m_padded = b.m_padded;
-        for (int k = 0; k < b.n_groups; ++k) { g.group_start[k] = b.group_start[k]; g.group_count[k] = b.group_count[k]; }
+        for (int k = 0; k < b.n_groups; ++k) {
+            g.group_start[k] = b.group_start[k]; g.group_count[k] = b.group_count[k]; g.group_degree[k] = b.group_degree[k];
+        }
         for (int k = 0; k < b.n_groups * m.n_scalers; ++k) g.coef[k] = c.coef[k];
         g.h = c.h[l]; g.W = pp.W; g.bias = pp.bias;
         g.agg = ar.take((long)N * A);
diff --git a/3dinfomax_amd/layer_native.py b/3dinfomax_amd/layer_native.py
--- a/3dinfomax_amd/layer_native.py
+++ b/3dinfomax_amd/layer_native.py
@@ -188,8 +188,8 @@
     _tail(p.tail, spec, ga, be, ar.take(Fp0), ar.take(Fp0), Fp0, dev)
     p.num_nodes, p.f_h, p.f_out, p.agg_width, p.ldw = N, Fh, Fp0, A, W.stride(0)
     p.n_groups, p.n_scalers, p.m_padded = nG, nS, rows_d.shape[0]
-    for gi, (_, start, count) in enumerate(groups):
-        p.group_start[gi], p.group_count[gi] = start, count
+    for gi, (degree, start, count) in enumerate(groups):
+        p.group_start[gi], p.group_count[gi], p.group_degree[gi] = start, count, degree
     k = 0
     for g_ in plan.coef:
         for v in g_:
diff --git a/include/infomax3d_hip.h b/include/infomax3d_hip.h
--- a/include/infomax3d_hip.h
+++ b/include/infomax3d_hip.h
@@ -106,6 +106,11 @@
 int i3d_gemm_f32_grouped(int trans_b, int m_padded, int N, int K, const float* A, int lda, long a_rows_total,
                          const int* m_rows, const int* tile_group, const float* B, int ldb, long b_group_stride,
                          float* C, int ldc, int accumulate, void* stream);
+int i3d_pna_combine_weights_fwd_deg1(const float* W, int ldw, int f_in, int f_out, int agg_width, int n_groups, int n_scalers,
+                                     const float* coef, unsigned collapse_mask, float* WD, void* stream);
+int i3d_gemm_f32_grouped_live(int m_padded, int N, int K, const float* A, int lda, long a_rows_total, const int* m_rows,
+                              const int* tile_group, const float* B, int ldb, long b_group_stride, float* C, int ldc,
+                              unsigned group_mask, int n_begin, int n_end, void* stream);
 int i3d_gemm_f32_rowsubset(int M, int N, int n_rows, const float* A, int lda, const float* B, int ldb,
                            const int* k_rows, long rows_total, float* C, int ldc, int accumulate, void* stream);
 int i3d_gemm_f32_rowsubset_multi(int M, int N, int n_groups, const int* group_start, const int* group_count,
@@ -261,6 +266,10 @@
                            int ldc, const float* c_in, int ldcin, const float* bias, int accumulate, const float* a_aff,
                            int epi_act, float* stats, const int* m_rows, const int* tile_group, long b_group_stride,
                            void* stream);
+int i3d_gemm_f32_fused_src_kskip(int M, int N, int K, const float* A, int lda, long a_rows_total, const float* W, int ldb, float* C,
+                                 int ldc, const float* c_in, int ldcin, const float* bias, int accumulate, const float* a_aff,
+                                 int epi_act, float* stats, const int* m_rows, const int* tile_group, long b_group_stride,
+                                 unsigned group_mask, int k_begin, void* stream);
 int i3d_gemm_f32_fused_bf16out(int M, int N, int K, const float* A, int lda, long a_rows_total, const float* W, int ldb, void* C, int ldc,
                                const float* bias, const float* a_aff, int epi_act, float* stats, void* stream);
 int i3d_pna_pack_h_weights(const float* W_edge, int ldw_edge, int f_out_edge, const float* W_post, int ldw_post, int f_out_post,
@@ -447,7 +456,11 @@
     float* grad_bias;
     float* grad_h;
     float* grad_agg;
+    int group_degree[32];
 } I3dGroupedFcArgs;
+long i3d_pna_layer_args_bytes(void);
+int i3d_set_deg1_collapse(int mode);
+int i3d_get_deg1_collapse(void);
 
 #define I3D_MAX_EXTRA_FC 3
 typedef struct {
```

Measured after the change: 277,400. -1.3%, worse.
